# spacejam/tla-rust

Measured on AMD Instinct MI355X. Metric: distinct states/sec, raft.tla (3 servers), higher is better.
Workload: dtype u64

## Files before the change

### tla_rust_amd/build.py

```python
import os
import subprocess
from pathlib import Path

PKG = Path(__file__).resolve().parent
CSRC = PKG / "csrc"
OUT = PKG / "_build"
LIB = OUT / "libtlamc.so"
CLI = OUT / "mc"

SOURCES = ["engine.hip", "frontend.cpp"]

ENGINE_BASE = ["engine.hip", "hip_owned.h", "engine_kernels.h", "engine_sim.h", "sim_walk.h", "engine_behaviours.h", "behaviour.h", "engine_coverage.h", "coverage.h", "engine_violations.h", "violations.h",
               "engine_graph.h",
               "graph.h", "liveness.h", "live_query.h", "state_graph.h", "spec_gen.h", "mc_common.h", "spec_registry.h", "../../include/tlamc.h"]
ENGINE_OWN = {0: ["spec_pluscal.h", "spec_raft.h", "spec_ssi.h", "spec_vm.h", "spec_vm_cfg.h", "spec_paxos.h", "engine_pairs.h"], 7: ["spec_paxos.h"], 1: ["spec_pluscal.h"],
              2: ["spec_raft.h"], 3: ["spec_raft.h"], 4: ["spec_raft.h"], 5: ["spec_ssi.h", "engine_pairs.h"], 6: ["spec_vm.h", "spec_vm_cfg.h"]}
STATE_GRAPH_DEPS = ["state_graph.hip", "state_graph.h", "engine_live.h", "hip_owned.h", "liveness.h", "live_query.h", "graph.h", "coverage.h", "mc_common.h", "spec_registry.h",
                    "spec_gen.h", "spec_pluscal.h", "spec_raft.h", "spec_ssi.h", "spec_vm.h", "spec_vm_cfg.h", "spec_paxos.h", "../../include/tlamc.h"]


def _stale(target, deps):
    if not target.exists():
        return True
    t = target.stat().st_mtime
    return any(d.stat().st_mtime > t for d in deps)


def build(force=False, verbose=False):
    OUT.mkdir(exist_ok=True)
    hipcc = os.environ.get("HIPCC", "/opt/rocm/bin/hipcc")
    deps = list(CSRC.glob("*")) + [PKG.parent / "include" / "tlamc.h"]
    srcs = [str(CSRC / s) for s in SOURCES if (CSRC / s).exists()]
    common = [hipcc, "--offload-arch=gfx950", "-O3", "-std=c++17", "-fPIC", "-Wno-unused-value", "-Wno-unused-result",
              "-I", str(PKG.parent / "include")]
    if os.environ.get("TLAMC_LINE_TABLES"):
        common.append("-gline-tables-only")
    if os.environ.get("TLAMC_EXTRA_DEFS"):
        common += os.environ["TLAMC_EXTRA_DEFS"].split()
    if os.environ.get("TLAMC_PHASE_PROF"):
        common.append("-DMC_PHASE_PROF")
    jobs, objs = [], []
    for tu in range(8):
        obj = OUT / f"engine_tu{tu}.o"
        objs.append(obj)
        if force or _stale(obj, [CSRC / h for h in ENGINE_BASE + ENGINE_OWN[tu]]):
            jobs.append((obj, subprocess.Popen(common + ["-x", "hip", f"-DMC_TU={tu}", "-c", str(CSRC / "engine.hip"), "-o", str(obj)])))
    obj = OUT / "state_graph.o"
    objs.append(obj)
    if force or _stale(obj, [CSRC / d for d in STATE_GRAPH_DEPS]):
        jobs.append((obj, subprocess.Popen(common + ["-x", "hip", "-c", str(CSRC / "state_graph.hip"), "-o", str(obj)])))
    host_deps = {"frontend": ["frontend.cpp", "pcal.h", "spec_vm.h", "mc_common.h", "tlaeval.h"], "pcal": ["pcal.cpp", "pcal.h"],
                 "tlaeval": ["tlaeval.cpp", "tlaeval.h"],
                 "pcal_compile": ["pcal_compile.cpp", "pcal.h", "spec_vm.h", "spec_vm_cfg.h", "mc_common.h"],
                 "pcal_codegen": ["pcal_codegen.cpp", "pcal.h", "spec_vm.h", "mc_common.h"]}
    for name, dd in host_deps.items():
        obj = OUT / f"{name}.o"
        objs.append(obj)
        if force or _stale(obj, [CSRC / d for d in dd] + [PKG.parent / "include" / "tlamc.h"]):
            jobs.append((obj, subprocess.Popen(common + ["-x", "hip", "-c", str(CSRC / f"{name}.cpp"), "-o", str(obj)])))
    obj = OUT / "shard_rccl.o"
    objs.append(obj)
    if force or _stale(obj, [CSRC / "shard_rccl.cpp", CSRC / "shard_loop.h", PKG.parent / "include" / "tlamc.h"]):
        jobs.append((obj, subprocess.Popen(common + ["-x", "hip", "-c", str(CSRC / "shard_rccl.cpp"), "-o", str(obj)])))
    for obj, pr in jobs:
        if pr.wait() != 0:
            raise RuntimeError(f"hipcc failed for {obj.name}")
    if force or jobs or not LIB.exists():
        cmd = [hipcc, "--offload-arch=gfx950", "-shared", "-fPIC", "-o", str(LIB)] + [str(o) for o in objs] + ["-ldl", "-pthread"]
        if verbose:
            print(" ".join(cmd))
        subprocess.run(cmd, check=True)
    main = CSRC / "mc_main.cpp"
    if main.exists() and (force or _stale(CLI, deps + [LIB])):
        cmd = [hipcc, "-O2", "-std=c++17", "-I", str(PKG.parent / "include"), "-o", str(CLI), str(main),
               "-L", str(OUT), "-ltlamc", "-Wl,-rpath,$ORIGIN"]
        if verbose:
            print(" ".join(cmd))
        subprocess.run(cmd, check=True)
    calib_src = PKG.parent / "profiles" / "calib" / "calib_fetch.hip"
    calib = OUT / "calib_fetch"
    if calib_src.exists() and (force or _stale(calib, [calib_src])):
        subprocess.run([hipcc, "--offload-arch=gfx950", "-O3", "-Wno-unused-value", "-Wno-unused-result", "-o", str(calib), str(calib_src)], check=True)
    loc_src = PKG.parent / "profiles" / "calib" / "probe_locality.hip"
    loc = OUT / "probe_locality"
    if loc_src.exists() and (force or _stale(loc, [loc_src])):
        subprocess.run([hipcc, "--offload-arch=gfx950", "-O3", "-Wno-unused-value", "-Wno-unused-result", "-o", str(loc), str(loc_src)], check=True)
    return LIB


if __name__ == "__main__":
    print(build(force=True, verbose=True))
```

### tla_rust_amd/csrc/coverage.h

```cpp
#pragma once
#include "mc_common.h"
#include "spec_registry.h"
#include "spec_gen.h"

namespace mc {

constexpr int COV_MAX_BINS = 512;

MC_HD bool cov_counts(unsigned st) { return (st & ST_ENABLED) != 0; }

template <class S>
struct CovAction;

template <>
struct CovAction<SpecAtomicAdd> {
    static constexpr bool BY_SLOT = true;
    MC_HD static int nbins(const SpecAtomicAdd::Params &) { return 3 + 1; }
    MC_HD static bool listed(const SpecAtomicAdd::Params &, int a) { return a >= 0 && a < 3; }
    template <class Ref>
    MC_HD static int of(const SpecAtomicAdd::Params &p, const SpecAtomicAdd::Local &, Ref, int slot) { return SpecAtomicAdd::action_of(p, nullptr, slot); }
};
template <>
struct CovAction<SpecPcalIntro> {
    static constexpr bool BY_SLOT = false;
    MC_HD static int nbins(const SpecPcalIntro::Params &) { return 5 + 1; }
    MC_HD static bool listed(const SpecPcalIntro::Params &, int a) { return a >= 0 && a < 5; }
    template <class Ref>
    MC_HD static int of(const SpecPcalIntro::Params &p, const SpecPcalIntro::Local &l, Ref, int slot) { return SpecPcalIntro::action_of(p, &l.w, slot); }
};
template <>
struct CovAction<SpecPaxos> {
    static constexpr bool BY_SLOT = true;
    MC_HD static int nbins(const PaxosParams &) { return 6 + 1; }
    MC_HD static bool listed(const PaxosParams &p, int a) { return p.kind == 1 ? (a >= 0 && a < 2) : (a >= 2 && a < 6); }
    template <class Ref>
    MC_HD static int of(const PaxosParams &p, const SpecPaxos::Local &, Ref, int slot) { return SpecPaxos::action_of(p, nullptr, slot); }
};
template <int N>
struct CovAction<SpecRaft<N>> {
    using S = SpecRaft<N>;
    static constexpr bool BY_SLOT = false;
    MC_HD static int nbins(const RaftParams &) { return 10 + 1; }
    MC_HD static bool listed(const RaftParams &, int a) { return a >= 0 && a < 10; }
    template <class Ref>
    MC_HD static int of(const RaftParams &p, const typename S::Local &l, Ref s, int slot) {
        typename S::Delta d;
        int action = -1;
        S::compute(p, l, s, slot, d, action);
        return action;
    }
};
template <>
struct CovAction<SpecSsi> {
    static constexpr bool BY_SLOT = false;
    MC_HD static int nbins(const SsiParams &) { return 7 + 1; }
    MC_HD static bool listed(const SsiParams &, int a) { return a >= 0 && a < 7; }
    template <class Ref>
    MC_HD static int of(const SsiParams &p, const SpecSsi::Local &l, Ref, int slot) {
        SpecSsi::Delta d;
        int action = -1;
        SpecSsi::compute(p, l, slot, d, action);
        return action;
    }
};
MC_HD int cov_vm_nlabels(const VmParams &p) { return p.self_tab - p.label_tab; }
template <int MAXV>
struct CovAction<SpecVmT<MAXV>> {
    using S = SpecVmT<MAXV>;
    static constexpr bool BY_SLOT = false;
    MC_HD static int nbins(const VmParams &p) { return cov_vm_nlabels(p) + 1 + 1; }
    MC_HD static bool listed(const VmParams &p, int a) { return a >= 0 && a <= cov_vm_nlabels(p) && a != p.done; }
    template <class Ref>
    MC_HD static int of(const VmParams &p, const typename S::Local &l, Ref, int slot) {
        if (slot >= p.ninst * p.maxch) return cov_vm_nlabels(p);
        return slot < 0 ? -1 : l.v[p.pc_base + slot / p.maxch];
    }
};
template <int MAXV>
struct CovAction<SpecVmCfgT<MAXV>> : CovAction<SpecVmT<MAXV>> {};
template <class G>
struct CovAction<SpecGenT<G>> {
    using S = SpecGenT<G>;
    static constexpr bool BY_SLOT = false;
    MC_HD static int nbins(const VmParams &) { return G::NLABELS + 1 + 1; }
    MC_HD static bool listed(const VmParams &, int a) { return a >= 0 && a <= G::NLABELS && a != G::DONE; }
    template <class Ref>
    MC_HD static int of(const VmParams &, const typename S::Local &, Ref s, int slot) {
        if (slot >= G::NINST * G::MAXCH) return G::NLABELS;
        return slot < 0 ? -1 : (int)G::pc_from_row(s, slot / G::MAXCH);
    }
};

template <class S, class Add>
inline void cov_state(const typename S::Params &prm, CWordRef s, Add &&add) {
    typename S::Local loc;
    S::load(prm, s, loc);
    const int ns = S::nslots(prm, loc);
    for (int slot = 0; slot < ns; ++slot) {
        uint64_t fp = 0;
        const unsigned st = S::eval(prm, loc, s, slot, fp);
        if (cov_counts(st)) add(CovAction<S>::of(prm, loc, s, slot));
    }
}

}
```

### tla_rust_amd/csrc/engine.hip

```cpp
#include <hip/hip_runtime.h>

#include <algorithm>
#include <chrono>
#include <memory>
#include <type_traits>
#include <string>
#include <vector>

#include "spec_registry.h"
#include "hip_owned.h"

namespace mc {

#ifndef MC_TU
#define MC_TU -1
#endif
}
#include "engine_kernels.h"
#include "engine_pairs.h"
#include "engine_sim.h"
#include "engine_behaviours.h"
#include "engine_coverage.h"
#include "engine_violations.h"
#include "engine_graph.h"
#include "state_graph.h"
namespace mc {

struct EngineBase {
    DevBuf<int32_t> owned_device_blob;
    uint64_t program_hash = 0;
    mc_progress_fn progress_fn = nullptr;
    void *progress_user = nullptr;
    double progress_interval = 1.0;
    std::chrono::steady_clock::time_point progress_last;
    bool stop_requested = false;
    void report_progress(uint32_t levels, uint64_t generated, uint64_t distinct, uint64_t queue) {
        if (!progress_fn) return;
        const auto now = std::chrono::steady_clock::now();
        if (std::chrono::duration<double>(now - progress_last).count() < progress_interval) return;
        progress_last = now;
        progress_fn(progress_user, levels, generated, distinct, queue);
    }
    virtual ~EngineBase() = default;
    virtual int run(mc_result *out) = 0;
    virtual int step(uint32_t levels, mc_result *out) = 0;
    virtual int trace(uint8_t *states_out, int32_t *actions_out, size_t *n_inout) = 0;
    virtual int kernel_stats(mc_kernel_stats *out) = 0;
    virtual int read_states(uint64_t first, uint64_t count, uint8_t *out) = 0;
    virtual int debug_reexpand(unsigned extra_flags, double *ms) = 0;
    virtual int debug_phases(uint64_t *out48, int reset) = 0;
    virtual int debug_flags(uint32_t set, uint32_t clear) = 0;
    virtual int seen_layout(uint64_t *buckets, uint32_t *slots) = 0;
    virtual int checkpoint(const char *path) = 0;
    virtual int restore(const char *path) = 0;
    virtual int shard_begin() = 0;
    virtual int shard_begin_replicated(uint64_t min_frontier, uint64_t max_distinct, uint64_t max_levels, uint64_t *levels_out, uint32_t *nlevels) = 0;
    virtual int shard_level_size(uint64_t *n) = 0;
    virtual int shard_set_stream(void *hip_stream, int enable) = 0;
    virtual int shard_expand_launch(unsigned slot, uint64_t first, uint64_t count, uint64_t send_cap) = 0;
    virtual int shard_expand_finish(unsigned slot, uint64_t *send_fp, uint64_t send_cap, uint64_t *send_counts) = 0;
    virtual int shard_probe(const uint64_t *recv_fp, uint64_t n, uint8_t *answers) = 0;
    virtual int shard_expand_pack(unsigned slot, uint64_t *send_fp, uint64_t cap) = 0;
    virtual int shard_probe_pack(const uint64_t *recv_fp, uint64_t cap, uint8_t *answers) = 0;
    virtual int shard_keep_pack(unsigned slot, const uint8_t *answers_back, uint64_t cap) = 0;
    virtual int shard_wait_keep(unsigned slot) = 0;
    virtual int shard_materialise(unsigned slot, const uint8_t *answers_back, uint8_t *send_states, uint64_t send_cap, uint64_t *send_counts) = 0;
    virtual int shard_ingest(const uint8_t *recv_states, uint64_t n) = 0;
    virtual int shard_keep(unsigned slot, const uint8_t *answers_back, uint64_t *n_new) = 0;
    virtual int shard_end_level(uint64_t *new_local) = 0;
    virtual int shard_counters(uint64_t *generated, uint64_t *distinct_local, int32_t *verdict) = 0;
    virtual int shard_check_frontier() = 0;
    virtual int shard_materialise_parents(unsigned slot, uint64_t *send_parents) = 0;
    virtual int shard_ingest_parents(const uint64_t *recv_parents, uint64_t n, unsigned src_rank) = 0;
    virtual int shard_violation(int32_t *found, uint64_t *idx, uint32_t *slot, int32_t *verdict, int32_t *invariant) = 0;
    virtual int shard_fetch(uint64_t idx, uint8_t *state_out, uint32_t *parent_rank, uint64_t *parent_idx, uint32_t *parent_slot) = 0;
    virtual int shard_info(void **main_stream, uint64_t *chunk_states, int32_t *traced) = 0;
    virtual int shard_note_levels(const uint64_t *levels, uint32_t n, int32_t verdict) = 0;
    virtual int shard_resume(uint64_t *levels_out, uint32_t *nlevels) = 0;
    virtual int shard_checkpoint(const char *path) = 0;
    virtual int shard_restore(const char *path) = 0;
    virtual size_t state_bytes() const = 0;
    virtual int simulate(const mc_sim_opts *opts, mc_sim_result *out) = 0;
    virtual int behaviours(const mc_beh_opts *opts, mc_beh_verdict *out, mc_beh_result *result) = 0;
    virtual int behaviours_refused() = 0;
    virtual const mc_spec_desc *spec_desc() const = 0;
    virtual int coverage(mc_action_coverage *out, size_t *n_inout) = 0;
    virtual int violations(mc_violations_info *info, mc_violation *out, size_t *n_inout) = 0;
    virtual int violation_trace(size_t k, uint8_t *states_out, int32_t *actions_out, size_t *n_inout) = 0;
    StateGraph gr;
    bool sharded = false;
    hipStream_t graph_stream = nullptr;
    const std::vector<uint64_t> *graph_levels = nullptr;
    virtual int graph(mc_graph_info *out) = 0;
    virtual int predicates(uint64_t first, uint64_t count, uint32_t *bits_out) = 0;
    virtual int liveness_run(const LiveQuery &q, const mc_live_property *prop, mc_live_info *out, mc_live_check_info *check_out, mc_live_strong_info *strong_out) = 0;
    int liveness_edge_units(uint64_t first, uint64_t count, int8_t *unit_out) { return gr.live_unit_read(first, count, unit_out); }
    int graph_read(uint64_t first, uint64_t count, uint64_t *offsets_out, uint32_t *dst_out, int32_t *action_out, size_t *nedges_inout) {
        return gr.read(first, count, offsets_out, dst_out, action_out, nedges_inout);
    }
    int scc(mc_scc_info *out) {
        memset(out, 0, sizeof *out);
        if (sharded) { set_error("mc_engine_scc: not available for a sharded engine (shard_count > 1)"); return MC_EBADCFG; }
        if (!gr.built) { mc_graph_info gi; if (int rc = graph(&gi)) return rc; }
        return gr.scc(graph_stream, out);
    }
    int scc_read(uint64_t first, uint64_t count, uint32_t *scc_out) { return gr.scc_read(first, count, scc_out); }
    int liveness_components(uint64_t first, uint64_t count, uint32_t *scc_out) { return gr.live_scc_read(first, count, scc_out); }
    int liveness_trace(uint32_t *prefix_out, size_t *nprefix_inout, uint32_t *cycle_out, size_t *ncycle_inout) {
        return gr.live_trace(*graph_levels, prefix_out, nprefix_inout, cycle_out, ncycle_inout);
    }
};

static uint64_t round_pow2(uint64_t v) {
    uint64_t p = 1;
    while (p < v) p <<= 1;
    return p;
}

struct KTimer {
    std::vector<Event> pool;
    struct Pending { int which; size_t e0, e1; uint64_t units; };
    std::vector<Pending> pending;
    size_t used = 0;
    bool enabled = false;
    hipEvent_t get() {
        if (used == pool.size()) pool.emplace_back(hipEventDefault);
        return pool[used++].get();
    }
    void resolve(mc_kernel_stat *stats ) {
        for (auto &p : pending) {
            float ms = 0;
            hipEventElapsedTime(&ms, pool[p.e0].get(), pool[p.e1].get());
            stats[p.which].launches++;
            stats[p.which].ms_total += ms;
            stats[p.which].units += p.units;
        }
        pending.clear();
        used = 0;
    }
};

template <class S, class = void>
struct HasExport : std::false_type {};
template <class S>
struct HasExport<S, decltype((void)S::EXPORT_WORDS)> : std::true_type {};
template <class S, class = void>
struct PackedRows : std::false_type {};
template <class S>
struct PackedRows<S, decltype((void)S::PACKED_ROWS)> : std::integral_constant<bool, S::PACKED_ROWS> {};

static_assert((unsigned)SIM_VK_INVARIANT == VK_INVARIANT && (unsigned)SIM_VK_ASSERT == VK_ASSERT && (unsigned)SIM_VK_DEADLOCK == VK_DEADLOCK, "one verdict_of_kind");
static int32_t verdict_of_kind(unsigned kind) {
    return kind == VK_INVARIANT ? MC_V_INVARIANT : kind == VK_ASSERT ? MC_V_ASSERT : kind == VK_DEADLOCK ? MC_V_DEADLOCK : MC_V_SPECERR;
}
struct Viol {
    unsigned kind, slot;
    int32_t verdict, invariant;
    explicit Viol(unsigned long long key)
        : kind((unsigned)(key & 7u)), slot((unsigned)(key >> 8 & 0xffffu)), verdict(verdict_of_kind(kind)), invariant(kind == VK_INVARIANT ? (int32_t)(key >> 3 & 31u) : -1) {}
    bool extra_state() const { return kind == VK_INVARIANT && slot < SLOT_PARENT; }
};

struct CkIdent {
    char magic[8];
    uint32_t spec_id, nparams;
    int64_t params[16];
    uint32_t words, has_trace;
};
struct CkHeader {
    CkIdent id;
    uint64_t distinct, generated, cells, lo, hi, nlevels;
};
struct ShCkHeader {
    CkIdent id;
    uint32_t rank, world;
    uint64_t table_cap, lo, hi, next, dup, nlevels;
};
struct ShCkCounters {
    uint64_t arena_next, viol_key, via_list;
    uint64_t generated[NSHARD], cells[NSHARD];
    uint32_t error, pad;
};
static_assert(sizeof(CkIdent) == 152 && offsetof(CkIdent, spec_id) == 8 && offsetof(CkIdent, params) == 16 && offsetof(CkIdent, words) == 144 && offsetof(CkIdent, has_trace) == 148, "checkpoint identity");
static_assert(sizeof(CkHeader) == 200 && offsetof(CkHeader, distinct) == 152 && offsetof(CkHeader, generated) == 160 && offsetof(CkHeader, cells) == 168 &&
              offsetof(CkHeader, lo) == 176 && offsetof(CkHeader, hi) == 184 && offsetof(CkHeader, nlevels) == 192, "TLAMCCK1 header");
static_assert(sizeof(ShCkHeader) == 208 && offsetof(ShCkHeader, rank) == 152 && offsetof(ShCkHeader, world) == 156 && offsetof(ShCkHeader, table_cap) == 160 &&
              offsetof(ShCkHeader, lo) == 168 && offsetof(ShCkHeader, hi) == 176 && offsetof(ShCkHeader, next) == 184 && offsetof(ShCkHeader, dup) == 192 &&
              offsetof(ShCkHeader, nlevels) == 200, "TLAMCSK2 header");
static_assert(NSHARD == 8 && sizeof(ShCkCounters) == 160 && offsetof(ShCkCounters, generated) == 24 && offsetof(ShCkCounters, cells) == 88 && offsetof(ShCkCounters, error) == 152, "TLAMCSK2 counters");
struct CkFormat { const char *magic, *writer, *reader, *not_ours, *other_program; };
static constexpr CkFormat CK_FUSED{"TLAMCCK1", "checkpoint", "restore", "not a checkpoint file",
                                   "the checkpoint was written by another compiled program (algorithm, constants, invariants or constraints differ)"};
static constexpr CkFormat CK_RANK{"TLAMCSK2", "mc_shard_checkpoint", "mc_shard_restore", "not a per-rank checkpoint file (of this library version)",
                                  "the checkpoint was written by another compiled program"};
struct CkPart { void *p; size_t bytes; };
struct FileCloser { FILE *f; ~FileCloser() { if (f) fclose(f); } };

template <class S>
struct Engine : EngineBase {
    using Params = typename S::Params;
    int W = 1;
    unsigned max_slots = 1;
    Params prm;
    mc_spec_desc desc;
    mc_config cfg;
    Stream stream, stream2;
    Stream stream_b;
    Event ev_level, ev_e[2], ev_m[2];
    DevBuf<uint64_t> d_arena, d_table, d_cand, d_inittmp;
    DevBuf<uint32_t> d_newlist, d_parent;
    DevBuf<uint64_t> d_newfp;
    DevBuf<uint16_t> d_nsl, d_pslot;
    DevBuf<uint8_t> d_prank;
    DevBuf<DevCounters> d_ctr;
    PinnedBuf<DevCounters> h_ctr;
    DevBuf<LevelCtl> d_lc;
    PinnedBuf<LevelCtl> h_lc;
    uint64_t table_cap = 0, arena_cap = 0, chunk = 0, row_stride = 0, seg_cap = 0;
    bool seen_sparse = false, use_matrix = false;
    bool no_slices = getenv("TLAMC_NOSLICE") != nullptr;
    double inwave_growth_limit = getenv("TLAMC_INWAVE_GROWTH") ? atof(getenv("TLAMC_INWAVE_GROWTH")) : 10.0;
    KTimer timer;
    mc_kernel_stat kstat[3];
    struct Fused {
        bool have_run = false, have_viol = false;
        unsigned long long last_viol = ~0ull;
        std::vector<uint64_t> level_start;
        uint64_t last_distinct = 0, last_generated = 0, cells = 0, inwave = 0;
        uint64_t stop_frontier = 0, lo = 0, hi = 0;
        bool mat_inwave_level = false;
        uint64_t mat_list_hint = 0;
    } fr;
    struct HandOver {
        bool pending = false, in_place = false;
        uint64_t distinct = 0, generated = 0, cells = 0, lo = 0;
        std::vector<uint64_t> level_start;
    } ck;
    struct ShSlot {
        DevBuf<uint64_t> rt_fp;
        DevBuf<uint32_t> rt_src, pend_src;
        DevBuf<PaddedCounter> rt_cur;
        uint64_t rt_subcap = 0, pend_total = 0, chunk_base = 0, count = 0, ncols = 0;
        BlockPlan plan;
        uint64_t moved = 0;
        OwnerOffsets pend_off;
        bool launched = false, keep_pending = false;
    };
    struct Shard {
        uint64_t lo = 0, hi = 0, next = 0;
        uint64_t dup = 0;
        ShSlot sl[2];
        DevBuf<uint32_t> d_new_src, d_incl;
        DevBuf<unsigned long long> d_ends;
        PinnedBuf<unsigned long long> h_ends;
        PinnedBuf<PaddedCounter> h_cur;
        DevBuf<char> d_scan_tmp;
        hipStream_t ext_stream = nullptr;
        bool ext_side = false;
        Event ev_slot[2], ev_keep[2], ev_ans;
        Event ev_append;
        Event ev_exp[2];
        Event ev_mat[2];
        std::vector<uint64_t> levels;
        bool ck_ok = false, resume = false;
        std::unique_ptr<mc_result> prefix_res{new mc_result()};
    } sh;
    struct Sim {
        DevBuf<uint64_t> buf[2];
        DevBuf<uint32_t> wst;
        DevBuf<SimCounters> ctr;
        std::vector<uint64_t> trace_rows;
        std::vector<int32_t> trace_acts;
        size_t trace_n = 0;
    } sim;
    struct Beh {
        DevBuf<uint64_t> set[2], stage, rows, first, carry, mask;
        DevBuf<mc_beh_verdict> out;
        DevBuf<BehCounters> ctr;
    } beh;
    struct Cov {
        bool on = false;
        int nbins = 0;
        DevBuf<unsigned long long> bins;
        std::vector<uint64_t> host;
        uint64_t init_generated = 0;
    } cov;
    struct Vio {
        bool on = false;
        DevBuf<ViolBins> bins;
        ViolBins host;
        bool have_first = false, fatal = false;
        unsigned long long first_key = ~0ull;
        uint32_t flagged_levels = 0, passes = 0;
    } vio;

    unsigned slices_for(uint64_t ncols, bool blind) const {
        if (!WantsSlices<S>::value || S::FIX_SLOTS != 0 || UsesFamilies<S>::value || pairs_only() || use_matrix || max_slots < 16 || no_slices) return 1;
        const uint64_t waves = (ncols + 63) / 64;
        uint64_t sg = blind ? 32 : (16384 + waves - 1) / waves;
        if (sg > 32) sg = 32;
        if (sg > max_slots / 4) sg = max_slots / 4;
        return sg < 1 ? 1u : (unsigned)sg;
    }
    uint64_t seen_arg() const { return seen_sparse ? ((table_cap / MC_SPARSE_SLOTS) | SEEN_SPARSE) : table_cap / 8; }
    unsigned nranks() const { return cfg.shard_count > 1 ? cfg.shard_count : 1; }

    int alloc() {
        W = S::words(prm);
        max_slots = (unsigned)S::max_slots(prm);
        use_matrix = (cfg.flags & MC_F_MATRIX) != 0;
        HIP_TRY(hipSetDevice(cfg.device));
        HIP_TRY(stream.create());
        sharded = cfg.shard_count > 1;
        graph_stream = stream;
        graph_levels = &fr.level_start;
        {
            const char *pe = getenv("TLAMC_PRIO");
            int lo_p = 0, hi_p = 0;
            hipDeviceGetStreamPriorityRange(&lo_p, &hi_p);
            if (pe && *pe == '1') HIP_TRY(stream2.create(hi_p));
            else if (pe && *pe == '2') HIP_TRY(stream2.create(lo_p));
            else HIP_TRY(stream2.create());
        }
        for (int i = 0; i < 2; i++) { HIP_TRY(ev_e[i].create()); HIP_TRY(ev_m[i].create()); }
        {
            const char *es = getenv("TLAMC_EXPAND_STREAMS");
            if (es && *es == '2') {
                HIP_TRY(stream_b.create());
                HIP_TRY(ev_level.create());
            }
        }
        table_cap = cfg.table_capacity ? cfg.table_capacity : (1ull << 24);
        table_cap = (table_cap + 63) / 64 * 64;
        if (table_cap / 8 > 0xffffffffull) { set_error("table_capacity: at most 2^35 - 8 slots per device"); return MC_EBADCFG; }
        arena_cap = cfg.arena_capacity ? cfg.arena_capacity : (1ull << 22);
        arena_cap = (arena_cap + 63) & ~63ull;
        if (arena_cap >= (1ull << 32) - 1) { set_error("arena_capacity must be < 2^32 states"); return MC_EBADCFG; }
        static const double sparse_ratio = getenv("TLAMC_SPARSE_RATIO") && atof(getenv("TLAMC_SPARSE_RATIO")) >= 1.25 ? atof(getenv("TLAMC_SPARSE_RATIO")) : 3.0;
        seen_sparse = (double)table_cap >= sparse_ratio * (double)arena_cap && table_cap / MC_SPARSE_SLOTS <= 0xffffffffull && !getenv("TLAMC_DENSE_TABLE");
        chunk = cfg.chunk_states ? cfg.chunk_states : (1ull << 18);
        chunk = (chunk + 255) & ~255ull;
        if (chunk > (1ull << 24) - 256) chunk = (1ull << 24) - 256;
        if (max_slots > 255) { set_error("spec has more than 255 action slots per state"); return MC_EBADCFG; }
        row_stride = chunk + 256;
        HIP_TRY(d_arena.alloc(arena_cap * W));
        HIP_TRY(d_table.alloc(table_cap));
        HIP_TRY(d_cand.alloc((size_t)(use_matrix ? max_slots : 1) * row_stride));
        seg_cap = (row_stride / NSHARD + 256) * max_slots;
        seg_cap += seg_cap / 64 + 65;
        HIP_TRY(d_newlist.alloc((size_t)2 * NSHARD * seg_cap));
        if (HasKnownFp<S>::value && !use_matrix) HIP_TRY(d_newfp.alloc((size_t)2 * NSHARD * seg_cap));
        {
            const uint64_t ni = S::num_init(prm);
            HIP_TRY(d_inittmp.alloc((size_t)(ni < chunk ? ni : chunk) * W));
        }
        HIP_TRY(d_nsl.alloc(row_stride));
        if (cfg.flags & MC_F_TRACE) {
            HIP_TRY(d_parent.alloc(arena_cap));
            HIP_TRY(d_pslot.alloc(arena_cap));
            if (cfg.shard_count > 1) {
                HIP_TRY(d_prank.alloc(arena_cap));
                HIP_TRY(hipMemset(d_prank, 0xff, arena_cap));
            }
        }
        HIP_TRY(d_ctr.alloc(1));
        HIP_TRY(h_ctr.alloc(1));
        HIP_TRY(d_lc.alloc(1));
        HIP_TRY(h_lc.alloc(1));
        timer.enabled = (cfg.flags & MC_F_TIMING) != 0;
        if (cfg.flags & MC_F_COVERAGE) {
            cov.nbins = CovAction<S>::nbins(prm);
            if (cov.nbins > COV_MAX_BINS) { set_error("MC_F_COVERAGE: the model has more actions than the coverage histogram has bins (" + std::to_string(COV_MAX_BINS - 1) + ")"); return MC_EBADCFG; }
            HIP_TRY(cov.bins.alloc((size_t)2 * cov.nbins));
            HIP_TRY(hipMemset(cov.bins, 0, (size_t)2 * cov.nbins * sizeof(unsigned long long)));
            cov.host.assign((size_t)2 * cov.nbins, 0);
            cov.on = true;
        }
        if (cfg.flags & MC_F_CONTINUE) {
            if (ViolModel<S>::ninv(prm) > VIOL_MAX_INV) { set_error("MC_F_CONTINUE: the model has more than 32 invariants"); return MC_EBADCFG; }
            HIP_TRY(vio.bins.alloc(1));
            vio.on = true;
        }
        return MC_OK;
    }

    int viol_begin() {
        memset(&vio.host, 0, sizeof vio.host);
        for (int i = 0; i < VIOL_CELLS; i++) vio.host.first[i] = ~0ull;
        vio.have_first = vio.fatal = false;
        vio.first_key = ~0ull;
        vio.flagged_levels = vio.passes = 0;
        HIP_TRY(hipMemcpyAsync(vio.bins, &vio.host, sizeof vio.host, hipMemcpyHostToDevice, stream));
        return MC_OK;
    }
    void viol_stored(uint64_t lo, uint64_t hi) {
        for (uint64_t c0 = lo; c0 < hi; c0 += chunk) {
            const uint64_t c1 = c0 + chunk < hi ? c0 + chunk : hi;
            hipLaunchKernelGGL(k_viol_stored<S>, dim3((unsigned)((c1 - c0 + 255) / 256)), dim3(256), 0, stream, prm, (const uint64_t *)d_arena,
                               (const uint32_t *)d_parent, (const uint16_t *)d_pslot, c0, c1, vio.bins.p);
            vio.passes++;
        }
    }
    void viol_frontier(uint64_t lo, uint64_t hi) {
        each_chunk(lo, hi, [&](uint64_t c0, uint64_t c1, uint64_t ncols) {
            hipLaunchKernelGGL(k_viol_frontier<S>, dim3((unsigned)((ncols + 255) / 256)), dim3(256), 0, stream, prm, (const uint64_t *)d_arena,
                               c0, c1, ncols, (unsigned)cfg.flags, vio.bins.p);
            vio.passes++;
        });
    }
    int viol_level(uint64_t lo, uint64_t hi, uint64_t new_hi, bool expanded) {
        if (!vio.have_first) { vio.have_first = true; vio.first_key = h_ctr->viol_key; }
        vio.flagged_levels++;
        if (expanded) viol_frontier(lo, hi);
        if (!expanded || ChecksOnExpand<S>::value) viol_stored(lo, hi);
        else viol_stored(hi, new_hi);
        HIP_TRY(hipGetLastError());
        HIP_TRY(hipMemcpyAsync(&vio.host, vio.bins, sizeof vio.host, hipMemcpyDeviceToHost, stream));
        HIP_TRY(hipStreamSynchronize(stream));
        if (vio.host.count[VIOL_BINS + VIOL_BIN_FATAL]) { vio.fatal = true; return MC_OK; }
        hipLaunchKernelGGL(k_clear_viol_key, dim3(1), dim3(1), 0, stream, d_ctr.p);
        h_ctr->viol_key = ~0ull;
        return MC_OK;
    }
    uint32_t level_of(uint64_t idx) const {
        const auto it = std::upper_bound(fr.level_start.begin(), fr.level_start.end(), idx);
        return (uint32_t)(it - fr.level_start.begin());
    }
    struct ViolEntry { mc_violation v; int shown; unsigned long long key; };
    size_t viol_entries() const { return (size_t)ViolModel<S>::ninv(prm) + ((cfg.flags & MC_F_DEADLOCK) ? 1 : 0) + (vio.fatal ? 1 : 0); }
    int viol_entry(size_t k, ViolEntry &e) {
        const size_t ninv = (size_t)ViolModel<S>::ninv(prm);
        memset(&e, 0, sizeof e);
        e.v.invariant = -1;
        e.v.first_state = ~0ull;
        const bool dl = (cfg.flags & MC_F_DEADLOCK) != 0;
        int bin;
        if (k < ninv) { bin = (int)k; e.v.kind = MC_V_INVARIANT; e.v.invariant = (int32_t)k; }
        else if (dl && k == ninv) { bin = VIOL_BIN_DEADLOCK; e.v.kind = MC_V_DEADLOCK; }
        else if (vio.fatal && k == ninv + (dl ? 1 : 0)) bin = VIOL_BIN_FATAL;
        else { set_error("mc_engine_violations: entry out of range"); return MC_EBADCFG; }
        e.v.states = vio.host.count[bin];
        e.v.outside = vio.host.count[VIOL_BINS + bin];
        if (e.v.states) { e.shown = 1; e.v.first_state = vio.host.first[bin]; }
        else if (e.v.outside) {
            e.shown = 2;
            e.key = vio.host.first[VIOL_BINS + bin];
            e.v.first_state = viol_idx(e.key);
            if (bin == VIOL_BIN_FATAL) { const Viol f(e.key); e.v.kind = f.verdict; e.v.invariant = f.invariant; }
        }
        if (e.shown) {
            e.v.first_level = level_of(e.v.first_state);
            e.v.trace_len = e.v.first_level + (e.shown == 2 && Viol(e.key).extra_state() ? 1u : 0u);
        }
        return MC_OK;
    }
    int violations(mc_violations_info *info, mc_violation *out, size_t *n_inout) override {
        if (!vio.on) { set_error("mc_engine_violations: the engine was created without MC_F_CONTINUE"); return MC_ESTATE; }
        if (!fr.have_run) { set_error("mc_engine_violations: needs a search of this engine that returned a result"); return MC_ESTATE; }
        const size_t n = viol_entries();
        if (info) { info->flagged_levels = vio.flagged_levels; info->passes = vio.passes; info->fatal = vio.fatal ? 1u : 0u; info->pad = 0; }
        if (n > *n_inout || !out) { *n_inout = n; set_error("mc_engine_violations: buffer too small"); return MC_EBADCFG; }
        HIP_TRY(hipSetDevice(cfg.device));
        for (size_t k = 0; k < n; k++) {
            ViolEntry e;
            if (int rc = viol_entry(k, e)) return rc;
            out[k] = e.v;
        }
        *n_inout = n;
        return MC_OK;
    }
    int violation_trace(size_t k, uint8_t *states_out, int32_t *actions_out, size_t *n_inout) override {
        if (!vio.on) { set_error("mc_engine_violation_trace: the engine was created without MC_F_CONTINUE"); return MC_ESTATE; }
        if (!fr.have_run) { set_error("mc_engine_violation_trace: needs a search of this engine that returned a result"); return MC_ESTATE; }
        if (k >= viol_entries()) { set_error("mc_engine_violation_trace: entry out of range"); return MC_EBADCFG; }
        HIP_TRY(hipSetDevice(cfg.device));
        ViolEntry e;
        if (int rc = viol_entry(k, e)) return rc;
        if (!e.shown) { set_error("mc_engine_violation_trace: the entry has nothing to show"); return MC_EBADCFG; }
        const bool extra = e.shown == 2 && Viol(e.key).extra_state();
        return chain_trace(e.v.first_state, extra, extra ? Viol(e.key).slot : 0u, states_out, actions_out, n_inout);
    }

    template <class F>
    void each_chunk(uint64_t lo, uint64_t hi, F &&f) { mc::each_chunk(lo, hi, chunk, f); }
    void cov_generated(uint64_t lo, uint64_t hi) {
        each_chunk(lo, hi, [&](uint64_t c0, uint64_t c1, uint64_t ncols) {
            hipLaunchKernelGGL(k_coverage_generated<S>, dim3((unsigned)((ncols + 255) / 256)), dim3(256), 0, stream, prm, (const uint64_t *)d_arena,
                               c0, c1, ncols, cov.bins.p, cov.nbins);
        });
    }
    void cov_distinct(uint64_t lo, uint64_t hi) {
        for (uint64_t c0 = lo; c0 < hi; c0 += chunk) {
            const uint64_t c1 = c0 + chunk < hi ? c0 + chunk : hi;
            hipLaunchKernelGGL(k_coverage_distinct<S>, dim3((unsigned)((c1 - c0 + 255) / 256)), dim3(256), 0, stream, prm, (const uint64_t *)d_arena,
                               (const uint32_t *)d_parent, (const uint16_t *)d_pslot, c0, c1, cov.bins.p + cov.nbins, cov.nbins);
        }
    }
    int cov_begin(uint64_t expanded, uint64_t stored) {
        HIP_TRY(hipMemsetAsync(cov.bins, 0, (size_t)2 * cov.nbins * sizeof(unsigned long long), stream));
        cov.init_generated = S::num_init(prm);
        cov_generated(0, expanded);
        cov_distinct(0, stored);
        return MC_OK;
    }
    int cov_end() {
        HIP_TRY(hipMemcpyAsync(cov.host.data(), cov.bins, cov.host.size() * sizeof(uint64_t), hipMemcpyDeviceToHost, stream));
        HIP_TRY(hipStreamSynchronize(stream));
        cov.host[0] += cov.init_generated;
        return MC_OK;
    }
    int coverage(mc_action_coverage *out, size_t *n_inout) override {
        if (!cov.on) { set_error("mc_engine_coverage: the engine was created without MC_F_COVERAGE"); return MC_ESTATE; }
        size_t n = 1;
        for (int a = 0; a + 1 < cov.nbins; a++) n += CovAction<S>::listed(prm, a) ? 1 : 0;
        if (n > *n_inout || !out) { *n_inout = n; set_error("mc_engine_coverage: buffer too small"); return MC_EBADCFG; }
        size_t k = 0;
        for (int a = -1; a + 1 < cov.nbins; a++) {
            if (a >= 0 && !CovAction<S>::listed(prm, a)) continue;
            out[k].action = a;
            out[k].pad = 0;
            out[k].generated = cov.host[(size_t)a + 1];
            out[k].distinct = cov.host[(size_t)cov.nbins + a + 1];
            k++;
        }
        *n_inout = n;
        return MC_OK;
    }

    template <class K, class... A>
    void graph_chunks(K kernel, uint64_t lo, uint64_t hi, A... args) {
        each_chunk(lo, hi, [&](uint64_t c0, uint64_t c1, uint64_t ncols) {
            hipLaunchKernelGGL(kernel, dim3((unsigned)((ncols + 255) / 256)), dim3(256), 0, stream, prm, (const uint64_t *)d_arena, c0, c1, ncols,
                               (const uint64_t *)d_table, seen_arg(), args...);
        });
    }
    int graph(mc_graph_info *out) override {
        memset(out, 0, sizeof *out);
        if (cfg.shard_count > 1) { set_error("mc_engine_graph: not available for a sharded engine (shard_count > 1)"); return MC_EBADCFG; }
        if (!fr.have_run || ck.pending) {
            set_error("mc_engine_graph: needs a search of this engine that returned a result (mc_engine_run / mc_engine_step; not a simulation, "
                      "not a restored checkpoint that has not run yet: its seen-set is not built)");
            return MC_ESTATE;
        }
        gr.release();
        gr.device = cfg.device;
        const uint64_t n = fr.last_distinct, expanded = fr.lo;
        if (n + 1 > 0x7fffffffull) { set_error("mc_engine_graph: at most 2^31 - 2 states (the scan's item count)"); return MC_EBADCFG; }
        HIP_TRY(hipSetDevice(cfg.device));
        const auto t0 = std::chrono::steady_clock::now();
        DevBuf<uint32_t> slot_index, degree;
        DevBuf<GraphCounters> d_gc;
        DevBuf<char> scan_tmp;
        int rc;
        if ((rc = graph_alloc(slot_index, table_cap, "the fingerprint -> state index"))) return rc;
        if ((rc = graph_alloc(degree, n + 1, "the out-degrees"))) return rc;
        if ((rc = graph_alloc(gr.offsets, n + 1, "the row offsets"))) { gr.release(); return rc; }
        if ((rc = graph_alloc(d_gc, 1, "the counters"))) { gr.release(); return rc; }
        const int built = graph_build(n, expanded, slot_index, degree, d_gc, scan_tmp);
        if (built) { gr.release(); return built; }
        gr.info.states = n;
        gr.info.expanded = expanded;
        gr.info.init_states = fr.level_start.size() > 1 ? fr.level_start[1] : n;
        gr.info.seconds = std::chrono::duration<double>(std::chrono::steady_clock::now() - t0).count();
        gr.built = true;
        *out = gr.info;
        return MC_OK;
    }
    int graph_build(uint64_t n, uint64_t expanded, DevBuf<uint32_t> &slot_index, DevBuf<uint32_t> &degree, DevBuf<GraphCounters> &d_gc, DevBuf<char> &scan_tmp) {
        GraphCounters gc;
        memset(&gc, 0, sizeof gc);
        gc.first_bad = ~0ull;
        HIP_TRY(hipMemcpyAsync(d_gc, &gc, sizeof gc, hipMemcpyHostToDevice, stream));
        HIP_TRY(hipMemsetAsync(slot_index, 0xff, table_cap * sizeof(uint32_t), stream));
        HIP_TRY(hipMemsetAsync(degree, 0, (n + 1) * sizeof(uint32_t), stream));
        if (n) hipLaunchKernelGGL(k_graph_index<S>, dim3((unsigned)((n + 255) / 256)), dim3(256), 0, stream, prm, (const uint64_t *)d_arena, n,
                                  (const uint64_t *)d_table, seen_arg(), slot_index.p, table_cap, d_gc.p);
        graph_chunks(k_graph_degree<S>, 0, expanded, degree.p, d_gc.p);
        HIP_TRY(hipGetLastError());
        if (int rc = scan_exclusive_u32_to_u64(degree.p, gr.offsets.p, n + 1, scan_tmp, stream, "mc_engine_graph")) return rc;
        uint64_t edges = 0;
        HIP_TRY(hipMemcpyAsync(&edges, gr.offsets.p + n, sizeof edges, hipMemcpyDeviceToHost, stream));
        HIP_TRY(hipMemcpyAsync(&gc, d_gc, sizeof gc, hipMemcpyDeviceToHost, stream));
        HIP_TRY(hipStreamSynchronize(stream));
        if (int rc = graph_inconsistent(gc)) return rc;
        if (int rc = graph_alloc(gr.dst, edges, "the edges' successors")) return rc;
        if (int rc = graph_alloc(gr.act, edges, "the edges' actions")) return rc;
        graph_chunks(k_graph_fill<S>, 0, expanded, (const uint32_t *)slot_index.p, table_cap, (const uint64_t *)gr.offsets.p, gr.dst.p, gr.act.p, d_gc.p);
        HIP_TRY(hipGetLastError());
        HIP_TRY(hipMemcpyAsync(&gc, d_gc, sizeof gc, hipMemcpyDeviceToHost, stream));
        HIP_TRY(hipStreamSynchronize(stream));
        if (int rc = graph_inconsistent(gc)) return rc;
        gr.info.edges = edges;
        gr.info.self_loops = gc.self_loops;
        gr.info.dropped = gc.dropped;
        gr.info.max_out_degree = gc.max_degree;
        return MC_OK;
    }
    static int graph_inconsistent(const GraphCounters &gc) {
        if (!gc.missing_states && !gc.missing_succ) return MC_OK;
        const unsigned long long idx = gc.first_bad >> 16;
        const unsigned slot = (unsigned)(gc.first_bad & 0xffffu);
        set_error("mc_engine_graph: the seen-set does not hold " + std::to_string(gc.missing_states) + " stored state(s) and " + std::to_string(gc.missing_succ) +
                  " in-model successor(s); the first: state " + std::to_string(idx) + (slot == GRAPH_SLOT_SELF ? " itself" : ", slot " + std::to_string(slot)) +
                  " (two different states with one 64-bit fingerprint are the only legitimate cause: the second is never stored); no graph was built");
        return MC_ESTATE;
    }

    int predicates_build(const char *call) {
        if constexpr (!LivePred<S>::HAS) {
            return MC_ENOSPEC;
        } else {
            auto &lv = gr.lv;
            if (lv.pred_built) return MC_OK;
            LivePredTab tab;
            memset(&tab, 0, sizeof tab);
            tab.n = vm_live_preds(prm.host, tab.entry, LIVE_MAX_PREDS);
            if (tab.n > LIVE_MAX_PREDS) { set_error(std::string(call) + ": at most 32 predicates"); return MC_EBADCFG; }
            const uint64_t n = gr.info.states;
            HIP_TRY(hipSetDevice(cfg.device));
            DevBuf<unsigned long long> d_bad;
            if (int rc = graph_alloc(lv.pred, n, "the predicate bits", call)) return rc;
            if (int rc = graph_alloc(d_bad, 1, "the counters", call)) return rc;
            unsigned long long bad = ~0ull;
            HIP_TRY(hipMemcpyAsync(d_bad, &bad, sizeof bad, hipMemcpyHostToDevice, stream));
            HIP_TRY(hipMemsetAsync(lv.pred, 0, (n ? n : 1) * sizeof(uint32_t), stream));
            if (tab.n) graph_chunks(k_live_pred<S>, 0, n, tab, lv.pred.p, d_bad.p);
            HIP_TRY(hipGetLastError());
            HIP_TRY(hipMemcpyAsync(&bad, d_bad, sizeof bad, hipMemcpyDeviceToHost, stream));
            HIP_TRY(hipStreamSynchronize(stream));
            if (bad != ~0ull) {
                lv.pred.reset();
                set_error(std::string(call) + ": evaluating the predicate `" + vm_live_pred_text(prm.host, (int)(bad & 0xff)) + "` fails in state " +
                          std::to_string(bad >> 8) + " (an evaluation error: a function applied outside its domain, an overflow, ...)");
                return MC_ESTATE;
            }
            lv.pred_built = true;
            lv.npred = tab.n;
            return MC_OK;
        }
    }
    int predicates(uint64_t first, uint64_t count, uint32_t *bits_out) override {
        if (cfg.shard_count > 1) { set_error("mc_engine_predicates: not available for a sharded engine (shard_count > 1)"); return MC_EBADCFG; }
        if constexpr (!LivePred<S>::HAS) {
            set_error("mc_engine_predicates: this lowering has no compiled predicates (compiled PlusCal programs only)");
            return MC_ENOSPEC;
        } else {
            if (!gr.built) { mc_graph_info gi; if (int rc = graph(&gi)) return rc; }
            if (int rc = predicates_build("mc_engine_predicates")) return rc;
            return gr.pred_read(first, count, bits_out);
        }
    }

    static_assert(LiveProc<S>::HAS == LivePred<S>::HAS, "a lowering with process instances compiles predicates, and no other does");
    DevBuf<int8_t> live_unit_tab;
    int liveness_run(const LiveQuery &query, const mc_live_property *prop, mc_live_info *out, mc_live_check_info *check_out, mc_live_strong_info *strong_out) override {
        LiveQuery q = query;
        const std::string call(q.call);
        auto t0 = std::chrono::steady_clock::now();
        if (out) memset(out, 0, sizeof *out);
        if (check_out) memset(check_out, 0, sizeof *check_out);
        if (strong_out) memset(strong_out, 0, sizeof *strong_out);
        if (cfg.shard_count > 1) { set_error(call + ": not available for a sharded engine (shard_count > 1)"); return MC_EBADCFG; }
        if constexpr (!LiveProc<S>::HAS) {
            set_error(call + ": this lowering has no process instances (compiled PlusCal programs only)");
            return MC_ENOSPEC;
        } else {
            if (!fr.have_run || ck.pending || fr.have_viol || fr.hi != fr.lo) {
                set_error(call + ": needs a search of this engine that finished without a violation and with an empty queue (the complete state graph)");
                return MC_ESTATE;
            }
            if (!q.fu) {
                const int np = LiveProc<S>::count(prm);
                if (np > LIVE_MAX_PROCS) { set_error(call + ": at most 64 process instances"); return MC_EBADCFG; }
                q.all = np >= 64 ? ~0ull : (1ull << np) - 1;
            }
            if (prop && prop->refused) { set_error(call + ": the front end refused " + prop->name); return MC_EBADCFG; }
            if (prop && q.term()) { set_error(call + ": " + live_unknown_kind(q.kind)); return MC_EBADCFG; }
            if (int rc = live_query_check(q, prop ? vm_live_preds(prm.host, nullptr, 0) : 0)) return rc;
            int ni = 0, nl = 0;
            if (q.fu) {
                const int nu = vm_live_units(prm.host, &ni, &nl, nullptr, 0);
                if (q.fu->nunits < nu) { set_error(call + ": the program has " + std::to_string(nu) + " units, the table " + std::to_string(q.fu->nunits)); return MC_EBADCFG; }
            }
            if (!gr.built || !gr.lv.scc_built) { mc_scc_info si; if (int rc = scc(&si)) return rc; }
            auto &lv = gr.lv;
            const uint64_t edges = gr.info.edges;
            HIP_TRY(hipSetDevice(cfg.device));
            if (!q.refine && !prop) t0 = std::chrono::steady_clock::now();
            if (!q.fu && !lv.proc_built) {
                if (int rc = graph_alloc(lv.proc, edges, "the edges' processes", q.call)) return rc;
                HIP_TRY(hipMemsetAsync(lv.proc, 0xff, (edges ? edges : 1) * sizeof(int8_t), stream));
                graph_chunks(k_live_proc<S>, 0, fr.lo, (const uint64_t *)gr.offsets.p, lv.proc.p);
                lv.proc_built = true;
            }
            if (q.fu && !lv.unit_built) {
                std::vector<int8_t> tab((size_t)ni * (size_t)nl + 1, (int8_t)LIVE_TERM);
                vm_live_units(prm.host, &ni, &nl, tab.data(), (int)tab.size());
                if (int rc = graph_alloc(live_unit_tab, tab.size(), "the units of the labels", q.call)) return rc;
                if (int rc = graph_alloc(lv.unit, edges, "the edges' units", q.call)) return rc;
                HIP_TRY(hipMemcpyAsync(live_unit_tab, tab.data(), tab.size() * sizeof(int8_t), hipMemcpyHostToDevice, stream));
                HIP_TRY(hipMemsetAsync(lv.unit, 0xff, (edges ? edges : 1) * sizeof(int8_t), stream));
                graph_chunks(k_live_unit<S>, 0, fr.lo, (const uint64_t *)gr.offsets.p, LiveUnitTab{ni, nl, (const int8_t *)live_unit_tab.p}, lv.unit.p);
                HIP_TRY(hipStreamSynchronize(stream));
                lv.unit_built = true;
            }
            if (prop) if (int rc = predicates_build(q.call)) return rc;
            return gr.live_check(q, stream, t0, out, check_out, strong_out);
        }
    }

    template <class F>
    void timed(int which, uint64_t units, F &&launch, hipStream_t on = nullptr) {
        if (!timer.enabled) { launch(); return; }
        if (!on) on = stream;
        hipEvent_t a = timer.get(), b = timer.get();
        size_t ia = timer.used - 2, ib = timer.used - 1;
        hipEventRecord(a, on);
        launch();
        hipEventRecord(b, on);
        timer.pending.push_back({which, ia, ib, units});
    }

    int read_counters() {
        if (stream_b) HIP_TRY(hipStreamSynchronize(stream_b));
        HIP_TRY(hipStreamSynchronize(stream2));
        HIP_TRY(hipMemcpyAsync(h_ctr, d_ctr, sizeof(DevCounters), hipMemcpyDeviceToHost, stream));
        HIP_TRY(hipStreamSynchronize(stream));
        if (timer.enabled) timer.resolve(kstat);
        return MC_OK;
    }
    int check_dev_error() {
        if (h_ctr->error & DEV_EOVERFLOW) { set_error("packed-state capacity exceeded (raft messages / elections / allLogs slots, or a PlusCal sequence longer than its cells, or a recursive PlusCal procedure deeper than $TLAMC_PCAL_STACK frames)"); return MC_EOVERFLOW; }
        if (h_ctr->error & DEV_ETABLE) { set_error("seen-set full: raise table_capacity"); return MC_ETABLEFULL; }
        if (h_ctr->error & DEV_EROUTE) { set_error("sharded round: an exchange bucket is full (raise the fan-out allowance / send capacity)"); return MC_EROUTE; }
        if (h_ctr->error & DEV_EARENA) { set_error("state arena full: raise arena_capacity"); return MC_EARENA; }
        return MC_OK;
    }

    bool inwave_ok() const { return (UsesFamilies<S>::value || UsesPairs<S>::value) && !use_matrix && !(cfg.flags & (MC_F_NOFAMILY | MC_F_NOINWAVE)); }
    bool pairs_only() const { return UsesPairs<S>::value && inwave_ok(); }
    void set_inwave(RouteArgs &rt) const {
        if (!inwave_ok()) return;
        rt.arena_w = d_arena;
        rt.arena_cap = arena_cap;
        rt.parent = d_parent;
        rt.pslot = d_pslot;
    }
    static unsigned mat_grid(uint64_t ncols) {
        const unsigned bx = (unsigned)((ncols + 255) / 256);
        const unsigned gm = bx < 8 * 256 ? (bx + 7) / 8 : 256;
        return gm ? gm : 1u;
    }
    void finish_materialise(uint64_t chunk_base, uint64_t ncols, unsigned parity, hipStream_t expanded_on = nullptr) {
        if (pairs_only()) return;
        unsigned gm = mat_grid(ncols);
        if (fr.mat_inwave_level) {
            const uint64_t want = (fr.mat_list_hint * 4 + 255) / 256;
            const unsigned per_seg = (unsigned)((want + NSHARD - 1) / NSHARD);
            if (per_seg < gm) gm = per_seg ? per_seg : 1u;
        }
        hipEventRecord(ev_e[parity].get(), expanded_on ? expanded_on : stream.s);
        hipStreamWaitEvent(stream2, ev_e[parity].get(), 0);
        timed(2, 0, [&] {
            hipLaunchKernelGGL(k_materialise<S>, dim3(gm, NSHARD), dim3(256), 0, stream2, prm, d_arena, chunk_base, d_newlist,
                               seg_cap, arena_cap, d_parent, d_pslot, d_ctr, parity, (const LevelCtl *)nullptr, (const uint64_t *)d_newfp);
        }, stream2);
        hipLaunchKernelGGL(k_commit, dim3(1), dim3(1), 0, stream2, d_ctr, parity);
        hipEventRecord(ev_m[parity].get(), stream2);
        static const bool serial = getenv("TLAMC_SERIAL") != nullptr;
        if (serial) hipStreamSynchronize(stream2);
    }
    void enqueue_blind_level(uint64_t max_states) {
        const uint64_t ncols = max_states + 64;
        RouteArgs rt{};
        rt.lc = d_lc;
        rt.new_fp = d_newfp;
        set_inwave(rt);
        const unsigned sg = slices_for(ncols, true);
        const bool dl = sg > 1 && (cfg.flags & MC_F_DEADLOCK);
        if (dl) { rt.succ = d_nsl; hipMemsetAsync(d_nsl, 0, ncols * sizeof(uint16_t), stream); }
        const unsigned lflags = cfg.flags | ((cfg.flags & MC_F_PARK) ? MC_FI_PARK : 0u);
        timed(0, 0, [&] {
            launch_expand<S, false>(!(cfg.flags & MC_F_NOFAMILY), lflags, ncols, stream, sg, prm, (const uint64_t *)d_arena,
                                    (uint64_t)0, (uint64_t)0, ncols, d_table.p, seen_arg(), d_newlist.p, seg_cap, d_ctr.p, cfg.flags, rt, 0u);
            if (dl) hipLaunchKernelGGL(k_deadlock_slices, dim3((unsigned)((ncols + 255) / 256)), dim3(256), 0, stream, (const uint16_t *)d_nsl,
                                       (uint64_t)0, (uint64_t)0, ncols, (const LevelCtl *)d_lc, d_ctr);
        });
        if (!pairs_only()) timed(2, 0, [&] {
            hipLaunchKernelGGL(k_materialise<S>, dim3(32, NSHARD), dim3(256), 0, stream, prm, d_arena, (uint64_t)0, d_newlist, seg_cap,
                               arena_cap, d_parent, d_pslot, d_ctr, 0u, (const LevelCtl *)d_lc, (const uint64_t *)d_newfp);
        });
        hipLaunchKernelGGL(k_end_level, dim3(1), dim3(1), 0, stream, d_ctr, d_lc);
    }

    template <bool INIT>
    void finish_chunk(uint64_t chunk_base_or_first, uint64_t ncols, unsigned rows) {
        const unsigned bx = (unsigned)((ncols + 255) / 256);
        timed(1, ncols * rows, [&] {
            hipLaunchKernelGGL(k_insert, dim3(bx, rows), dim3(256), 0, stream, d_cand, row_stride, ncols, d_nsl, d_table,
                               seen_arg(), d_newlist, d_ctr);
        });
        const unsigned gm = bx < 2048 ? bx : 2048;
        timed(2, 0, [&] {
            if (INIT)
                hipLaunchKernelGGL(k_init_materialise<S>, dim3(gm), dim3(256), 0, stream, prm, d_arena, chunk_base_or_first,
                                   d_inittmp, d_newlist, arena_cap, d_parent, d_pslot, d_ctr);
            else
                hipLaunchKernelGGL(k_materialise<S>, dim3(gm, 1), dim3(256), 0, stream, prm, d_arena, chunk_base_or_first,
                                   d_newlist, seg_cap, arena_cap, d_parent, d_pslot, d_ctr, 0u, (const LevelCtl *)nullptr, (const uint64_t *)nullptr);
        });
        hipLaunchKernelGGL(k_commit, dim3(1), dim3(1), 0, stream, d_ctr, 0u);
    }

    int seed_init(unsigned rank, unsigned count, bool resuming, bool in_place, std::chrono::steady_clock::time_point *t0) {
        if (!in_place) HIP_TRY(hipMemsetAsync(d_table, 0, table_cap * sizeof(uint64_t), stream));
        HIP_TRY(hipMemsetAsync(d_ctr, 0, sizeof(DevCounters), stream));
        DevCounters init_c;
        memset(&init_c, 0, sizeof init_c);
        init_c.viol_key = ~0ull;
        if (resuming) {
            init_c.arena_next = ck.distinct;
            init_c.generated[0].v = ck.generated;
            init_c.cells[0].v = ck.cells;
        }
        HIP_TRY(hipMemcpyAsync(d_ctr, &init_c, sizeof init_c, hipMemcpyHostToDevice, stream));
        if (t0) {
            HIP_TRY(hipStreamSynchronize(stream));
            *t0 = std::chrono::steady_clock::now();
        }
        if (resuming && ck.distinct && !in_place)
            hipLaunchKernelGGL(k_reseed_table<S>, dim3((unsigned)((ck.distinct + 255) / 256)), dim3(256), 0, stream, prm,
                               (const uint64_t *)d_arena, ck.distinct, d_table, seen_arg(), d_ctr);
        const uint64_t ninit = resuming ? 0 : S::num_init(prm);
        for (uint64_t first = 0; first < ninit; first += chunk) {
            const uint64_t n = ninit - first < chunk ? ninit - first : chunk;
            const uint64_t ncols = (n + 63) & ~63ull;
            hipLaunchKernelGGL(k_init_cand<S>, dim3((unsigned)((ncols + 255) / 256)), dim3(256), 0, stream, prm, first, n,
                               d_inittmp, d_cand, ncols, d_nsl, d_ctr, rank, count);
            finish_chunk<true>(first, ncols, 1);
        }
        return MC_OK;
    }
    int close_level(uint64_t &lo, uint64_t &hi, uint64_t new_hi, uint32_t &level, mc_result *out) {
        lo = hi;
        hi = new_hi;
        if (hi > lo) {
            fr.level_start.push_back(lo);
            if (level < MC_MAX_LEVELS) out->level_distinct[level] = hi - lo;
            level++;
        }
        if (level >= MC_MAX_LEVELS) { set_error("too many BFS levels"); return MC_EBADCFG; }
        return MC_OK;
    }

    int run(mc_result *out) override {
        memset(out, 0, sizeof *out);
        out->violated_invariant = -1;
        memset(kstat, 0, sizeof kstat);
        fr.have_viol = false;
        sim.trace_n = 0;
        stop_requested = false;
        gr.release();
        fr.have_run = false;
        fr.level_start.clear();
        HIP_TRY(hipSetDevice(cfg.device));
        const bool resuming = ck.pending, in_place = ck.pending && ck.in_place;
        ck.pending = ck.in_place = false;
        std::chrono::steady_clock::time_point t0;
        int rc = seed_init(0u, 1u, resuming, in_place, &t0);
        if (rc) return rc;
        progress_last = t0;
        auto progress = [&](uint32_t lv, uint64_t lo_, uint64_t hi_) {
            if (!progress_fn) return;
            uint64_t g = 0;
            for (int t = 0; t < NSHARD; t++) g += h_ctr->generated[t].v;
            report_progress(lv, g, hi_, hi_ - lo_);
        };
        if (inwave_ok()) hipLaunchKernelGGL(k_set_alloc_mode, dim3(1), dim3(1), 0, stream, d_ctr, 1u);
        bool alloc_atomic = inwave_ok();
        uint64_t prev_frontier = ~0ull >> 12;
        if ((rc = read_counters())) return rc;
        if ((rc = check_dev_error())) return rc;
        uint64_t lo = 0, hi = h_ctr->arena_next;
        uint32_t level = 1;
        out->level_distinct[0] = hi;
        fr.level_start.push_back(0);
        if (cov.on && !in_place && (rc = cov_begin(resuming ? ck.lo : 0, hi))) return rc;
        if (vio.on) {
            if ((rc = viol_begin())) return rc;
            if (!resuming && h_ctr->viol_key != ~0ull && (rc = viol_level(0, hi, hi, false))) return rc;
        }
        if (resuming) {
            fr.level_start = ck.level_start;
            level = (uint32_t)fr.level_start.size();
            lo = ck.lo;
            for (uint32_t k = 0; k < level && k < MC_MAX_LEVELS; k++)
                out->level_distinct[k] = (k + 1 < level ? fr.level_start[k + 1] : hi) - fr.level_start[k];
        }
        int budget = 0;
        uint64_t via_seen = 0;
        const bool park_levels = (cfg.flags & MC_F_PARK) != 0;
        fr.mat_list_hint = ~0ull >> 8;
        fr.mat_inwave_level = false;
        static const int blind_log2 = getenv("TLAMC_BLIND_LOG2") ? atoi(getenv("TLAMC_BLIND_LOG2")) : 20;
        uint64_t blind_max = 1ull << (blind_log2 >= 10 && blind_log2 <= 23 && slices_for((1ull << 16) + 64, true) == 1 ? blind_log2 : 16);
        if (chunk < blind_max) blind_max = chunk;
        while (hi > lo) {
            if (h_ctr->viol_key != ~0ull) break;
            if (fr.stop_frontier && hi - lo >= fr.stop_frontier) break;
            if (cfg.max_levels && level >= cfg.max_levels) { budget = 1; break; }
            if (cfg.max_distinct && hi >= cfg.max_distinct) { budget = 1; break; }
            if (stop_requested) { budget = 1; break; }
            if (!use_matrix && !(cfg.flags & MC_F_NOBATCH) && hi - lo <= blind_max) {
                memset(h_lc, 0, sizeof(LevelCtl));
                h_lc->lo = lo;
                h_lc->hi = hi;
                h_lc->max_states = fr.stop_frontier && fr.stop_frontier - 1 < blind_max ? fr.stop_frontier - 1 : blind_max;
                h_lc->max_distinct = cfg.max_distinct;
                h_lc->levels_left = cfg.max_levels ? (unsigned)(cfg.max_levels - level) : 0u;
                HIP_TRY(hipMemcpyAsync(d_lc, h_lc, sizeof(LevelCtl), hipMemcpyHostToDevice, stream));
                HIP_TRY(hipStreamSynchronize(stream2));
                if (inwave_ok() && !alloc_atomic) {
                    hipLaunchKernelGGL(k_set_alloc_mode, dim3(1), dim3(1), 0, stream, d_ctr, 1u);
                    alloc_atomic = true;
                }
                for (int k = 0; k < BLIND_BATCH; k++) enqueue_blind_level(blind_max);
                HIP_TRY(hipMemcpyAsync(h_lc, d_lc, sizeof(LevelCtl), hipMemcpyDeviceToHost, stream));
                if ((rc = read_counters())) return rc;
                if ((rc = check_dev_error())) return rc;
                for (unsigned k = 0; k < h_lc->nlev; k++) {
                    kstat[0].units += hi - lo;
                    if (cov.on) { cov_generated(lo, hi); cov_distinct(hi, h_lc->level_hi[k]); }
                    if (vio.on && k + 1 == h_lc->nlev && h_ctr->viol_key != ~0ull && (rc = viol_level(lo, hi, h_lc->level_hi[k], true))) return rc;
                    if ((rc = close_level(lo, hi, h_lc->level_hi[k], level, out))) return rc;
                }
                progress(level, lo, hi);
                prev_frontier = hi > lo ? hi - lo : 1;
                continue;
            }
            const bool lvl_inwave = inwave_ok() && (pairs_only() || (double)(hi - lo) <= inwave_growth_limit * (double)prev_frontier);
            if (inwave_ok() && lvl_inwave != alloc_atomic) {
                hipLaunchKernelGGL(k_set_alloc_mode, dim3(1), dim3(1), 0, stream, d_ctr, lvl_inwave ? 1u : 0u);
                alloc_atomic = lvl_inwave;
            }
            prev_frontier = hi - lo;
            fr.mat_inwave_level = lvl_inwave;
            unsigned chunk_no = 0;
            const bool two_streams = stream_b && !use_matrix && hi - lo > chunk && !(slices_for(chunk, false) > 1 && (cfg.flags & MC_F_DEADLOCK));
            if (two_streams) {
                hipEventRecord(ev_level.get(), stream);
                hipStreamWaitEvent(stream_b, ev_level.get(), 0);
            }
            for (uint64_t c0 = lo; c0 < hi; ++chunk_no) {
                const unsigned parity = chunk_no & 1u;
                const uint64_t base = c0 & ~63ull;
                uint64_t c1 = base + chunk;
                if (c1 > hi) c1 = hi;
                const uint64_t ncols = ((c1 - base) + 63) & ~63ull;
                if (use_matrix) {
                    timed(0, c1 - c0, [&] {
                        hipLaunchKernelGGL(k_expand<S>, dim3((unsigned)((ncols + 255) / 256)), dim3(256), 0, stream, prm, d_arena,
                                           c0, c1, d_cand, row_stride, ncols, d_nsl, d_ctr, cfg.flags);
                    });
                    finish_chunk<false>(base, ncols, max_slots);
                } else {
                    hipStream_t es = two_streams && parity ? stream_b.s : stream.s;
                    if (chunk_no >= 2) hipStreamWaitEvent(es, ev_m[parity].get(), 0);
                    RouteArgs rt_new{};
                    rt_new.new_fp = d_newfp;
                    if (lvl_inwave) set_inwave(rt_new);
                    const unsigned sg = slices_for(ncols, false);
                    const bool dl = sg > 1 && (cfg.flags & MC_F_DEADLOCK);
                    if (dl) { rt_new.succ = d_nsl; hipMemsetAsync(d_nsl, 0, ncols * sizeof(uint16_t), es); }
                    const unsigned lflags = cfg.flags | (lvl_inwave && park_levels ? MC_FI_PARK : 0u);
                    timed(0, c1 - c0, [&] {
                        launch_expand<S, false>(!(cfg.flags & MC_F_NOFAMILY), lflags, ncols, es, sg, prm,
                                                (const uint64_t *)d_arena, c0, c1, ncols, d_table.p, seen_arg(), d_newlist.p, seg_cap, d_ctr.p,
                                                cfg.flags, rt_new, parity);
                        if (dl) hipLaunchKernelGGL(k_deadlock_slices, dim3((unsigned)((ncols + 255) / 256)), dim3(256), 0, es,
                                                   (const uint16_t *)d_nsl, c0, c1, ncols, (const LevelCtl *)nullptr, d_ctr);
                    }, es);
                    finish_materialise(base, ncols, parity, es);
                }
                c0 = c1;
            }
            if ((rc = read_counters())) return rc;
            if ((rc = check_dev_error())) return rc;
            {
                const uint64_t via = h_ctr->via_list - via_seen;
                via_seen = h_ctr->via_list;
                const double growth = hi > lo ? (double)(h_ctr->arena_next - hi) / (double)(hi - lo) : 1.0;
                fr.mat_list_hint = (uint64_t)((double)(via / (chunk_no ? chunk_no : 1u)) * (growth > 1.0 ? growth : 1.0)) + 1;
            }
            if (cov.on) { cov_generated(lo, hi); cov_distinct(hi, h_ctr->arena_next); }
            if (vio.on && h_ctr->viol_key != ~0ull && (rc = viol_level(lo, hi, h_ctr->arena_next, true))) return rc;
            if ((rc = close_level(lo, hi, h_ctr->arena_next, level, out))) return rc;
            progress(level, lo, hi);
        }
        if (cov.on && (rc = cov_end())) return rc;
        if (hi > lo && h_ctr->viol_key == ~0ull && !fr.stop_frontier && (rc = check_frontier(lo, hi))) return rc;
        if (vio.on && hi > lo && !vio.fatal && h_ctr->viol_key != ~0ull && (rc = viol_level(lo, hi, hi, false))) return rc;
        const unsigned long long run_key = vio.on && vio.have_first ? vio.first_key : h_ctr->viol_key;
        const auto t1 = std::chrono::steady_clock::now();
        out->seconds = std::chrono::duration<double>(t1 - t0).count();
        out->distinct = h_ctr->arena_next;
        fr.last_distinct = h_ctr->arena_next;
        kstat[2].units = h_ctr->arena_next;
        out->generated = 0;
        fr.cells = 0;
        for (int t = 0; t < NSHARD; t++) { out->generated += h_ctr->generated[t].v; fr.cells += h_ctr->cells[t].v; }
        fr.last_generated = out->generated;
        fr.inwave = inwave_ok() && h_ctr->arena_next >= h_ctr->via_list + (resuming ? ck.distinct : 0)
                           ? h_ctr->arena_next - h_ctr->via_list - (resuming ? ck.distinct : 0) : 0;
        fr.have_run = true;
        out->queue_left = hi - lo;
        out->depth = level;
        out->levels = level;
        fr.lo = lo;
        fr.hi = hi;
        if (run_key != ~0ull) {
            fr.have_viol = true;
            fr.last_viol = run_key;
            const Viol v(fr.last_viol);
            out->verdict = v.verdict;
            out->violated_invariant = v.invariant;
            std::vector<uint64_t> chain;
            if (build_chain(chain) == MC_OK) out->trace_len = (uint32_t)chain.size() + (v.extra_state() ? 1u : 0u);
        } else {
            out->verdict = budget ? MC_V_BUDGET : MC_V_OK;
        }
        return MC_OK;
    }

    int step(uint32_t levels, mc_result *out) override {
        if (!levels) return MC_EBADCFG;
        const uint64_t saved = cfg.max_levels;
        const bool cont = fr.have_run && !fr.have_viol && fr.hi > fr.lo && !ck.pending;
        if (cont) {
            ck.distinct = fr.last_distinct; ck.generated = fr.last_generated; ck.cells = fr.cells; ck.lo = fr.lo;
            ck.level_start = fr.level_start;
            ck.pending = ck.in_place = true;
            cfg.max_levels = (uint64_t)fr.level_start.size() + levels;
        } else if (ck.pending) {
            cfg.max_levels = (uint64_t)ck.level_start.size() + levels;
        } else {
            cfg.max_levels = levels;
        }
        const int rc = run(out);
        cfg.max_levels = saved;
        if (rc) ck.pending = ck.in_place = false;
        return rc;
    }
    bool ck_params_comparable() const { return desc.spec_id != MC_SPEC_PCAL; }
    void ck_fill_ident(CkIdent &id, const CkFormat &fmt) const {
        memcpy(id.magic, fmt.magic, 8);
        id.spec_id = desc.spec_id;
        id.nparams = ck_params_comparable() ? desc.nparams : 1;
        for (uint32_t i = 0; i < id.nparams && i < 16; i++) id.params[i] = desc.params[i];
        if (!ck_params_comparable()) id.params[0] = (int64_t)program_hash;
        id.words = (uint32_t)W;
        id.has_trace = d_parent ? 1u : 0u;
    }
    static int ck_fail(int code, const char *who, const std::string &msg) { set_error(std::string(who) + ": " + msg); return code; }
    int ck_check_ident(const CkIdent &id, const CkFormat &fmt) const {
        if (memcmp(id.magic, fmt.magic, 8) != 0) return ck_fail(MC_EPARSE, fmt.reader, fmt.not_ours);
        if (id.spec_id != desc.spec_id || id.words != (uint32_t)W) return ck_fail(MC_EBADCFG, fmt.reader, "the checkpoint belongs to another spec");
        if (ck_params_comparable() && (id.nparams != desc.nparams || memcmp(id.params, desc.params, sizeof(int64_t) * (id.nparams < 16 ? id.nparams : 16)) != 0))
            return ck_fail(MC_EBADCFG, fmt.reader, "the checkpoint was written with other constants / invariants");
        if (!ck_params_comparable() && (id.nparams != 1 || (uint64_t)id.params[0] != program_hash)) return ck_fail(MC_EBADCFG, fmt.reader, fmt.other_program);
        return MC_OK;
    }
    std::vector<CkPart> ck_sections(uint64_t n, bool per_rank) const {
        std::vector<CkPart> v{{d_arena.p, (size_t)((n + 63) >> 6) * (size_t)W * 64 * sizeof(uint64_t)}};
        if (d_parent) {
            v.push_back({d_parent.p, (size_t)n * sizeof(uint32_t)});
            v.push_back({d_pslot.p, (size_t)n * sizeof(uint16_t)});
        }
        if (per_rank && d_prank) v.push_back({d_prank.p, (size_t)n});
        if (per_rank) v.push_back({d_table.p, (size_t)table_cap * sizeof(uint64_t)});
        return v;
    }
    int ck_write(const CkFormat &fmt, const char *path, std::initializer_list<CkPart> host, const std::vector<CkPart> &dev) {
        FILE *f = fopen(path, "wb");
        if (!f) return ck_fail(MC_EBADCFG, fmt.writer, std::string("cannot write ") + path);
        FileCloser closer{f};
        int rc = MC_OK;
        for (const CkPart &h : host)
            if (!rc && fwrite(h.p, 1, h.bytes, f) != h.bytes) rc = ck_fail(MC_EBADCFG, fmt.writer, "short write");
        for (const CkPart &d : dev) {
            if (rc) break;
            std::vector<char> buf(d.bytes < (64u << 20) ? d.bytes : (64u << 20));
            for (size_t off = 0; off < d.bytes && !rc; off += buf.size()) {
                const size_t n = d.bytes - off < buf.size() ? d.bytes - off : buf.size();
                HIP_TRY(hipMemcpy(buf.data(), (const char *)d.p + off, n, hipMemcpyDeviceToHost));
                if (fwrite(buf.data(), 1, n, f) != n) rc = ck_fail(MC_EBADCFG, "checkpoint", "short write");
            }
        }
        closer.f = nullptr;
        if (fclose(f) != 0 && !rc) rc = ck_fail(MC_EBADCFG, fmt.writer, "close failed");
        return rc;
    }
    template <class H>
    int ck_read_header(const CkFormat &fmt, FILE *f, H &h) const {
        if (fread(&h, sizeof h, 1, f) != 1) return ck_fail(MC_EPARSE, fmt.reader, fmt.not_ours);
        return ck_check_ident(h.id, fmt);
    }
    static int ck_read_host(const CkFormat &fmt, FILE *f, std::initializer_list<CkPart> host) {
        for (const CkPart &h : host)
            if (fread(h.p, 1, h.bytes, f) != h.bytes) return ck_fail(MC_EPARSE, fmt.reader, "the checkpoint file is truncated");
        return MC_OK;
    }
    static int ck_read_sections(FILE *f, const std::vector<CkPart> &dev) {
        for (const CkPart &d : dev) {
            std::vector<char> buf(d.bytes < (64u << 20) ? d.bytes : (64u << 20));
            for (size_t off = 0; off < d.bytes; off += buf.size()) {
                const size_t n = d.bytes - off < buf.size() ? d.bytes - off : buf.size();
                if (fread(buf.data(), 1, n, f) != n) return ck_fail(MC_EPARSE, "restore", "the checkpoint file is truncated");
                HIP_TRY(hipMemcpy((char *)d.p + off, buf.data(), n, hipMemcpyHostToDevice));
            }
        }
        return MC_OK;
    }
    int checkpoint(const char *path) override {
        if (cfg.shard_count > 1) { set_error("checkpoint: not available for a sharded engine"); return MC_EBADCFG; }
        if (!fr.have_run || fr.have_viol) { set_error("checkpoint: needs a completed mc_engine_run that stopped on a budget (or finished) without a violation"); return MC_EBADCFG; }
        HIP_TRY(hipSetDevice(cfg.device));
        HIP_TRY(hipDeviceSynchronize());
        CkHeader h;
        memset(&h, 0, sizeof h);
        ck_fill_ident(h.id, CK_FUSED);
        h.distinct = fr.last_distinct; h.generated = fr.last_generated; h.cells = fr.cells;
        h.lo = fr.lo; h.hi = fr.hi; h.nlevels = fr.level_start.size();
        return ck_write(CK_FUSED, path, {{&h, sizeof h}, {fr.level_start.data(), fr.level_start.size() * sizeof(uint64_t)}}, ck_sections(fr.last_distinct, false));
    }
    int restore(const char *path) override {
        if (cfg.shard_count > 1) { set_error("restore: not available for a sharded engine"); return MC_EBADCFG; }
        gr.release();
        FileCloser f{fopen(path, "rb")};
        if (!f.f) return ck_fail(MC_EPARSE, "restore", std::string("cannot read ") + path);
        CkHeader h;
        int rc = ck_read_header(CK_FUSED, f.f, h);
        if (rc) return rc;
        if (h.distinct * 10 > table_cap * 9) return ck_fail(MC_ETABLEFULL, "restore", "table_capacity cannot hold the checkpoint's states (load > 0.9)");
        if (h.distinct > arena_cap) return ck_fail(MC_EARENA, "restore", "arena_capacity is smaller than the checkpoint");
        if (h.hi != h.distinct || h.lo > h.hi || h.nlevels == 0 || h.nlevels >= MC_MAX_LEVELS) return ck_fail(MC_EPARSE, "restore", "inconsistent header");
        if (d_parent && !h.id.has_trace) return ck_fail(MC_EBADCFG, "restore", "the checkpoint holds no parent pointers (written without MC_F_TRACE); run without MC_F_TRACE");
        ck.level_start.assign((size_t)h.nlevels, 0);
        if ((rc = ck_read_host(CK_FUSED, f.f, {{ck.level_start.data(), ck.level_start.size() * sizeof(uint64_t)}}))) return rc;
        bool ok = ck.level_start[0] == 0 && ck.level_start.back() < h.hi && (h.lo == h.hi || ck.level_start.back() == h.lo);
        for (size_t k = 1; k < ck.level_start.size() && ok; k++) ok = ck.level_start[k] > ck.level_start[k - 1];
        if (!ok) return ck_fail(MC_EPARSE, "restore", "inconsistent level table");
        HIP_TRY(hipSetDevice(cfg.device));
        if ((rc = ck_read_sections(f.f, ck_sections(h.distinct, false)))) return rc;
        ck.distinct = h.distinct; ck.generated = h.generated; ck.cells = h.cells; ck.lo = h.lo;
        ck.pending = true;
        return MC_OK;
    }
    int shard_checkpoint(const char *path) override {
        if (!sh.ck_ok || sh.levels.empty()) { set_error("mc_shard_checkpoint: needs a sharded run that ended (finished, or stopped on a budget) without an error"); return MC_EBADCFG; }
        HIP_TRY(hipSetDevice(cfg.device));
        HIP_TRY(hipDeviceSynchronize());
        ShCkHeader h;
        memset(&h, 0, sizeof h);
        ck_fill_ident(h.id, CK_RANK);
        h.rank = cfg.shard_rank; h.world = nranks();
        h.table_cap = table_cap | (seen_sparse ? SEEN_SPARSE : 0); h.lo = sh.lo; h.hi = sh.hi; h.next = sh.next; h.dup = sh.dup; h.nlevels = sh.levels.size();
        DevCounters dc;
        HIP_TRY(hipMemcpy(&dc, d_ctr, sizeof dc, hipMemcpyDeviceToHost));
        ShCkCounters c;
        memset(&c, 0, sizeof c);
        c.arena_next = dc.arena_next; c.viol_key = dc.viol_key; c.via_list = dc.via_list; c.error = dc.error;
        for (int t = 0; t < NSHARD; t++) { c.generated[t] = dc.generated[t].v; c.cells[t] = dc.cells[t].v; }
        return ck_write(CK_RANK, path, {{&h, sizeof h}, {sh.levels.data(), sh.levels.size() * sizeof(uint64_t)}, {&c, sizeof c}}, ck_sections(sh.next, true));
    }
    int shard_restore_read(FILE *f, ShCkHeader &h, ShCkCounters &fc) {
        int rc = ck_read_header(CK_RANK, f, h);
        if (rc) return rc;
        const char *who = CK_RANK.reader;
        if (h.rank != cfg.shard_rank || h.world != nranks()) return ck_fail(MC_EBADCFG, who, "the file is another rank's, or of a run with another number of ranks");
        if (h.table_cap != (table_cap | (seen_sparse ? SEEN_SPARSE : 0)))
            return ck_fail(MC_EBADCFG, who, "table_capacity differs from the checkpointed run's, or the bucket form it implies (4 slots when the table is >= 3 x the arena): the seen-set slice is stored as it lay in HBM");
        if (h.next > arena_cap) return ck_fail(MC_EARENA, who, "arena_capacity is smaller than the checkpoint");
        if (h.lo > h.hi || h.hi != h.next || h.dup > h.next || h.nlevels == 0 || h.nlevels >= MC_MAX_LEVELS) return ck_fail(MC_EPARSE, who, "inconsistent header");
        if ((d_parent.p != nullptr) != (h.id.has_trace != 0)) return ck_fail(MC_EBADCFG, who, "MC_F_TRACE differs from the checkpointed run's");
        sh.levels.assign((size_t)h.nlevels, 0);
        if ((rc = ck_read_host(CK_RANK, f, {{sh.levels.data(), sh.levels.size() * sizeof(uint64_t)}, {&fc, sizeof fc}}))) return rc;
        if (fc.arena_next != h.next || fc.viol_key != ~0ull || fc.error) return ck_fail(MC_EPARSE, who, "inconsistent counters");
        HIP_TRY(hipSetDevice(cfg.device));
        HIP_TRY(hipDeviceSynchronize());
        if ((rc = ck_read_sections(f, ck_sections(h.next, true)))) return rc;
        if (fgetc(f) != EOF) return ck_fail(MC_EPARSE, who, "trailing bytes (not the file this engine's configuration wrote)");
        return MC_OK;
    }
    int shard_restore(const char *path) override {
        if (int rc = refuse_packed()) return rc;
        FileCloser f{fopen(path, "rb")};
        if (!f.f) return ck_fail(MC_EPARSE, "mc_shard_restore", std::string("cannot read ") + path);
        ShCkHeader h;
        ShCkCounters fc;
        if (int rc = shard_restore_read(f.f, h, fc)) { sh.levels.clear(); return rc; }
        DevCounters c;
        memset(&c, 0, sizeof c);
        c.arena_next = fc.arena_next; c.viol_key = fc.viol_key; c.via_list = fc.via_list;
        for (int t = 0; t < NSHARD; t++) { c.generated[t].v = fc.generated[t]; c.cells[t].v = fc.cells[t]; }
        HIP_TRY(hipMemcpy(d_ctr, &c, sizeof c, hipMemcpyHostToDevice));
        memset(kstat, 0, sizeof kstat);
        sh.lo = h.lo; sh.hi = h.hi; sh.next = h.next; sh.dup = h.dup;
        fr.last_distinct = sh.next;
        fr.have_viol = false;
        sh.sl[0].launched = sh.sl[1].launched = false;
        sh.resume = true;
        sh.ck_ok = false;
        return MC_OK;
    }

    int fetch_state(uint64_t idx, uint64_t *words) {
        const uint64_t *src = d_arena + ((idx >> 6) * (uint64_t)W) * 64 + (idx & 63);
        HIP_TRY(hipMemcpy2D(words, sizeof(uint64_t), src, 64 * sizeof(uint64_t), sizeof(uint64_t), W, hipMemcpyDeviceToHost));
        return MC_OK;
    }
    int build_chain(std::vector<uint64_t> &chain) {
        chain.clear();
        if (!fr.have_viol) return MC_ESTATE;
        if (Viol(fr.last_viol).slot == SLOT_INIT) return MC_OK;
        return chain_to(viol_idx(fr.last_viol), chain);
    }
    int chain_to(uint64_t idx, std::vector<uint64_t> &chain) {
        chain.clear();
        if (!d_parent) { set_error("engine created without MC_F_TRACE"); return MC_ESTATE; }
        for (int guard = 0; guard < MC_MAX_LEVELS; ++guard) {
            chain.push_back(idx);
            uint32_t p;
            HIP_TRY(hipMemcpy(&p, d_parent + idx, sizeof p, hipMemcpyDeviceToHost));
            if (p == 0xffffffffu) break;
            idx = p;
        }
        std::vector<uint64_t> rev(chain.rbegin(), chain.rend());
        chain.swap(rev);
        return MC_OK;
    }
    int trace(uint8_t *states_out, int32_t *actions_out, size_t *n_inout) override {
        if (sim.trace_n) return sim_trace_out(states_out, actions_out, n_inout);
        if (!fr.have_viol) { *n_inout = 0; return MC_OK; }
        HIP_TRY(hipSetDevice(cfg.device));
        const Viol v(fr.last_viol);
        if (v.slot == SLOT_INIT) {
            std::vector<uint64_t> words(W);
            S::init(prm, viol_idx(fr.last_viol), WordRef{words.data(), 1});
            std::vector<int32_t> acts{-1};
            return trace_out(words, acts, states_out, actions_out, n_inout);
        }
        return chain_trace(viol_idx(fr.last_viol), v.extra_state(), v.slot, states_out, actions_out, n_inout);
    }
    int chain_trace(uint64_t end, bool extra, unsigned slot, uint8_t *states_out, int32_t *actions_out, size_t *n_inout) {
        std::vector<uint64_t> words, chain;
        std::vector<int32_t> acts;
        int rc = chain_to(end, chain);
        if (rc) return rc;
        words.resize(chain.size() * W);
        for (size_t k = 0; k < chain.size(); ++k) {
            if ((rc = fetch_state(chain[k], &words[k * W]))) return rc;
            if (k == 0) acts.push_back(-1);
            else {
                uint16_t ps;
                HIP_TRY(hipMemcpy(&ps, d_pslot + chain[k], sizeof ps, hipMemcpyDeviceToHost));
                acts.push_back(S::action_of(prm, &words[(k - 1) * W], (int)ps));
            }
        }
        if (extra) {
            std::vector<uint64_t> last(words.end() - W, words.end());
            words.resize(words.size() + W);
            S::apply(prm, CWordRef{last.data(), 1}, (int)slot, WordRef{&words[words.size() - W], 1});
            acts.push_back(S::action_of(prm, last.data(), (int)slot));
        }
        return trace_out(words, acts, states_out, actions_out, n_inout);
    }
    int trace_out(const std::vector<uint64_t> &words, const std::vector<int32_t> &acts, uint8_t *states_out, int32_t *actions_out, size_t *n_inout) {
        const size_t n = acts.size();
        if (n > *n_inout) { *n_inout = n; set_error("trace buffer too small"); return MC_EBADCFG; }
        if constexpr (HasExport<S>::value) {
            for (size_t k = 0; k < n; ++k) S::export_row(prm, &words[k * W], (uint64_t *)states_out + k * (size_t)S::EXPORT_WORDS);
        } else
        memcpy(states_out, words.data(), n * W * sizeof(uint64_t));
        memcpy(actions_out, acts.data(), n * sizeof(int32_t));
        *n_inout = n;
        return MC_OK;
    }
    int read_states(uint64_t first, uint64_t count, uint8_t *out) override {
        if (!count) return MC_OK;
        if (first + count > fr.last_distinct) { set_error("read_states: range beyond the states found by the last run"); return MC_EBADCFG; }
        HIP_TRY(hipSetDevice(cfg.device));
        DevBuf<uint64_t> tmp;
        const uint64_t piece = 1ull << 20;
        HIP_TRY(tmp.alloc((count < piece ? count : piece) * W));
        for (uint64_t off = 0; off < count; off += piece) {
            const uint64_t n = count - off < piece ? count - off : piece;
            hipLaunchKernelGGL(k_gather_states, dim3((unsigned)((n * W + 255) / 256)), dim3(256), 0, stream, d_arena, W, first + off, n, tmp);
            hipError_t e1, e2;
            if constexpr (HasExport<S>::value) {
                std::vector<uint64_t> rows((size_t)n * W);
                e1 = hipMemcpyAsync(rows.data(), tmp, n * W * sizeof(uint64_t), hipMemcpyDeviceToHost, stream);
                e2 = hipStreamSynchronize(stream);
                if (e1 == hipSuccess && e2 == hipSuccess)
                    for (uint64_t k = 0; k < n; ++k) S::export_row(prm, &rows[(size_t)k * W], (uint64_t *)out + (size_t)(off + k) * (size_t)S::EXPORT_WORDS);
            } else {
                e1 = hipMemcpyAsync(out + off * W * sizeof(uint64_t), tmp, n * W * sizeof(uint64_t), hipMemcpyDeviceToHost, stream);
                e2 = hipStreamSynchronize(stream);
            }
            if (e1 != hipSuccess || e2 != hipSuccess) { set_error("read_states: copy failed"); return MC_EHIP; }
        }
        return MC_OK;
    }
    int debug_flags(uint32_t set, uint32_t clear) override { cfg.flags = (cfg.flags & ~clear) | set; return MC_OK; }
    int seen_layout(uint64_t *buckets, uint32_t *slots) override {
        *buckets = seen_arg() & ~SEEN_SPARSE;
        *slots = seen_sparse ? MC_SPARSE_SLOTS : 8;
        return MC_OK;
    }
    int debug_phases(uint64_t *out48, int reset) override {
#ifdef MC_PHASE_PROF
        HIP_TRY(hipSetDevice(cfg.device));
        HIP_TRY(hipDeviceSynchronize());
        HIP_TRY(hipMemcpyFromSymbol(out48, HIP_SYMBOL(g_phase), 48 * sizeof(uint64_t)));
        if (reset) { static const unsigned long long zero[48] = {}; HIP_TRY(hipMemcpyToSymbol(HIP_SYMBOL(g_phase), zero, sizeof zero)); }
        return MC_OK;
#else
        (void)out48; (void)reset;
        set_error("the library was built without MC_PHASE_PROF");
        return MC_ESTATE;
#endif
    }
    int debug_reexpand(unsigned extra_flags, double *ms) override {
        HIP_TRY(hipSetDevice(cfg.device));
        Event a(hipEventDefault), b(hipEventDefault);
        HIP_TRY(hipEventRecord(a.get(), stream));
        for (uint64_t c0 = 0; c0 < fr.last_distinct; c0 += chunk) {
            const uint64_t c1 = c0 + chunk < fr.last_distinct ? c0 + chunk : fr.last_distinct;
            const uint64_t ncols = ((c1 - c0) + 63) & ~63ull;
            launch_expand<S, false>(!((cfg.flags | extra_flags) & MC_F_NOFAMILY), cfg.flags | extra_flags, ncols, stream, 0u, prm,
                                    (const uint64_t *)d_arena, c0, c1, ncols, d_table.p, seen_arg(), d_newlist.p, seg_cap, d_ctr.p,
                                    cfg.flags | extra_flags, RouteArgs{}, 0u);
            hipLaunchKernelGGL(k_commit, dim3(1), dim3(1), 0, stream, d_ctr, 0u);
        }
        HIP_TRY(hipEventRecord(b.get(), stream));
        HIP_TRY(hipStreamSynchronize(stream));
        float t = 0;
        HIP_TRY(hipEventElapsedTime(&t, a.get(), b.get()));
        *ms = t;
        return MC_OK;
    }
    int shard_alloc(ShSlot &q, uint64_t send_cap) {
        const unsigned P = nranks();
        if (send_cap > q.pend_src.n) {
            q.rt_fp.reset(); q.rt_src.reset(); q.pend_src.reset();
            q.rt_subcap = (send_cap / (P * NSHARD)) * 2 + 4096;
            HIP_TRY(q.rt_fp.alloc((size_t)P * NSHARD * q.rt_subcap));
            HIP_TRY(q.rt_src.alloc((size_t)P * NSHARD * q.rt_subcap));
            HIP_TRY(q.pend_src.alloc(send_cap));
        }
        HIP_TRY(q.rt_cur.reserve((size_t)(P * NSHARD)));
        if (send_cap > sh.d_incl.n) {
            sh.d_new_src.reset(); sh.d_incl.reset();
            HIP_TRY(sh.d_new_src.alloc(send_cap));
            HIP_TRY(sh.d_incl.alloc(send_cap));
        }
        HIP_TRY(sh.d_ends.reserve(8));
        HIP_TRY(sh.h_ends.reserve(8));
        HIP_TRY(sh.h_cur.reserve((size_t)8 * NSHARD));
        return MC_OK;
    }
    static int refuse_packed() {
        if constexpr (PackedRows<S>::value) { set_error("this engine of generated code stores rows packed to its program's cell ranges and serves ONE GPU: create a sharded engine with shard_count > 1 (or $TLAMC_JIT_PACK=0)"); return MC_EBADCFG; }
        return MC_OK;
    }
    void shard_reset_slots() {
        hipSetDevice(cfg.device);
        hipDeviceSynchronize();
        for (auto &q : sh.sl) { q.launched = false; q.keep_pending = false; q.pend_total = 0; q.moved = 0; q.count = 0; }
    }
    int shard_begin() override {
        int rc = refuse_packed();
        if (rc) return rc;
        if (nranks() > 8) { set_error("at most 8 shards"); return MC_EBADCFG; }
        sh.dup = 0;
        sh.resume = sh.ck_ok = false;
        shard_reset_slots();
        HIP_TRY(hipSetDevice(cfg.device));
        memset(kstat, 0, sizeof kstat);
        if ((rc = seed_init(cfg.shard_rank, cfg.shard_count, false, false, nullptr))) return rc;
        if ((rc = read_counters())) return rc;
        if ((rc = check_dev_error())) return rc;
        sh.lo = 0;
        sh.hi = sh.next = h_ctr->arena_next;
        fr.last_distinct = sh.next;
        return MC_OK;
    }
    int shard_begin_replicated(uint64_t min_frontier, uint64_t max_distinct, uint64_t max_levels, uint64_t *levels_out, uint32_t *nlevels) override {
        if (int rc = refuse_packed()) return rc;
        if (nranks() > 8) { set_error("at most 8 shards"); return MC_EBADCFG; }
        mc_result &res = *sh.prefix_res;
        sh.resume = sh.ck_ok = false;
        shard_reset_slots();
        const uint64_t saved_md = cfg.max_distinct, saved_ml = cfg.max_levels;
        cfg.max_distinct = max_distinct;
        cfg.max_levels = max_levels;
        fr.stop_frontier = min_frontier ? min_frontier : 1;
        const int rc = run(&res);
        fr.stop_frontier = 0;
        cfg.max_distinct = saved_md;
        cfg.max_levels = saved_ml;
        if (rc) return rc;
        const uint32_t cap = *nlevels;
        *nlevels = res.levels;
        for (uint32_t k = 0; k < res.levels && k < cap; k++) levels_out[k] = res.level_distinct[k];
        if (res.levels > cap) { set_error("shard_begin_replicated: level buffer too small"); return MC_EBADCFG; }
        const unsigned P = nranks(), r = cfg.shard_rank;
        const uint64_t lo = fr.lo, hi = fr.hi;
        const bool go_on = h_ctr->viol_key == ~0ull && hi > lo;
        if (go_on)
            hipLaunchKernelGGL(k_take_owned<S>, dim3((unsigned)((hi - lo + 255) / 256)), dim3(256), 0, stream, prm, d_arena, lo, hi, r, P, hi,
                               arena_cap, d_parent, d_pslot, d_ctr);
        hipLaunchKernelGGL(k_after_prefix, dim3(1), dim3(1), 0, stream, d_ctr, (unsigned long long)hi, r != 0 ? 1 : 0);
        int rc2 = read_counters();
        if (rc2) return rc2;
        if ((rc2 = check_dev_error())) return rc2;
        sh.lo = hi;
        sh.hi = sh.next = h_ctr->arena_next;
        sh.dup = r == 0 ? sh.hi - hi : sh.hi;
        fr.last_distinct = sh.next;
        return MC_OK;
    }
    int shard_level_size(uint64_t *n) override { *n = sh.hi - sh.lo; return MC_OK; }
    int shard_note_levels(const uint64_t *levels, uint32_t n, int32_t verdict) override {
        sh.levels.assign(levels, levels + n);
        sh.ck_ok = verdict == MC_V_OK || verdict == MC_V_BUDGET;
        return MC_OK;
    }
    int shard_resume(uint64_t *levels_out, uint32_t *nlevels) override {
        const uint32_t cap = *nlevels;
        *nlevels = 0;
        if (!sh.resume) return MC_OK;
        if (sh.levels.size() > cap) { set_error("shard_resume: level buffer too small"); return MC_EBADCFG; }
        for (size_t k = 0; k < sh.levels.size(); k++) levels_out[k] = sh.levels[k];
        *nlevels = (uint32_t)sh.levels.size();
        sh.resume = false;
        return MC_OK;
    }
    int shard_info(void **main_stream, uint64_t *chunk_states, int32_t *traced) override {
        HIP_TRY(hipSetDevice(cfg.device));
        if (main_stream) *main_stream = (void *)stream;
        if (chunk_states) *chunk_states = chunk;
        if (traced) *traced = d_parent.p != nullptr;
        return MC_OK;
    }
    size_t state_bytes() const override { return (size_t)W * 8; }
    hipStream_t side() const { return sh.ext_side ? sh.ext_stream : stream2; }
    void append_begin(hipStream_t s) { if (sh.ev_append.made()) hipStreamWaitEvent(s, sh.ev_append.get(), 0); }
    void append_end(hipStream_t s) { hipEventRecord(sh.ev_append.get(), s); }
    int side_done() {
        if (!sh.ext_side) HIP_TRY(hipStreamSynchronize(stream2));
        return MC_OK;
    }
    int shard_set_stream(void *hip_stream, int enable) override {
        HIP_TRY(hipSetDevice(cfg.device));
        HIP_TRY(hipStreamSynchronize(side()));
        sh.ext_stream = (hipStream_t)hip_stream;
        sh.ext_side = enable != 0;
        return MC_OK;
    }
    int materialise_local(unsigned slot) {
        const ShSlot &q = sh.sl[slot];
        append_begin(stream2);
        timed(2, 0, [&] {
            hipLaunchKernelGGL(k_materialise<S>, dim3(mat_grid(q.ncols), NSHARD), dim3(256), 0, stream2, prm, d_arena, q.chunk_base, d_newlist, seg_cap,
                               arena_cap, d_parent, d_pslot, d_ctr, slot, (const LevelCtl *)nullptr, (const uint64_t *)d_newfp);
        }, stream2);
        hipLaunchKernelGGL(k_commit, dim3(1), dim3(1), 0, stream2, d_ctr, slot);
        append_end(stream2);
        HIP_TRY(hipEventRecord(sh.ev_mat[slot].get(), stream2));
        return MC_OK;
    }
    int shard_expand_launch(unsigned slot, uint64_t first, uint64_t count, uint64_t send_cap) override {
        HIP_TRY(hipSetDevice(cfg.device));
        if (slot > 1) { set_error("shard_expand: slot must be 0 or 1"); return MC_EBADCFG; }
        ShSlot &q = sh.sl[slot];
        const unsigned P = nranks();
        int rc = shard_alloc(q, send_cap);
        if (rc) return rc;
        q.pend_total = 0;
        q.count = count;
        q.launched = true;
        for (unsigned t = 0; t <= 8; t++) q.pend_off.off[t] = 0;
        if (first + count > sh.hi - sh.lo) { set_error("shard_expand: chunk outside the local frontier"); return MC_EBADCFG; }
        if (count > chunk) { set_error("shard_expand: chunk larger than chunk_states"); return MC_EBADCFG; }
        if (!count) return MC_OK;
        if (sh.ev_slot[slot].made()) HIP_TRY(hipStreamWaitEvent(stream, sh.ev_slot[slot].get(), 0));
        if (sh.ev_mat[slot].made()) HIP_TRY(hipStreamWaitEvent(stream, sh.ev_mat[slot].get(), 0));
        HIP_TRY(hipMemsetAsync(q.rt_cur, 0, (size_t)(P * NSHARD) * sizeof(PaddedCounter), stream));
        const uint64_t c0 = sh.lo + first, c1 = c0 + count, base = c0 & ~63ull;
        const uint64_t ncols = ((c1 - base) + 63) & ~63ull;
        q.chunk_base = base;
        RouteArgs rt{P, q.rt_cur, q.rt_fp, q.rt_src, q.rt_subcap};
        rt.my_rank = cfg.shard_rank;
        rt.new_fp = d_newfp;
        q.ncols = ncols;
        timed(0, count, [&] {
            launch_expand<S, true>(!(cfg.flags & MC_F_NOFAMILY), cfg.flags, ncols, stream, 0u, prm,
                                   (const uint64_t *)d_arena, c0, c1, ncols, d_table.p, seen_arg(), d_newlist.p, seg_cap, d_ctr.p, cfg.flags, rt, slot);
        });
        return MC_OK;
    }
    int shard_expand_finish(unsigned slot, uint64_t *send_fp, uint64_t send_cap, uint64_t *send_counts) override {
        HIP_TRY(hipSetDevice(cfg.device));
        if (slot > 1 || !sh.sl[slot].launched) { set_error("shard_expand_finish: no expand in flight for this slot"); return MC_EBADCFG; }
        ShSlot &q = sh.sl[slot];
        q.launched = false;
        const unsigned P = nranks();
        for (unsigned t = 0; t < P; t++) send_counts[t] = 0;
        if (!q.count) return MC_OK;
        PaddedCounter *cur = sh.h_cur;
        HIP_TRY(hipMemcpyAsync(cur, q.rt_cur, (size_t)(P * NSHARD) * sizeof(PaddedCounter), hipMemcpyDeviceToHost, stream));
        HIP_TRY(hipMemcpyAsync(h_ctr, d_ctr, sizeof(DevCounters), hipMemcpyDeviceToHost, stream));
        HIP_TRY(hipStreamSynchronize(stream));
        int rc;
        if ((rc = check_dev_error())) return rc;
        uint64_t total = 0;
        for (unsigned t = 0; t < P; t++) {
            q.pend_off.off[t] = total;
            for (unsigned x = 0; x < NSHARD; x++) {
                if (cur[t * NSHARD + x].v > q.rt_subcap) { set_error("shard_expand: route bucket overflow (raise send_cap)"); return MC_EROUTE; }
                send_counts[t] += cur[t * NSHARD + x].v;
            }
            total += send_counts[t];
        }
        for (unsigned t = P; t <= 8; t++) q.pend_off.off[t] = total;
        if (total >= (1ull << 31)) { set_error("shard_expand: more than 2^31 candidates in one round (lower chunk_states)"); return MC_EARENA; }
        if (total > q.pend_src.n) { set_error("shard_expand: more candidates in one round than the slot's pending list holds (raise the fan-out allowance)"); return MC_EROUTE; }
        if (total > send_cap) { set_error("shard_expand: send buffer too small (raise the fan-out allowance)"); return MC_EROUTE; }
        q.pend_total = total;
        if (q.keep_pending) {
            HIP_TRY(hipStreamWaitEvent(side(), sh.ev_keep[slot].get(), 0));
            q.keep_pending = false;
        }
        if ((rc = materialise_local(slot))) return rc;
        if (total) {
            RouteArgs rt{P, q.rt_cur, q.rt_fp, q.rt_src, q.rt_subcap};
            hipLaunchKernelGGL(k_compact_buckets, dim3(64, P * NSHARD), dim3(256), 0, side(), rt, send_fp, q.pend_src);
        }
        HIP_TRY(hipEventRecord(sh.ev_slot[slot].get(), side()));
        return side_done();
    }
    int shard_probe(const uint64_t *recv_fp, uint64_t n, uint8_t *answers) override {
        HIP_TRY(hipSetDevice(cfg.device));
        if (!n) return MC_OK;
        timed(1, n, [&] {
            hipLaunchKernelGGL(k_probe, dim3((unsigned)((n + 255) / 256)), dim3(256), 0, side(), recv_fp, n, d_table, seen_arg(), answers, d_ctr);
        }, side());
        return side_done();
    }
    int shard_expand_pack(unsigned slot, uint64_t *send_fp, uint64_t cap) override {
        HIP_TRY(hipSetDevice(cfg.device));
        if (slot > 1 || !sh.sl[slot].launched) { set_error("shard_expand_pack: no expand in flight for this slot"); return MC_EBADCFG; }
        ShSlot &q = sh.sl[slot];
        q.launched = false;
        const unsigned P = nranks();
        if (cap < 2 || (uint64_t)P * cap > q.pend_src.n || (uint64_t)P * cap >= (1ull << 31)) { set_error("shard_expand_pack: capacity does not fit the slot's buffers"); return MC_EBADCFG; }
        q.pend_total = (uint64_t)P * cap;
        for (unsigned t = 0; t <= 8; t++) q.pend_off.off[t] = (t < P ? t : P) * cap;
        HIP_TRY(hipEventRecord(sh.ev_exp[slot].get(), stream));
        if (q.keep_pending) {
            HIP_TRY(hipStreamWaitEvent(stream, sh.ev_keep[slot].get(), 0));
            q.keep_pending = false;
        }
        if (q.count) {
            HIP_TRY(hipStreamWaitEvent(stream2, sh.ev_exp[slot].get(), 0));
            const int rc = materialise_local(slot);
            if (rc) return rc;
            RouteArgs rt{P, q.rt_cur, q.rt_fp, q.rt_src, q.rt_subcap};
            hipLaunchKernelGGL(k_compact_packed, dim3(64, P * NSHARD), dim3(256), 0, stream, rt, cap, send_fp, q.pend_src, d_ctr);
        } else {
            for (unsigned t = 0; t < P; t++) HIP_TRY(hipMemsetAsync(send_fp + (uint64_t)t * cap, 0, sizeof(uint64_t), stream));
        }
        HIP_TRY(hipEventRecord(sh.ev_slot[slot].get(), stream));
        if (!sh.ext_side) HIP_TRY(hipStreamSynchronize(stream));
        return side_done();
    }
    int shard_probe_pack(const uint64_t *recv_fp, uint64_t cap, uint8_t *answers) override {
        HIP_TRY(hipSetDevice(cfg.device));
        const uint64_t total = (uint64_t)nranks() * cap;
        if (!total) return MC_OK;
        timed(1, total, [&] {
            hipLaunchKernelGGL(k_probe_packed, dim3((unsigned)(nranks() * ((cap + 255) / 256))), dim3(256), 0, side(), recv_fp, cap, nranks(), d_table,
                               seen_arg(), answers, d_ctr);
        }, side());
        return side_done();
    }
    int shard_keep_pack(unsigned slot, const uint8_t *answers_back, uint64_t cap) override {
        if (slot > 1 || sh.sl[slot].pend_total != (uint64_t)nranks() * cap) { set_error("shard_keep_pack: not the capacity the slot was packed with"); return MC_EBADCFG; }
        return shard_keep(slot, answers_back, nullptr);
    }
    int shard_wait_keep(unsigned slot) override {
        if (slot > 1) return MC_EBADCFG;
        HIP_TRY(hipSetDevice(cfg.device));
        if (sh.sl[slot].keep_pending) HIP_TRY(hipStreamWaitEvent(side(), sh.ev_keep[slot].get(), 0));
        return MC_OK;
    }
    int shard_materialise(unsigned slot, const uint8_t *answers_back, uint8_t *send_states, uint64_t send_cap, uint64_t *send_counts) override {
        HIP_TRY(hipSetDevice(cfg.device));
        if (slot > 1) return MC_EBADCFG;
        ShSlot &q = sh.sl[slot];
        const unsigned P = nranks();
        for (unsigned t = 0; t < P; t++) send_counts[t] = 0;
        q.moved = 0;
        if (!q.pend_total) return MC_OK;
        const unsigned bx = (unsigned)((q.pend_total + 255) / 256);
        int rc = scan_answers_inclusive(answers_back, sh.d_incl.p, q.pend_total, sh.d_scan_tmp, side());
        if (rc) return rc;
        hipLaunchKernelGGL(k_gather_range_ends, dim3(1), dim3(64), 0, side(), sh.d_incl, q.pend_off, P, sh.d_ends);
        unsigned long long *ends = sh.h_ends;
        HIP_TRY(hipMemcpyAsync(ends, sh.d_ends, P * sizeof(unsigned long long), hipMemcpyDeviceToHost, side()));
        HIP_TRY(hipStreamSynchronize(side()));
        OwnerOffsets start;
        std::vector<PaddedCounter> cnt(P);
        for (unsigned t = 0; t <= 8; t++) start.off[t] = 0;
        for (unsigned t = 0; t < P; t++) {
            start.off[t] = t ? ends[t - 1] : 0;
            cnt[t].v = ends[t] - start.off[t];
        }
        hipLaunchKernelGGL(k_compact_new, dim3(bx), dim3(256), 0, side(), answers_back, sh.d_incl, q.pend_src, q.pend_total, q.pend_off, start, P,
                           sh.d_new_src);
        BlockPlan plan;
        uint64_t blocks = 0;
        for (unsigned t = 0; t < 8; t++) {
            plan.blk_off[t] = blocks;
            plan.cnt[t] = t < P ? cnt[t].v : 0;
            if (t < P) { send_counts[t] = cnt[t].v; blocks += (cnt[t].v + 63) / 64; }
        }
        plan.blk_off[8] = blocks;
        for (unsigned t = P; t < 8; t++) plan.blk_off[t] = blocks;
        q.plan = plan;
        q.moved = 0;
        for (unsigned t = 0; t < P; t++) q.moved += plan.cnt[t];
        if (blocks * 64 > send_cap) { set_error("shard_materialise: state send buffer too small"); return MC_EARENA; }
        if (blocks) {
            timed(2, blocks * 64, [&] {
                hipLaunchKernelGGL(k_send_materialise<S>, dim3((unsigned)((blocks * 64 + 255) / 256)), dim3(256), 0, side(), prm, d_arena,
                                   q.chunk_base, sh.d_new_src, q.pend_off, plan, P, (uint64_t *)send_states);
            }, side());
        }
        return side_done();
    }
    int shard_keep(unsigned slot, const uint8_t *answers_back, uint64_t *n_new) override {
        HIP_TRY(hipSetDevice(cfg.device));
        if (n_new) *n_new = 0;
        if (slot > 1) return MC_EBADCFG;
        ShSlot &q = sh.sl[slot];
        if (!q.pend_total) return MC_OK;
        const unsigned bx = (unsigned)((q.pend_total + 255) / 256);
        hipStream_t ks = stream2;
        if (sh.ext_side) {
            HIP_TRY(hipEventRecord(sh.ev_ans.get(), sh.ext_stream));
            HIP_TRY(hipStreamWaitEvent(ks, sh.ev_ans.get(), 0));
        }
        int rc = scan_answers_inclusive(answers_back, sh.d_incl.p, q.pend_total, sh.d_scan_tmp, ks);
        if (rc) return rc;
        append_begin(ks);
        const uint32_t *d_total = sh.d_incl + (q.pend_total - 1);
        OwnerOffsets one, zero;
        for (unsigned t = 0; t <= 8; t++) { one.off[t] = t ? q.pend_total : 0; zero.off[t] = 0; }
        hipLaunchKernelGGL(k_compact_new, dim3(bx), dim3(256), 0, ks, answers_back, sh.d_incl, q.pend_src, q.pend_total, one, zero, 1u, sh.d_new_src);
        timed(2, 0, [&] {
            hipLaunchKernelGGL(k_materialise_list<S>, dim3(bx), dim3(256), 0, ks, prm, d_arena, q.chunk_base, sh.d_new_src, d_total, arena_cap,
                               d_parent, d_pslot, d_ctr);
        }, ks);
        hipLaunchKernelGGL(k_bump_arena_next, dim3(1), dim3(1), 0, ks, d_ctr, d_total, 0ull, (unsigned long long)arena_cap);
        append_end(ks);
        HIP_TRY(hipEventRecord(sh.ev_keep[slot].get(), ks));
        q.keep_pending = true;
        if (!sh.ext_side) {
            uint32_t total32 = 0;
            HIP_TRY(hipMemcpyAsync(&total32, d_total, sizeof total32, hipMemcpyDeviceToHost, ks));
            HIP_TRY(hipStreamSynchronize(ks));
            if (n_new) *n_new = total32;
        }
        return MC_OK;
    }
    int shard_ingest(const uint8_t *recv_states, uint64_t n) override {
        HIP_TRY(hipSetDevice(cfg.device));
        if (!n) return MC_OK;
        append_begin(side());
        hipLaunchKernelGGL(k_ingest, dim3((unsigned)((n + 255) / 256)), dim3(256), 0, side(), d_arena, W, (const uint64_t *)recv_states, n,
                           arena_cap, d_parent, d_ctr);
        hipLaunchKernelGGL(k_bump_arena_next, dim3(1), dim3(1), 0, side(), d_ctr, (const uint32_t *)nullptr, (unsigned long long)n,
                           (unsigned long long)arena_cap);
        append_end(side());
        return side_done();
    }
    int shard_materialise_parents(unsigned slot, uint64_t *send_parents) override {
        HIP_TRY(hipSetDevice(cfg.device));
        if (slot > 1) return MC_EBADCFG;
        ShSlot &q = sh.sl[slot];
        if (!q.moved) return MC_OK;
        hipLaunchKernelGGL(k_send_parents, dim3((unsigned)((q.moved + 255) / 256)), dim3(256), 0, side(), (const uint32_t *)sh.d_new_src, q.chunk_base,
                           q.pend_off, q.plan, nranks(), send_parents);
        return side_done();
    }
    int shard_ingest_parents(const uint64_t *recv_parents, uint64_t n, unsigned src_rank) override {
        HIP_TRY(hipSetDevice(cfg.device));
        if (!n || !d_prank) return MC_OK;
        hipLaunchKernelGGL(k_ingest_parents, dim3((unsigned)((n + 255) / 256)), dim3(256), 0, side(), recv_parents, n, src_rank, d_parent, d_pslot,
                           d_prank, (const DevCounters *)d_ctr);
        return side_done();
    }
    int shard_violation(int32_t *found, uint64_t *idx, uint32_t *slot, int32_t *verdict, int32_t *invariant) override {
        HIP_TRY(hipSetDevice(cfg.device));
        HIP_TRY(hipStreamSynchronize(side()));
        int rc = read_counters();
        if (rc) return rc;
        *found = h_ctr->viol_key != ~0ull;
        *idx = 0; *slot = 0; *verdict = MC_V_OK; *invariant = -1;
        if (*found) {
            const Viol v(h_ctr->viol_key);
            *idx = viol_idx(h_ctr->viol_key);
            *slot = v.slot;
            *verdict = v.verdict;
            *invariant = v.invariant;
        }
        return MC_OK;
    }
    int shard_fetch(uint64_t idx, uint8_t *state_out, uint32_t *parent_rank, uint64_t *parent_idx, uint32_t *parent_slot) override {
        HIP_TRY(hipSetDevice(cfg.device));
        if (idx & (1ull << 63)) {
            const uint64_t ord = idx & ~(1ull << 63);
            if (ord >= S::num_init(prm)) return MC_EBADCFG;
            S::init(prm, ord, WordRef{(uint64_t *)state_out, 1});
            *parent_rank = cfg.shard_rank;
            *parent_idx = 0xffffffffull;
            *parent_slot = SLOT_INIT;
            return MC_OK;
        }
        if (!d_parent) { set_error("engine created without MC_F_TRACE"); return MC_ESTATE; }
        if (idx >= arena_cap) return MC_EBADCFG;
        HIP_TRY(hipDeviceSynchronize());
        int rc = fetch_state(idx, (uint64_t *)state_out);
        if (rc) return rc;
        uint32_t p = 0;
        uint16_t ps = 0;
        uint8_t pr = 0xff;
        HIP_TRY(hipMemcpy(&p, d_parent + idx, sizeof p, hipMemcpyDeviceToHost));
        HIP_TRY(hipMemcpy(&ps, d_pslot + idx, sizeof ps, hipMemcpyDeviceToHost));
        if (d_prank) HIP_TRY(hipMemcpy(&pr, d_prank + idx, sizeof pr, hipMemcpyDeviceToHost));
        *parent_rank = pr == 0xff ? cfg.shard_rank : pr;
        *parent_idx = p;
        *parent_slot = ps;
        return MC_OK;
    }
    int shard_end_level(uint64_t *new_local) override {
        HIP_TRY(hipSetDevice(cfg.device));
        if (sh.sl[0].launched || sh.sl[1].launched) { set_error("shard_end_level: an expand is still in flight"); return MC_EBADCFG; }
        HIP_TRY(hipStreamSynchronize(side()));
        HIP_TRY(hipStreamSynchronize(stream2));
        int rc = read_counters();
        if (rc) return rc;
        if ((rc = check_dev_error())) return rc;
        sh.next = h_ctr->arena_next;
        fr.last_distinct = sh.next;
        sh.lo = sh.hi;
        sh.hi = sh.next;
        *new_local = sh.hi - sh.lo;
        return MC_OK;
    }
    int check_frontier(uint64_t lo, uint64_t hi) {
        if constexpr (ChecksOnExpand<S>::value) {
            if (hi > lo) {
                hipLaunchKernelGGL(k_check_frontier<S>, dim3((unsigned)((hi - lo + 255) / 256)), dim3(256), 0, stream, prm,
                                   (const uint64_t *)d_arena, lo, hi, d_ctr);
                return read_counters();
            }
        }
        return MC_OK;
    }
    int shard_check_frontier() override {
        HIP_TRY(hipSetDevice(cfg.device));
        HIP_TRY(hipStreamSynchronize(side()));
        HIP_TRY(hipStreamSynchronize(stream2));
        return check_frontier(sh.lo, sh.hi);
    }
    int shard_counters(uint64_t *generated, uint64_t *distinct_local, int32_t *verdict) override {
        HIP_TRY(hipSetDevice(cfg.device));
        HIP_TRY(hipStreamSynchronize(side()));
        int rc = read_counters();
        if (rc) return rc;
        if ((rc = check_dev_error())) return rc;
        *generated = 0;
        for (int t = 0; t < NSHARD; t++) *generated += h_ctr->generated[t].v;
        *distinct_local = h_ctr->arena_next - sh.dup;
        *verdict = h_ctr->viol_key != ~0ull ? Viol(h_ctr->viol_key).verdict : MC_V_OK;
        return MC_OK;
    }
    static constexpr uint64_t SIM_ROUND = 1ull << 18;
    static constexpr uint32_t SIM_ITERS = 16;
    static constexpr uint64_t SIM_MAX_WALKS = 1ull << 40;
    int sim_round(SimArgs a, uint64_t n, SimCounters &c, uint64_t walks_before, bool allow_stop, uint64_t rounds_done, bool *complete) {
        a.n = n;
        a.ncols = (n + 63) & ~63ull;
        *complete = false;
        HIP_TRY(hipMemsetAsync(sim.wst, 0, n * sizeof(uint32_t), stream));
        const unsigned blocks = (unsigned)((a.ncols + 255) / 256);
        const uint64_t launches = ((uint64_t)a.depth + 1 + SIM_ITERS - 1) / SIM_ITERS;
        for (uint64_t l = 0; l < launches; ++l) {
            hipLaunchKernelGGL(k_simulate<S>, dim3(blocks), dim3(256), 0, stream, prm, a);
            HIP_TRY(hipGetLastError());
            HIP_TRY(hipMemcpyAsync(&c, sim.ctr, sizeof c, hipMemcpyDeviceToHost, stream));
            HIP_TRY(hipStreamSynchronize(stream));
            if (c.error) break;
            if (allow_stop) report_progress((uint32_t)rounds_done, c.generated, c.steps, c.walks);
            if (c.walks - walks_before >= n) { *complete = true; break; }
            if (allow_stop && stop_requested) break;
        }
        return MC_OK;
    }
    int simulate(const mc_sim_opts *o, mc_sim_result *out) override {
        memset(out, 0, sizeof *out);
        out->violated_invariant = -1;
        if (!o || o->depth < 1 || o->depth > MC_SIM_MAX_DEPTH || (o->record && (!o->record_slots || !o->record_len || !o->record_end))) {
            set_error("simulate: depth must be 1 .. MC_SIM_MAX_DEPTH, and a record request needs its three arrays");
            return MC_EBADCFG;
        }
        if (o->num > SIM_MAX_WALKS) { set_error("simulate: at most 2^40 walks"); return MC_EBADCFG; }
        if (cfg.shard_count > 1) { set_error("simulate: not available for a sharded engine"); return MC_EBADCFG; }
        fr.have_run = fr.have_viol = false;
        ck.pending = ck.in_place = false;
        stop_requested = false;
        gr.release();
        sim.trace_n = 0;
        sim.trace_rows.clear();
        sim.trace_acts.clear();
        HIP_TRY(hipSetDevice(cfg.device));
        const uint64_t lanes = ((o->num && o->num < SIM_ROUND ? o->num : SIM_ROUND) + 63) & ~63ull;
        HIP_TRY(sim.buf[0].reserve(lanes * W));
        HIP_TRY(sim.buf[1].reserve(lanes * W));
        HIP_TRY(sim.wst.reserve(lanes));
        HIP_TRY(sim.ctr.reserve(1));
        int rc;
        const uint64_t K = o->record;
        DevBuf<int32_t> d_rslots, d_tslots;
        DevBuf<uint32_t> d_rlen, d_tlen;
        DevBuf<uint64_t> d_rows;
        if (K) {
            HIP_TRY(d_rslots.alloc(K * o->depth));
            HIP_TRY(d_rlen.alloc(2 * K));
            HIP_TRY(hipMemsetAsync(d_rslots, 0xff, K * o->depth * sizeof(int32_t), stream));
            HIP_TRY(hipMemsetAsync(d_rlen, 0, 2 * K * sizeof(uint32_t), stream));
        }
        SimCounters c;
        memset(&c, 0, sizeof c);
        c.viol = ~0ull;
        HIP_TRY(hipMemcpyAsync(sim.ctr, &c, sizeof c, hipMemcpyHostToDevice, stream));
        SimArgs a{};
        a.seed = o->seed;
        a.buf0 = sim.buf[0];
        a.buf1 = sim.buf[1];
        a.wst = sim.wst;
        a.depth = o->depth;
        a.iters = SIM_ITERS;
        a.deadlock = (cfg.flags & MC_F_DEADLOCK) ? 1u : 0u;
        a.ctr = sim.ctr;
        a.rec_first = 0;
        a.rec_count = K;
        a.rec_slots = d_rslots;
        a.rec_len = d_rlen;
        a.rec_end = d_rlen ? d_rlen + K : nullptr;
        const auto t0 = std::chrono::steady_clock::now();
        progress_last = t0;
        bool stopped = false;
        uint64_t rounds = 0;
        for (uint64_t first = 0; !o->num || first < o->num; first += SIM_ROUND, ++rounds) {
            if (first >= SIM_MAX_WALKS) { stopped = true; break; }
            const uint64_t n = o->num && o->num - first < SIM_ROUND ? o->num - first : SIM_ROUND;
            a.w0 = first;
            const uint64_t before = c.walks;
            bool complete = false;
            if ((rc = sim_round(a, n, c, before, true, rounds, &complete))) return rc;
            if (c.error & DEV_EOVERFLOW) { set_error("packed-state capacity exceeded (raft messages / elections / allLogs slots, or a PlusCal sequence longer than its cells, or a recursive PlusCal procedure deeper than $TLAMC_PCAL_STACK frames)"); return MC_EOVERFLOW; }
            if (!complete) { stopped = true; c.viol = ~0ull; break; }
            if (c.viol != ~0ull) break;
            if (stop_requested) { stopped = true; break; }
        }
        out->seconds = std::chrono::duration<double>(std::chrono::steady_clock::now() - t0).count();
        out->walks = c.walks;
        out->steps = c.steps;
        out->generated = c.generated;
        out->max_depth = c.max_depth;
        out->verdict = stopped ? MC_V_BUDGET : MC_V_OK;
        if (K) {
            HIP_TRY(hipMemcpy(o->record_slots, d_rslots, K * o->depth * sizeof(int32_t), hipMemcpyDeviceToHost));
            HIP_TRY(hipMemcpy(o->record_len, d_rlen, K * sizeof(uint32_t), hipMemcpyDeviceToHost));
            HIP_TRY(hipMemcpy(o->record_end, d_rlen + K, K * sizeof(uint32_t), hipMemcpyDeviceToHost));
        }
        if (c.viol == ~0ull) return MC_OK;
        const unsigned long long key = c.viol;
        const unsigned kind = sim_key_kind(key), vslot = sim_key_slot(key);
        out->verdict = verdict_of_kind(kind);
        if (kind == SIM_VK_INVARIANT) out->violated_invariant = (int)sim_key_inv(key);
        out->violating_walk = sim_key_walk(key);
        HIP_TRY(d_tslots.alloc((size_t)o->depth));
        HIP_TRY(d_tlen.alloc(2));
        HIP_TRY(d_rows.alloc(((size_t)o->depth + 1) * W));
        HIP_TRY(hipMemsetAsync(d_tslots, 0xff, (size_t)o->depth * sizeof(int32_t), stream));
        SimCounters c2;
        memset(&c2, 0, sizeof c2);
        c2.viol = ~0ull;
        HIP_TRY(hipMemcpyAsync(sim.ctr, &c2, sizeof c2, hipMemcpyHostToDevice, stream));
        a.w0 = out->violating_walk;
        a.rec_first = out->violating_walk;
        a.rec_count = 1;
        a.rec_slots = d_tslots;
        a.rec_len = d_tlen;
        a.rec_end = d_tlen + 1;
        a.rec_rows = d_rows;
        bool complete = false;
        if ((rc = sim_round(a, 1, c2, 0, false, 0, &complete))) return rc;
        uint32_t len = 0;
        HIP_TRY(hipMemcpy(&len, d_tlen, sizeof len, hipMemcpyDeviceToHost));
        if (c2.viol != key || len < 1 || len > o->depth) { set_error("simulate: the violating walk did not repeat in record mode"); return MC_ESTATE; }
        const bool extra = kind == SIM_VK_INVARIANT && vslot < SIM_SLOT_PARENT;
        const size_t n = len + (extra ? 1u : 0u);
        std::vector<int32_t> slots(len > 1 ? len - 1 : 1);
        sim.trace_rows.resize(n * W);
        HIP_TRY(hipMemcpy(sim.trace_rows.data(), d_rows, n * W * sizeof(uint64_t), hipMemcpyDeviceToHost));
        if (len > 1) HIP_TRY(hipMemcpy(slots.data(), d_tslots, (len - 1) * sizeof(int32_t), hipMemcpyDeviceToHost));
        sim.trace_acts.assign(1, -1);
        for (size_t k = 1; k < len; ++k) sim.trace_acts.push_back(S::action_of(prm, &sim.trace_rows[(k - 1) * W], slots[k - 1]));
        if (extra) sim.trace_acts.push_back(S::action_of(prm, &sim.trace_rows[(size_t)(len - 1) * W], (int)vslot));
        sim.trace_n = n;
        out->trace_len = (uint32_t)n;
        return MC_OK;
    }
    int sim_trace_out(uint8_t *states_out, int32_t *actions_out, size_t *n_inout) {
        const size_t n = sim.trace_n;
        if (n > *n_inout) { *n_inout = n; set_error("trace buffer too small"); return MC_EBADCFG; }
        if constexpr (HasExport<S>::value) {
            for (size_t k = 0; k < n; ++k) S::export_row(prm, &sim.trace_rows[k * W], (uint64_t *)states_out + k * (size_t)S::EXPORT_WORDS);
        } else
        memcpy(states_out, sim.trace_rows.data(), n * W * sizeof(uint64_t));
        memcpy(actions_out, sim.trace_acts.data(), n * sizeof(int32_t));
        *n_inout = n;
        return MC_OK;
    }
    static constexpr uint32_t BEH_ITERS = 16;
    const mc_spec_desc *spec_desc() const override { return &desc; }
    int behaviours_refused() override {
        if (cfg.shard_count > 1) { set_error("behaviours: not available for a sharded engine (shard_count > 1)"); return MC_EBADCFG; }
        if (PackedRows<S>::value || HasExport<S>::value) {
            set_error("behaviours: not available for an MC_F_JIT engine: generated code packs its rows, and there is no import_row that turns an observation "
                      "in the interpreter's layout into one (create the engine without MC_F_JIT)");
            return MC_EBADCFG;
        }
        if (S::num_init(prm) > MC_BEH_MAX_INIT) { set_error("behaviours: the model has more than 65536 initial states"); return MC_EBADCFG; }
        return MC_OK;
    }
    int behaviours(const mc_beh_opts *o, mc_beh_verdict *out, mc_beh_result *res) override {
        memset(res, 0, sizeof *res);
        res->first_rejected = ~0ull;
        if (int rc = behaviours_refused()) return rc;
        if constexpr (PackedRows<S>::value || HasExport<S>::value) return MC_EBADCFG;
        else {
        if (o->count && (!o->first || !o->rows || !out)) { set_error("behaviours: first, rows and the verdict array are needed"); return MC_EBADCFG; }
        for (uint64_t b = 0; b < o->count; ++b)
            if (o->first[b + 1] <= o->first[b] || o->first[b + 1] - o->first[b] >= (1ull << 31)) {
                set_error("behaviours: behaviour " + std::to_string(b) + " is empty (T = 0), or longer than 2^31 - 1 observations");
                return MC_EBADCFG;
            }
        if (!o->count) return MC_OK;
        HIP_TRY(hipSetDevice(cfg.device));
        struct Drain { hipStream_t s; ~Drain() { (void)hipStreamSynchronize(s); } } drain{stream};
        const uint32_t iters = o->iters ? o->iters : BEH_ITERS;
        const uint64_t R = chunk / 64 < o->count ? chunk / 64 : o->count;
        std::vector<uint64_t> hmask(W, ~0ull);
        if (o->mask) memcpy(hmask.data(), o->mask, (size_t)W * sizeof(uint64_t));
        const bool full = beh_mask_full(hmask.data(), W);
        for (int k = 0; k < 2; ++k) HIP_TRY(beh.set[k].reserve(R * 64 * W));
        HIP_TRY(beh.stage.reserve(R * 64 * W));
        HIP_TRY(beh.first.reserve(R + 1));
        HIP_TRY(beh.carry.reserve(R));
        HIP_TRY(beh.out.reserve(R));
        HIP_TRY(beh.ctr.reserve(1));
        BehCounters c;
        memset(&c, 0, sizeof c);
        c.first_rejected = ~0ull;
        HIP_TRY(hipMemcpyAsync(beh.ctr, &c, sizeof c, hipMemcpyHostToDevice, stream));
        if (!full) {
            HIP_TRY(beh.mask.reserve(W));
            HIP_TRY(hipMemcpyAsync(beh.mask, hmask.data(), (size_t)W * sizeof(uint64_t), hipMemcpyHostToDevice, stream));
        }
        BehArgs a{};
        a.mask = full ? nullptr : (const uint64_t *)beh.mask;
        a.flags = o->flags;
        a.iters = iters;
        a.ctr = beh.ctr;
        const size_t lds = ((size_t)2 * W + MC_BEH_MAX_CANDIDATES) * sizeof(uint64_t);
        std::vector<uint64_t> rel(R + 1);
        const auto t0 = std::chrono::steady_clock::now();
        for (uint64_t b0 = 0; b0 < o->count; b0 += R) {
            const uint64_t n = o->count - b0 < R ? o->count - b0 : R;
            const uint64_t r0 = o->first[b0], nrows = o->first[b0 + n] - r0;
            uint64_t longest = 0;
            for (uint64_t k = 0; k <= n; ++k) rel[k] = o->first[b0 + k] - r0;
            for (uint64_t k = 0; k < n; ++k) longest = std::max(longest, rel[k + 1] - rel[k]);
            HIP_TRY(beh.rows.reserve(nrows * W));
            HIP_TRY(hipMemcpyAsync(beh.rows, o->rows + r0 * W * sizeof(uint64_t), nrows * W * sizeof(uint64_t), hipMemcpyHostToDevice, stream));
            HIP_TRY(hipMemcpyAsync(beh.first, rel.data(), (n + 1) * sizeof(uint64_t), hipMemcpyHostToDevice, stream));
            HIP_TRY(hipMemsetAsync(beh.carry, 0, n * sizeof(uint64_t), stream));
            HIP_TRY(hipMemsetAsync(beh.out, 0, n * sizeof(mc_beh_verdict), stream));
            a.b0 = b0;
            a.n = n;
            a.first = beh.first;
            a.rows = beh.rows;
            a.set0 = beh.set[0];
            a.set1 = beh.set[1];
            a.stage = beh.stage;
            a.carry = beh.carry;
            a.out = beh.out;
            for (uint64_t l = 0; l < (longest + iters - 1) / iters; ++l) {
                hipLaunchKernelGGL(k_behaviours<S>, dim3((unsigned)n), dim3(64), lds, stream, prm, a);
                HIP_TRY(hipGetLastError());
            }
            HIP_TRY(hipMemcpyAsync(out + b0, beh.out, n * sizeof(mc_beh_verdict), hipMemcpyDeviceToHost, stream));
            HIP_TRY(hipStreamSynchronize(stream));
        }
        HIP_TRY(hipMemcpy(&c, beh.ctr, sizeof c, hipMemcpyDeviceToHost));
        res->seconds = std::chrono::duration<double>(std::chrono::steady_clock::now() - t0).count();
        res->accepted = c.accepted;
        res->rejected = c.rejected;
        res->ambiguous = c.ambiguous;
        res->observations = c.observations;
        res->generated = c.generated;
        res->first_rejected = c.first_rejected;
        if (c.accepted + c.rejected + c.ambiguous != o->count) { set_error("behaviours: a behaviour was left undecided"); return MC_ESTATE; }
        return MC_OK;
        }
    }
    int kernel_stats(mc_kernel_stats *o) override {
        o->expand = kstat[0];
        o->insert = kstat[1];
        o->materialise = kstat[2];
        o->state_bytes = (uint64_t)W * 8;
        o->cand_cells = fr.cells;
        o->inwave_states = fr.inwave;
        return MC_OK;
    }
};

}

namespace mc {
static int spec_group(const mc_spec_desc *d) {
    if (!d) return 0;
    switch (d->spec_id) {
    case MC_SPEC_ATOMIC_ADD: case MC_SPEC_PCAL_INTRO: return 1;
    case MC_SPEC_RAFT: return d->nparams < 1 ? 0 : d->params[0] == 2 ? 2 : d->params[0] == 3 ? 3 : d->params[0] == 5 ? 4 : 0;
    case MC_SPEC_SSI: return 5;
    case MC_SPEC_PCAL: return 6;
    case MC_SPEC_PAXOS: return 7;
    default: return 0;
    }
}
template <class S>
static int make_engine(const typename S::Params &prm, const mc_spec_desc *spec, const mc_config *cfg, EngineBase **out) {
    auto *e = new Engine<S>();
    e->prm = prm;
    e->desc = *spec;
    e->cfg = *cfg;
    const int r = e->alloc();
    if (r) { delete e; return r; }
    *out = e;
    return MC_OK;
}
}
extern "C" {
int mc_make_engine_1(const mc_spec_desc *, const mc_config *, mc::EngineBase **);
int mc_make_engine_2(const mc_spec_desc *, const mc_config *, mc::EngineBase **);
int mc_make_engine_3(const mc_spec_desc *, const mc_config *, mc::EngineBase **);
int mc_make_engine_4(const mc_spec_desc *, const mc_config *, mc::EngineBase **);
int mc_make_engine_5(const mc_spec_desc *, const mc_config *, mc::EngineBase **);
int mc_make_engine_6(const mc_spec_desc *, const mc_config *, mc::EngineBase **);
int mc_make_engine_7(const mc_spec_desc *, const mc_config *, mc::EngineBase **);
void *mc_jit_factory_opts(const void *program, int pack);
#if MC_TU == 1 || MC_TU == -1
int mc_make_engine_1(const mc_spec_desc *d, const mc_config *c, mc::EngineBase **out) {
    if (d->spec_id == MC_SPEC_ATOMIC_ADD) {
        mc::SpecAtomicAdd::Params p;
        if (mc::SpecAtomicAdd::make_params(d->params, d->nparams, p)) return MC_EBADCFG;
        return mc::make_engine<mc::SpecAtomicAdd>(p, d, c, out);
    }
    mc::SpecPcalIntro::Params p;
    if (mc::SpecPcalIntro::make_params(d->params, d->nparams, p)) return MC_EBADCFG;
    return mc::make_engine<mc::SpecPcalIntro>(p, d, c, out);
}
#endif
#define MC_RAFT_FACTORY(K, SPEC)                                                                   \
    int mc_make_engine_##K(const mc_spec_desc *d, const mc_config *c, mc::EngineBase **out) {      \
        mc::RaftParams p;                                                                          \
        if (mc::SPEC::make_params(d->params, d->nparams, p)) return MC_EBADCFG;                    \
        return mc::make_engine<mc::SPEC>(p, d, c, out);                                            \
    }
#if MC_TU == 2 || MC_TU == -1
MC_RAFT_FACTORY(2, SpecRaft2)
#endif
#if MC_TU == 3 || MC_TU == -1
MC_RAFT_FACTORY(3, SpecRaft3)
#endif
#if MC_TU == 4 || MC_TU == -1
MC_RAFT_FACTORY(4, SpecRaft5)
#endif
#if MC_TU == 5 || MC_TU == -1
int mc_make_engine_5(const mc_spec_desc *d, const mc_config *c, mc::EngineBase **out) {
    mc::SsiParams p;
    if (mc::SpecSsi::make_params(d->params, d->nparams, p)) return MC_EBADCFG;
    return mc::make_engine<mc::SpecSsi>(p, d, c, out);
}
#endif
#if MC_TU == 7 || MC_TU == -1
int mc_make_engine_7(const mc_spec_desc *d, const mc_config *c, mc::EngineBase **out) {
    mc::PaxosParams p;
    if (mc::SpecPaxos::make_params(d->params, d->nparams, p)) return MC_EBADCFG;
    return mc::make_engine<mc::SpecPaxos>(p, d, c, out);
}
#endif
#if MC_TU == 6 || MC_TU == -1
int mc_make_engine_6(const mc_spec_desc *d, const mc_config *c, mc::EngineBase **out) {
    mc::VmParams p;
    if (mc::vm_make_params(d->params, d->nparams, p)) return MC_EBADCFG;
    if (hipSetDevice(c->device) != hipSuccess) { mc::set_error("hipSetDevice failed"); return MC_EHIP; }
    mc::DevBuf<int32_t> d_code;
    const size_t image_words = (size_t)p.code_len + (size_t)mc::vm_ext_words(p);
    if (d_code.alloc(image_words) != hipSuccess ||
        hipMemcpy(d_code, p.code, image_words * sizeof(int32_t), hipMemcpyHostToDevice) != hipSuccess) {
        mc::set_error("cannot upload the PlusCal program image");
        return MC_EHIP;
    }
    uint64_t ph = 0xcbf29ce484222325ull;
    auto mixin = [&](uint64_t v) { ph = (ph ^ v) * 0x100000001b3ull; ph ^= ph >> 29; };
    for (int i = 0; i < p.code_len; i++) mixin((uint32_t)p.code[i]);
    for (int v : {p.nv, p.words, p.ninst, p.maxch, p.pc_base, p.done, p.init_entry, p.ninv, p.ncon, p.label_tab, p.self_tab, p.code_len}) mixin((uint32_t)v);
    for (int i = 0; i < 8; i++) mixin((uint32_t)p.inv_entry[i]);
    mixin(p.num_init);
    if (p.code[p.code_len + mc::VMX_NACON] || p.code[p.code_len + mc::VMX_NVIEW])
        for (int i = 0; i < mc::vm_ext_words(p); i++) mixin((uint32_t)p.code[p.code_len + i]);
    p.code = d_code;
    const int rc = p.nv <= 16 ? mc::make_engine<mc::SpecVmCfg16>(p, d, c, out)
                 : p.nv <= 32 ? mc::make_engine<mc::SpecVmCfg32>(p, d, c, out)
                 : p.nv <= 64 ? mc::make_engine<mc::SpecVmCfg64>(p, d, c, out) : mc::make_engine<mc::SpecVmCfg>(p, d, c, out);
    if (!rc) { (*out)->owned_device_blob = std::move(d_code); (*out)->program_hash = ph ? ph : 1; }
    return rc;
}
#endif
#if MC_TU == 9
}
#include MC_GEN_HEADER
extern "C" {
int mc_make_engine_gen(const mc_spec_desc *d, const mc_config *c, mc::EngineBase **out) {
    mc::VmParams p;
    if (mc::SpecGen::make_params(d->params, d->nparams, p)) { mc::set_error("jit: the generated engine was built from another program"); return MC_EBADCFG; }
    uint64_t ph = 0xcbf29ce484222325ull;
    auto mixin = [&](uint64_t v) { ph = (ph ^ v) * 0x100000001b3ull; ph ^= ph >> 29; };
    for (int i = 0; i < p.code_len; i++) mixin((uint32_t)p.code[i]);
    for (int v : {p.nv, p.words, p.ninst, p.maxch, p.pc_base, p.done, p.init_entry, p.ninv, p.ncon, p.label_tab, p.self_tab, p.code_len}) mixin((uint32_t)v);
    for (int i = 0; i < 8; i++) mixin((uint32_t)p.inv_entry[i]);
    mixin(p.num_init);
    if (p.code[p.code_len + mc::VMX_NACON] || p.code[p.code_len + mc::VMX_NVIEW])
        for (int i = 0; i < mc::vm_ext_words(p); i++) mixin((uint32_t)p.code[p.code_len + i]);
    p.code = nullptr;
    const int rc = mc::make_engine<mc::SpecGen>(p, d, c, out);
    if (mc::SpecGen::PACKED_ROWS) { mixin(0x7061636bu); mixin((uint32_t)mc::SpecGen::MAX_WORDS); }
    if (!rc) (*out)->program_hash = ph ? ph : 1;
    return rc;
}
#endif
}

#if MC_TU == 0 || MC_TU == -1
static thread_local std::string g_last_error;
using namespace mc;

struct mc_engine {
    EngineBase *impl;
};

extern "C" {

int mc_device_count(void) {
    int n = 0;
    if (hipGetDeviceCount(&n) != hipSuccess) return 0;
    return n;
}

int mc_engine_create(const mc_spec_desc *spec, const mc_config *cfg, mc_engine **out) {
    if (!spec || !cfg || !out) return MC_EBADCFG;
    *out = nullptr;
    if (mc_device_count() <= 0) { set_error("no HIP device: libtlamc has no CPU fallback"); return MC_EHIP; }
    g_last_error.clear();
    mc_config with_trace;
    if (cfg->flags & MC_F_COVERAGE) {
        if (cfg->shard_count > 1) { set_error("MC_F_COVERAGE: not available for a sharded engine (shard_count > 1)"); return MC_EBADCFG; }
        with_trace = *cfg;
        with_trace.flags |= MC_F_TRACE;
        cfg = &with_trace;
    }
    if (cfg->flags & MC_F_CONTINUE) {
        if (cfg->shard_count > 1) { set_error("MC_F_CONTINUE: not available for a sharded engine (shard_count > 1)"); return MC_EBADCFG; }
        with_trace = *cfg;
        with_trace.flags |= MC_F_TRACE;
        cfg = &with_trace;
    }
    EngineBase *impl = nullptr;
    const int group = spec_group(spec);
    int rc = MC_EBADCFG;
    switch (group) {
    case 1: rc = mc_make_engine_1(spec, cfg, &impl); break;
    case 2: rc = mc_make_engine_2(spec, cfg, &impl); break;
    case 3: rc = mc_make_engine_3(spec, cfg, &impl); break;
    case 4: rc = mc_make_engine_4(spec, cfg, &impl); break;
    case 5: rc = mc_make_engine_5(spec, cfg, &impl); break;
    case 6: {
        const char *ej = getenv("TLAMC_JIT");
        rc = MC_EBADCFG;
        bool jit = false;
        if (((cfg->flags & MC_F_JIT) || (ej && *ej && *ej != '0')) && spec->nparams >= 1 && spec->params[0]) {
            typedef int (*factory_t)(const mc_spec_desc *, const mc_config *, EngineBase **);
            factory_t fn = (factory_t)mc_jit_factory_opts((const void *)(intptr_t)spec->params[0], cfg->shard_count > 1 ? 0 : 1);
            if (fn) { rc = fn(spec, cfg, &impl); jit = true; }
            else fprintf(stderr, "tlamc: MC_F_JIT: %s; interpreting the program on the device instead\n", g_last_error.c_str());
        }
        if (!jit) rc = mc_make_engine_6(spec, cfg, &impl);
        break;
    }
    case 7: rc = mc_make_engine_7(spec, cfg, &impl); break;
    default: break;
    }
    if (rc == MC_OK) *out = new mc_engine{impl};
    else if (rc == MC_EBADCFG && g_last_error.empty()) set_error("unknown spec id or constants out of range");
    return rc;
}
int mc_engine_run(mc_engine *e, mc_result *out) { return e && out ? e->impl->run(out) : MC_EBADCFG; }
int mc_engine_step(mc_engine *e, uint32_t levels, mc_result *out) { return e && out ? e->impl->step(levels, out) : MC_EBADCFG; }
int mc_engine_set_progress(mc_engine *e, mc_progress_fn fn, void *user, double min_interval_seconds) {
    if (!e) return MC_EBADCFG;
    e->impl->progress_fn = fn;
    e->impl->progress_user = user;
    e->impl->progress_interval = min_interval_seconds > 0 ? min_interval_seconds : 0.0;
    return MC_OK;
}
int mc_engine_request_stop(mc_engine *e) {
    if (!e) return MC_EBADCFG;
    e->impl->stop_requested = true;
    return MC_OK;
}
int mc_engine_trace(mc_engine *e, uint8_t *states_out, int32_t *actions_out, size_t *n_inout) {
    return e && n_inout ? e->impl->trace(states_out, actions_out, n_inout) : MC_EBADCFG;
}
int mc_engine_behaviours(mc_engine *e, const mc_beh_opts *opts, mc_beh_verdict *out, mc_beh_result *result) {
    return e && opts && result ? e->impl->behaviours(opts, out, result) : MC_EBADCFG;
}
int mc_engine_behaviour_witness(mc_engine *e, const mc_beh_opts *opts, uint64_t b, uint8_t *states_out, int32_t *slots_out, size_t *n_inout) {
    if (!e || !opts || !n_inout || !opts->first || !opts->rows || b >= opts->count || opts->first[b + 1] <= opts->first[b]) {
        mc_set_error_internal("behaviour_witness: no such behaviour");
        return MC_EBADCFG;
    }
    if (int rc = e->impl->behaviours_refused()) return rc;
    return dispatch_spec(e->impl->spec_desc(), [&](auto s, const auto &prm) {
        using S = decltype(s);
        const size_t W = (size_t)S::words(prm);
        const uint64_t T = opts->first[b + 1] - opts->first[b];
        std::vector<uint64_t> rows(T * W), mask(W);
        memcpy(rows.data(), opts->rows + opts->first[b] * W * sizeof(uint64_t), T * W * sizeof(uint64_t));
        if (opts->mask) memcpy(mask.data(), opts->mask, W * sizeof(uint64_t));
        mc_beh_verdict v;
        BehSets sets;
        beh_check<S>(prm, rows.data(), T, opts->mask ? mask.data() : nullptr, opts->flags, &v, &sets);
        const size_t n = sets.sets.size();
        if (n > *n_inout) { *n_inout = n; mc_set_error_internal("behaviour_witness: buffers too small"); return MC_EBADCFG; }
        *n_inout = n;
        if (!n) return MC_OK;
        if (!states_out || !slots_out) { mc_set_error_internal("behaviour_witness: states_out and slots_out are needed"); return MC_EBADCFG; }
        std::vector<uint64_t> path(n * W);
        beh_witness(sets, (int)W, path.data(), slots_out);
        memcpy(states_out, path.data(), n * W * sizeof(uint64_t));
        return MC_OK;
    });
}
int mc_engine_simulate(mc_engine *e, const mc_sim_opts *opts, mc_sim_result *out) {
    return e && opts && out ? e->impl->simulate(opts, out) : MC_EBADCFG;
}
int mc_engine_coverage(mc_engine *e, mc_action_coverage *out, size_t *n_inout) { return e && n_inout ? e->impl->coverage(out, n_inout) : MC_EBADCFG; }
int mc_engine_violations(mc_engine *e, mc_violations_info *info, mc_violation *out, size_t *n_inout) {
    return e && n_inout ? e->impl->violations(info, out, n_inout) : MC_EBADCFG;
}
int mc_engine_violation_trace(mc_engine *e, size_t k, uint8_t *states_out, int32_t *actions_out, size_t *n_inout) {
    return e && n_inout ? e->impl->violation_trace(k, states_out, actions_out, n_inout) : MC_EBADCFG;
}
int mc_engine_graph(mc_engine *e, mc_graph_info *out) { return e && out ? e->impl->graph(out) : MC_EBADCFG; }
int mc_engine_graph_read(mc_engine *e, uint64_t first, uint64_t count, uint64_t *offsets_out, uint32_t *dst_out, int32_t *action_out, size_t *nedges_inout) {
    return e && nedges_inout ? e->impl->graph_read(first, count, offsets_out, dst_out, action_out, nedges_inout) : MC_EBADCFG;
}
int mc_engine_scc(mc_engine *e, mc_scc_info *out) { return e && out ? e->impl->scc(out) : MC_EBADCFG; }
int mc_engine_scc_read(mc_engine *e, uint64_t first, uint64_t count, uint32_t *scc_out) {
    return e && (scc_out || !count) ? e->impl->scc_read(first, count, scc_out) : MC_EBADCFG;
}
int mc_engine_predicates(mc_engine *e, uint64_t first, uint64_t count, uint32_t *bits_out) {
    return e && (bits_out || !count) ? e->impl->predicates(first, count, bits_out) : MC_EBADCFG;
}
static LiveQuery live_query_procs(const char *call, uint64_t weak, uint64_t strong, const mc_live_property *prop, bool refine) {
    return LiveQuery{call, 0, weak, strong, nullptr, prop ? prop->kind : -1, prop ? prop->p : -1, prop ? prop->q : -1, refine};
}
int mc_engine_liveness(mc_engine *e, uint64_t weak_fair_mask, mc_live_info *out) {
    return e && out ? e->impl->liveness_run(live_query_procs("mc_engine_liveness", weak_fair_mask, 0, nullptr, false), nullptr, out, nullptr, nullptr) : MC_EBADCFG;
}
int mc_engine_liveness_check(mc_engine *e, uint64_t weak_fair_mask, const mc_live_property *prop, mc_live_check_info *out) {
    return e && prop && out ? e->impl->liveness_run(live_query_procs("mc_engine_liveness_check", weak_fair_mask, 0, prop, false), prop, nullptr, out, nullptr) : MC_EBADCFG;
}
int mc_engine_liveness_strong(mc_engine *e, uint64_t weak_mask, uint64_t strong_mask, mc_live_info *out, mc_live_strong_info *strong_out) {
    return e && out && strong_out ? e->impl->liveness_run(live_query_procs("mc_engine_liveness_strong", weak_mask, strong_mask, nullptr, true), nullptr, out, nullptr, strong_out)
                                  : MC_EBADCFG;
}
int mc_engine_liveness_check_strong(mc_engine *e, uint64_t weak_mask, uint64_t strong_mask, const mc_live_property *prop, mc_live_check_info *out,
                                    mc_live_strong_info *strong_out) {
    return e && prop && out && strong_out
               ? e->impl->liveness_run(live_query_procs("mc_engine_liveness_check_strong", weak_mask, strong_mask, prop, true), prop, nullptr, out, strong_out)
               : MC_EBADCFG;
}
int mc_engine_liveness_units(mc_engine *e, const mc_fair_units *fu, mc_live_info *out, mc_live_strong_info *strong_out) {
    return e && fu && out && strong_out ? e->impl->liveness_run(live_query_units("mc_engine_liveness_units", fu, -1, -1, -1), nullptr, out, nullptr, strong_out) : MC_EBADCFG;
}
int mc_engine_liveness_check_units(mc_engine *e, const mc_fair_units *fu, const mc_live_property *prop, mc_live_check_info *out,
                                   mc_live_strong_info *strong_out) {
    return e && fu && prop && out && strong_out
               ? e->impl->liveness_run(live_query_units("mc_engine_liveness_check_units", fu, prop->kind, prop->p, prop->q), prop, nullptr, out, strong_out)
               : MC_EBADCFG;
}
int mc_engine_liveness_edge_units(mc_engine *e, uint64_t first_edge, uint64_t count, int8_t *unit_out) {
    return e && (unit_out || !count) ? e->impl->liveness_edge_units(first_edge, count, unit_out) : MC_EBADCFG;
}
int mc_engine_liveness_components(mc_engine *e, uint64_t first, uint64_t count, uint32_t *scc_out) {
    return e && (scc_out || !count) ? e->impl->liveness_components(first, count, scc_out) : MC_EBADCFG;
}
int mc_engine_liveness_trace(mc_engine *e, uint32_t *prefix_out, size_t *nprefix_inout, uint32_t *cycle_out, size_t *ncycle_inout) {
    return e && nprefix_inout && ncycle_inout ? e->impl->liveness_trace(prefix_out, nprefix_inout, cycle_out, ncycle_inout) : MC_EBADCFG;
}
int mc_engine_kernel_stats(mc_engine *e, mc_kernel_stats *out) { return e && out ? e->impl->kernel_stats(out) : MC_EBADCFG; }
int mc_engine_read_states(mc_engine *e, uint64_t first, uint64_t count, uint8_t *out) {
    return e && (out || !count) ? e->impl->read_states(first, count, out) : MC_EBADCFG;
}
int mc_engine_checkpoint(mc_engine *e, const char *path) { return e && path ? e->impl->checkpoint(path) : MC_EBADCFG; }
int mc_engine_restore(mc_engine *e, const char *path) { return e && path ? e->impl->restore(path) : MC_EBADCFG; }
void mc_engine_destroy(mc_engine *e) {
    if (!e) return;
    delete e->impl;
    delete e;
}

size_t mc_state_bytes(const mc_spec_desc *spec) {
    size_t n = 0;
    dispatch_spec(spec, [&](auto s, const auto &prm) { n = sizeof(uint64_t) * decltype(s)::words(prm); return 0; });
    return n;
}
uint32_t mc_fp_owner(uint64_t fp, uint32_t shard_count) { return fp_owner(fp, shard_count); }
int mc_state_format(const mc_spec_desc *spec, const uint8_t *state, char *buf, size_t cap) {
    if (!state || !buf || !cap) return MC_EBADCFG;
    int n = MC_EBADCFG;
    int rc = dispatch_spec(spec, [&](auto s, const auto &prm) {
        using S = decltype(s);
        uint64_t w[S::MAX_WORDS];
        memcpy(w, state, sizeof(uint64_t) * S::words(prm));
        n = S::format(prm, w, buf, cap);
        if ((size_t)n < cap) buf[n] = 0; else buf[cap - 1] = 0;
        return 0;
    });
    return rc ? rc : n;
}
int mc_state_action(const mc_spec_desc *spec, const uint8_t *state, int32_t slot) {
    if (!state) return MC_EBADCFG;
    int a = -1;
    int rc = dispatch_spec(spec, [&](auto s, const auto &prm) {
        using S = decltype(s);
        uint64_t w[S::MAX_WORDS];
        memcpy(w, state, sizeof(uint64_t) * S::words(prm));
        a = S::action_of(prm, w, (int)slot);
        return 0;
    });
    return rc ? rc : a;
}
int mc_state_apply(const mc_spec_desc *spec, const uint8_t *state, int32_t slot, uint8_t *successor_out) {
    if (!state || !successor_out) return MC_EBADCFG;
    return dispatch_spec(spec, [&](auto s, const auto &prm) {
        using S = decltype(s);
        uint64_t w[S::MAX_WORDS], o[S::MAX_WORDS];
        memcpy(w, state, sizeof(uint64_t) * S::words(prm));
        S::apply(prm, CWordRef{w, 1}, (int)slot, WordRef{o, 1});
        memcpy(successor_out, o, sizeof(uint64_t) * S::words(prm));
        return 0;
    });
}
const char *mc_action_name(const mc_spec_desc *spec, int32_t action) {
    const char *nm = "?";
    dispatch_spec(spec, [&](auto s, const auto &prm) {
        if constexpr (std::is_same_v<std::decay_t<decltype(prm)>, VmParams>) nm = vm_action_name(prm.host, action);
        else nm = decltype(s)::action_name(action);
        return 0;
    });
    return nm;
}
const char *mc_strerror(int code) {
    switch (code) {
    case MC_OK: return "ok";
    case MC_EBADCFG: return "bad spec or configuration";
    case MC_EHIP: return "HIP error / no device";
    case MC_EOVERFLOW: return "packed-state slot array overflow";
    case MC_ETABLEFULL: return "seen-set full";
    case MC_EARENA: return "state arena full";
    case MC_ERCCL: return "exchange failure";
    case MC_ESTATE: return "call sequence error";
    case MC_EPARSE: return "parse error";
    case MC_ENOSPEC: return "module is not a lowered spec";
    case MC_EROUTE: return "exchange bucket full";
    default: return "unknown error";
    }
}
const char *mc_last_error(void) { return g_last_error.c_str(); }
void mc_set_error_internal(const char *msg) { g_last_error = msg ? msg : ""; }


int mc_engine_debug_reexpand(mc_engine *e, unsigned extra_flags, double *ms) { return e && ms ? e->impl->debug_reexpand(extra_flags, ms) : MC_EBADCFG; }
int mc_engine_debug_phases(mc_engine *e, uint64_t *out48, int reset) { return e && out48 ? e->impl->debug_phases(out48, reset) : MC_EBADCFG; }
int mc_engine_debug_flags(mc_engine *e, uint32_t set, uint32_t clear) { return e ? e->impl->debug_flags(set, clear) : MC_EBADCFG; }
int mc_engine_seen_layout(mc_engine *e, uint64_t *buckets, uint32_t *slots) { return e && buckets && slots ? e->impl->seen_layout(buckets, slots) : MC_EBADCFG; }
int mc_shard_begin(mc_engine *e) { return e ? e->impl->shard_begin() : MC_EBADCFG; }
int mc_shard_begin_replicated(mc_engine *e, uint64_t min_frontier, uint64_t max_distinct, uint64_t max_levels, uint64_t *levels_out,
                              uint32_t *nlevels) {
    return e && levels_out && nlevels ? e->impl->shard_begin_replicated(min_frontier, max_distinct, max_levels, levels_out, nlevels) : MC_EBADCFG;
}
int mc_shard_level_size(mc_engine *e, uint64_t *n) { return e && n ? e->impl->shard_level_size(n) : MC_EBADCFG; }
int mc_shard_info(mc_engine *e, void **main_stream_out, uint64_t *chunk_states_out, int32_t *traced_out) {
    return e ? e->impl->shard_info(main_stream_out, chunk_states_out, traced_out) : MC_EBADCFG;
}
size_t mc_engine_state_bytes_internal(mc_engine *e) { return e ? e->impl->state_bytes() : 0; }
int mc_shard_expand(mc_engine *e, uint64_t first, uint64_t count, uint64_t *send_fp, uint64_t send_cap, uint64_t *send_counts) {
    if (!e || !send_counts) return MC_EBADCFG;
    const int rc = e->impl->shard_expand_launch(0, first, count, send_cap);
    return rc ? rc : e->impl->shard_expand_finish(0, send_fp, send_cap, send_counts);
}
int mc_shard_set_stream(mc_engine *e, void *hip_stream, int enable) { return e ? e->impl->shard_set_stream(hip_stream, enable) : MC_EBADCFG; }
int mc_shard_expand_launch(mc_engine *e, uint32_t slot, uint64_t first, uint64_t count, uint64_t send_cap) {
    return e ? e->impl->shard_expand_launch(slot, first, count, send_cap) : MC_EBADCFG;
}
int mc_shard_expand_finish(mc_engine *e, uint32_t slot, uint64_t *send_fp, uint64_t send_cap, uint64_t *send_counts) {
    return e && send_counts ? e->impl->shard_expand_finish(slot, send_fp, send_cap, send_counts) : MC_EBADCFG;
}
int mc_shard_probe(mc_engine *e, const uint64_t *recv_fp, uint64_t n, uint8_t *answers) {
    return e ? e->impl->shard_probe(recv_fp, n, answers) : MC_EBADCFG;
}
int mc_shard_materialise(mc_engine *e, const uint8_t *answers_back, uint8_t *send_states, uint64_t send_cap, uint64_t *send_counts) {
    return e && send_counts ? e->impl->shard_materialise(0, answers_back, send_states, send_cap, send_counts) : MC_EBADCFG;
}
int mc_shard_materialise_slot(mc_engine *e, uint32_t slot, const uint8_t *answers_back, uint8_t *send_states, uint64_t send_cap,
                              uint64_t *send_counts) {
    return e && send_counts ? e->impl->shard_materialise(slot, answers_back, send_states, send_cap, send_counts) : MC_EBADCFG;
}
int mc_shard_ingest(mc_engine *e, const uint8_t *recv_states, uint64_t n) { return e ? e->impl->shard_ingest(recv_states, n) : MC_EBADCFG; }
int mc_shard_expand_pack(mc_engine *e, uint32_t slot, uint64_t *send_fp, uint64_t cap) { return e && send_fp ? e->impl->shard_expand_pack(slot, send_fp, cap) : MC_EBADCFG; }
int mc_shard_probe_pack(mc_engine *e, const uint64_t *recv_fp, uint64_t cap, uint8_t *answers) {
    return e && recv_fp && answers ? e->impl->shard_probe_pack(recv_fp, cap, answers) : MC_EBADCFG;
}
int mc_shard_keep_pack(mc_engine *e, uint32_t slot, const uint8_t *answers_back, uint64_t cap) {
    return e && answers_back ? e->impl->shard_keep_pack(slot, answers_back, cap) : MC_EBADCFG;
}
int mc_shard_wait_keep(mc_engine *e, uint32_t slot) { return e ? e->impl->shard_wait_keep(slot) : MC_EBADCFG; }
int mc_shard_keep(mc_engine *e, const uint8_t *answers_back, uint64_t *n_new) { return e && n_new ? e->impl->shard_keep(0, answers_back, n_new) : MC_EBADCFG; }
int mc_shard_keep_slot(mc_engine *e, uint32_t slot, const uint8_t *answers_back, uint64_t *n_new) {
    return e ? e->impl->shard_keep(slot, answers_back, n_new) : MC_EBADCFG;
}
int mc_shard_end_level(mc_engine *e, uint64_t *new_local) { return e && new_local ? e->impl->shard_end_level(new_local) : MC_EBADCFG; }
int mc_shard_counters(mc_engine *e, uint64_t *generated, uint64_t *distinct_local, int32_t *verdict) {
    return e && generated && distinct_local && verdict ? e->impl->shard_counters(generated, distinct_local, verdict) : MC_EBADCFG;
}
int mc_shard_check_frontier(mc_engine *e) { return e ? e->impl->shard_check_frontier() : MC_EBADCFG; }
int mc_shard_materialise_parents(mc_engine *e, uint32_t slot, uint64_t *send_parents) { return e ? e->impl->shard_materialise_parents(slot, send_parents) : MC_EBADCFG; }
int mc_shard_ingest_parents(mc_engine *e, const uint64_t *recv_parents, uint64_t n, uint32_t src_rank) {
    return e ? e->impl->shard_ingest_parents(recv_parents, n, src_rank) : MC_EBADCFG;
}
int mc_shard_violation(mc_engine *e, int32_t *found, uint64_t *idx, uint32_t *slot, int32_t *verdict, int32_t *invariant) {
    return e && found && idx && slot && verdict && invariant ? e->impl->shard_violation(found, idx, slot, verdict, invariant) : MC_EBADCFG;
}
int mc_shard_note_levels(mc_engine *e, const uint64_t *levels, uint32_t n, int32_t verdict) { return e && (levels || !n) ? e->impl->shard_note_levels(levels, n, verdict) : MC_EBADCFG; }
int mc_shard_resume(mc_engine *e, uint64_t *levels_out, uint32_t *nlevels) { return e && levels_out && nlevels ? e->impl->shard_resume(levels_out, nlevels) : MC_EBADCFG; }
int mc_shard_checkpoint(mc_engine *e, const char *path) { return e && path ? e->impl->shard_checkpoint(path) : MC_EBADCFG; }
int mc_shard_restore(mc_engine *e, const char *path) { return e && path ? e->impl->shard_restore(path) : MC_EBADCFG; }
int mc_shard_fetch(mc_engine *e, uint64_t idx, uint8_t *state_out, uint32_t *parent_rank, uint64_t *parent_idx, uint32_t *parent_slot) {
    return e && state_out && parent_rank && parent_idx && parent_slot ? e->impl->shard_fetch(idx, state_out, parent_rank, parent_idx, parent_slot) : MC_EBADCFG;
}

}
#endif
```

### tla_rust_amd/csrc/spec_registry.h

```cpp
#pragma once
#include "../../include/tlamc.h"
#include "spec_paxos.h"
#include "spec_pluscal.h"
#include "spec_raft.h"
#include "spec_ssi.h"
#include "spec_vm.h"
#include "spec_vm_cfg.h"

namespace mc {

using SpecRaft2 = SpecRaft<2>;
using SpecRaft3 = SpecRaft<3>;
using SpecRaft5 = SpecRaft<5>;

template <class F>
int dispatch_spec(const mc_spec_desc *d, F &&f) {
    if (!d || d->nparams > 16) return MC_EBADCFG;
    switch (d->spec_id) {
    case MC_SPEC_ATOMIC_ADD: {
        SpecAtomicAdd::Params p;
        if (SpecAtomicAdd::make_params(d->params, d->nparams, p)) return MC_EBADCFG;
        return f(SpecAtomicAdd{}, p);
    }
    case MC_SPEC_PCAL_INTRO: {
        SpecPcalIntro::Params p;
        if (SpecPcalIntro::make_params(d->params, d->nparams, p)) return MC_EBADCFG;
        return f(SpecPcalIntro{}, p);
    }
    case MC_SPEC_RAFT: {
        RaftParams p;
        if (d->nparams < 5) return MC_EBADCFG;
        switch (d->params[0]) {
        case 2: if (SpecRaft2::make_params(d->params, d->nparams, p)) return MC_EBADCFG; return f(SpecRaft2{}, p);
        case 3: if (SpecRaft3::make_params(d->params, d->nparams, p)) return MC_EBADCFG; return f(SpecRaft3{}, p);
        case 5: if (SpecRaft5::make_params(d->params, d->nparams, p)) return MC_EBADCFG; return f(SpecRaft5{}, p);
        default: return MC_EBADCFG;
        }
    }
    case MC_SPEC_SSI: {
        SsiParams p;
        if (SpecSsi::make_params(d->params, d->nparams, p)) return MC_EBADCFG;
        return f(SpecSsi{}, p);
    }
    case MC_SPEC_PAXOS: {
        PaxosParams p;
        if (SpecPaxos::make_params(d->params, d->nparams, p)) return MC_EBADCFG;
        return f(SpecPaxos{}, p);
    }
    case MC_SPEC_PCAL: {
        VmParams p;
        if (vm_make_params(d->params, d->nparams, p)) return MC_EBADCFG;
        if (p.nv <= 16) return f(SpecVmCfg16{}, p);
        if (p.nv <= 32) return f(SpecVmCfg32{}, p);
        if (p.nv <= 64) return f(SpecVmCfg64{}, p);
        return f(SpecVmCfg{}, p);
    }
    default: return MC_EBADCFG;
    }
}

}
```

### tla_rust_amd/csrc/violations.h

```cpp
#pragma once
#include "mc_common.h"
#include "spec_registry.h"
#include "spec_gen.h"

namespace mc {

constexpr int VIOL_MAX_INV = 32;
constexpr int VIOL_BIN_DEADLOCK = 32, VIOL_BIN_FATAL = 33, VIOL_BINS = 34;

template <class S, class = void>
struct ViolChecksStored { static constexpr bool value = false; };
template <class S>
struct ViolChecksStored<S, decltype((void)S::CHECK_ON_EXPAND)> { static constexpr bool value = true; };

template <class S>
struct ViolModel;
template <> struct ViolModel<SpecAtomicAdd> { MC_HD static int ninv(const SpecAtomicAdd::Params &) { return 0; } };
template <> struct ViolModel<SpecPcalIntro> { MC_HD static int ninv(const SpecPcalIntro::Params &) { return 1; } };
template <int N> struct ViolModel<SpecRaft<N>> { MC_HD static int ninv(const RaftParams &) { return 2; } };
template <> struct ViolModel<SpecSsi> { MC_HD static int ninv(const SsiParams &) { return 8; } };
template <> struct ViolModel<SpecPaxos> { MC_HD static int ninv(const PaxosParams &p) { return p.kind == 1 ? 1 : 4; } };
template <int MAXV> struct ViolModel<SpecVmT<MAXV>> { MC_HD static int ninv(const VmParams &p) { return p.ninv; } };
template <int MAXV> struct ViolModel<SpecVmCfgT<MAXV>> : ViolModel<SpecVmT<MAXV>> {};
template <class G> struct ViolModel<SpecGenT<G>> { MC_HD static int ninv(const VmParams &) { return G::NINV; } };

enum : unsigned { VIOL_P_NONE = 0, VIOL_P_OUTSIDE = 1 , VIOL_P_FATAL = 2  };
struct ViolPair { unsigned what, bin, kind, inv; bool flagged;  };
template <class S>
MC_HD ViolPair viol_pair(unsigned st) {
    ViolPair r{VIOL_P_NONE, 0u, 0u, 0u, false};
    if (!(st & ST_ENABLED) || (st & ST_OVERFLOW)) return r;
    r.flagged = (st & (ST_ASSERT | ST_SPECERR | ST_INVARIANT)) != 0;
    if (st & ST_ASSERT) { r.what = VIOL_P_FATAL; r.bin = VIOL_BIN_FATAL; r.kind = 2u; return r; }
    if (st & ST_SPECERR) { r.what = VIOL_P_FATAL; r.bin = VIOL_BIN_FATAL; r.kind = 4u; return r; }
    if (!(st & ST_INVARIANT)) return r;
    r.bin = r.inv = (st >> 8) & 31u;
    r.kind = 1u;
    if (st & ST_OUT_OF_MODEL) { r.what = VIOL_P_OUTSIDE; return r; }
    if (ViolChecksStored<S>::value && !(st & ST_SELFLOOP)) { r.what = VIOL_P_FATAL; r.bin = VIOL_BIN_FATAL; }
    return r;
}
template <class S>
MC_HD ViolPair viol_pair(unsigned st, int ninv) {
    ViolPair r = viol_pair<S>(st);
    if (!ViolChecksStored<S>::value && r.kind == 1u && (int)r.inv >= ninv) { r.what = VIOL_P_FATAL; r.bin = VIOL_BIN_FATAL; }
    return r;
}
MC_HD bool viol_ends_search(const ViolPair &r) { return r.what == VIOL_P_FATAL; }
MC_HD int viol_pair_column(const ViolPair &r) { return r.what == VIOL_P_OUTSIDE ? 1 : -1; }
MC_HD bool viol_deadlocked(unsigned enabled_pairs, bool check_deadlock) { return check_deadlock && enabled_pairs == 0; }

template <class S, class Ref, class Own, class Ev>
MC_HD int viol_stored_bin(const typename S::Params &prm, Ref self, bool has_parent, Own &&own, Ev &&ev) {
    unsigned st;
    if constexpr (ViolChecksStored<S>::value) { (void)prm; (void)self; (void)has_parent; (void)ev; st = own(); }
    else {
        (void)own;
        if (!has_parent) st = S::init_status(prm, self);
        else st = ev();
    }
    if (!(st & ST_INVARIANT) || (st & (ST_ASSERT | ST_SPECERR | ST_OUT_OF_MODEL))) return -1;
    return (int)((st >> 8) & 31u);
}
template <class S, class Ref, class Own, class Ev>
MC_HD int viol_stored_bin(const typename S::Params &prm, Ref self, bool has_parent, int ninv, Own &&own, Ev &&ev) {
    const int bin = viol_stored_bin<S>(prm, self, has_parent, own, ev);
    return !ViolChecksStored<S>::value && bin >= ninv ? -1 : bin;
}

}
```

Measured before the change: 4.130 billion.

## Add packed raft state layout with fewer words per row for single-GPU runs

Introduces SpecRaftPacked, a raft spec variant that stores each state row in fewer 64-bit words by bit-packing server, message and log fields, selected by default for 2- and 3-server single-GPU engines. Export, import and trace paths translate between the packed and public layouts, and sharded calls rebuild an unpacked engine when nothing has been searched yet. The aim is to cut memory traffic and hash/store cost per state, at the price of extra pack/unpack arithmetic in the kernels and more code paths to keep consistent.

```diff
diff --git a/tla_rust_amd/build.py b/tla_rust_amd/build.py
--- a/tla_rust_amd/build.py
+++ b/tla_rust_amd/build.py
@@ -13,10 +13,11 @@
 ENGINE_BASE = ["engine.hip", "hip_owned.h", "engine_kernels.h", "engine_sim.h", "sim_walk.h", "engine_behaviours.h", "behaviour.h", "engine_coverage.h", "coverage.h", "engine_violations.h", "violations.h",
                "engine_graph.h",
                "graph.h", "liveness.h", "live_query.h", "state_graph.h", "spec_gen.h", "mc_common.h", "spec_registry.h", "../../include/tlamc.h"]
-ENGINE_OWN = {0: ["spec_pluscal.h", "spec_raft.h", "spec_ssi.h", "spec_vm.h", "spec_vm_cfg.h", "spec_paxos.h", "engine_pairs.h"], 7: ["spec_paxos.h"], 1: ["spec_pluscal.h"],
-              2: ["spec_raft.h"], 3: ["spec_raft.h"], 4: ["spec_raft.h"], 5: ["spec_ssi.h", "engine_pairs.h"], 6: ["spec_vm.h", "spec_vm_cfg.h"]}
+ENGINE_OWN = {0: ["spec_pluscal.h", "spec_raft.h", "spec_raft_packed.h", "spec_ssi.h", "spec_vm.h", "spec_vm_cfg.h", "spec_paxos.h", "engine_pairs.h"], 7: ["spec_paxos.h"], 1: ["spec_pluscal.h"],
+              2: ["spec_raft.h"], 3: ["spec_raft.h"], 4: ["spec_raft.h"], 5: ["spec_ssi.h", "engine_pairs.h"], 6: ["spec_vm.h", "spec_vm_cfg.h"],
+              12: ["spec_raft.h", "spec_raft_packed.h"], 13: ["spec_raft.h", "spec_raft_packed.h"]}
 STATE_GRAPH_DEPS = ["state_graph.hip", "state_graph.h", "engine_live.h", "hip_owned.h", "liveness.h", "live_query.h", "graph.h", "coverage.h", "mc_common.h", "spec_registry.h",
-                    "spec_gen.h", "spec_pluscal.h", "spec_raft.h", "spec_ssi.h", "spec_vm.h", "spec_vm_cfg.h", "spec_paxos.h", "../../include/tlamc.h"]
+                    "spec_gen.h", "spec_pluscal.h", "spec_raft.h", "spec_raft_packed.h", "spec_ssi.h", "spec_vm.h", "spec_vm_cfg.h", "spec_paxos.h", "../../include/tlamc.h"]
 
 
 def _stale(target, deps):
@@ -40,7 +41,7 @@
     if os.environ.get("TLAMC_PHASE_PROF"):
         common.append("-DMC_PHASE_PROF")
     jobs, objs = [], []
-    for tu in range(8):
+    for tu in sorted(ENGINE_OWN):
         obj = OUT / f"engine_tu{tu}.o"
         objs.append(obj)
         if force or _stale(obj, [CSRC / h for h in ENGINE_BASE + ENGINE_OWN[tu]]):
diff --git a/tla_rust_amd/csrc/coverage.h b/tla_rust_amd/csrc/coverage.h
--- a/tla_rust_amd/csrc/coverage.h
+++ b/tla_rust_amd/csrc/coverage.h
@@ -42,6 +42,17 @@
     static constexpr bool BY_SLOT = false;
     MC_HD static int nbins(const RaftParams &) { return 10 + 1; }
     MC_HD static bool listed(const RaftParams &, int a) { return a >= 0 && a < 10; }
+    template <class Ref>
+    MC_HD static int of(const RaftParams &p, const typename S::Local &l, Ref s, int slot) {
+        typename S::Delta d;
+        int action = -1;
+        S::compute(p, l, s, slot, d, action);
+        return action;
+    }
+};
+template <int N>
+struct CovAction<SpecRaftPacked<N>> : CovAction<SpecRaft<N>> {
+    using S = SpecRaftPacked<N>;
     template <class Ref>
     MC_HD static int of(const RaftParams &p, const typename S::Local &l, Ref s, int slot) {
         typename S::Delta d;
diff --git a/tla_rust_amd/csrc/engine.hip b/tla_rust_amd/csrc/engine.hip
--- a/tla_rust_amd/csrc/engine.hip
+++ b/tla_rust_amd/csrc/engine.hip
@@ -80,6 +80,8 @@
     virtual int shard_checkpoint(const char *path) = 0;
     virtual int shard_restore(const char *path) = 0;
     virtual size_t state_bytes() const = 0;
+    virtual int narrow_rows() const = 0;
+    mc_config created_with;
     virtual int simulate(const mc_sim_opts *opts, mc_sim_result *out) = 0;
     virtual int behaviours(const mc_beh_opts *opts, mc_beh_verdict *out, mc_beh_result *result) = 0;
     virtual int behaviours_refused() = 0;
@@ -144,6 +146,16 @@
 struct HasExport : std::false_type {};
 template <class S>
 struct HasExport<S, decltype((void)S::EXPORT_WORDS)> : std::true_type {};
+template <class S, class = void>
+struct RaftPacked : std::false_type {};
+template <class S>
+struct RaftPacked<S, decltype((void)S::RAFT_PACKED)> : std::true_type {};
+template <class S>
+static size_t export_words_of(const typename S::Params &prm, int W) {
+    if constexpr (RaftPacked<S>::value) return (size_t)S::export_words(prm);
+    else if constexpr (HasExport<S>::value) return (size_t)S::EXPORT_WORDS;
+    else return (size_t)W;
+}
 template <class S, class = void>
 struct PackedRows : std::false_type {};
 template <class S>
@@ -1278,8 +1290,8 @@
     int trace_out(const std::vector<uint64_t> &words, const std::vector<int32_t> &acts, uint8_t *states_out, int32_t *actions_out, size_t *n_inout) {
         const size_t n = acts.size();
         if (n > *n_inout) { *n_inout = n; set_error("trace buffer too small"); return MC_EBADCFG; }
-        if constexpr (HasExport<S>::value) {
-            for (size_t k = 0; k < n; ++k) S::export_row(prm, &words[k * W], (uint64_t *)states_out + k * (size_t)S::EXPORT_WORDS);
+        if constexpr (HasExport<S>::value || RaftPacked<S>::value) {
+            for (size_t k = 0; k < n; ++k) S::export_row(prm, &words[k * W], (uint64_t *)states_out + k * export_words_of<S>(prm, W));
         } else
         memcpy(states_out, words.data(), n * W * sizeof(uint64_t));
         memcpy(actions_out, acts.data(), n * sizeof(int32_t));
@@ -1297,12 +1309,12 @@
             const uint64_t n = count - off < piece ? count - off : piece;
             hipLaunchKernelGGL(k_gather_states, dim3((unsigned)((n * W + 255) / 256)), dim3(256), 0, stream, d_arena, W, first + off, n, tmp);
             hipError_t e1, e2;
-            if constexpr (HasExport<S>::value) {
+            if constexpr (HasExport<S>::value || RaftPacked<S>::value) {
                 std::vector<uint64_t> rows((size_t)n * W);
                 e1 = hipMemcpyAsync(rows.data(), tmp, n * W * sizeof(uint64_t), hipMemcpyDeviceToHost, stream);
                 e2 = hipStreamSynchronize(stream);
                 if (e1 == hipSuccess && e2 == hipSuccess)
-                    for (uint64_t k = 0; k < n; ++k) S::export_row(prm, &rows[(size_t)k * W], (uint64_t *)out + (size_t)(off + k) * (size_t)S::EXPORT_WORDS);
+                    for (uint64_t k = 0; k < n; ++k) S::export_row(prm, &rows[(size_t)k * W], (uint64_t *)out + (size_t)(off + k) * export_words_of<S>(prm, W));
             } else {
                 e1 = hipMemcpyAsync(out + off * W * sizeof(uint64_t), tmp, n * W * sizeof(uint64_t), hipMemcpyDeviceToHost, stream);
                 e2 = hipStreamSynchronize(stream);
@@ -1371,7 +1383,12 @@
     }
     static int refuse_packed() {
         if constexpr (PackedRows<S>::value) { set_error("this engine of generated code stores rows packed to its program's cell ranges and serves ONE GPU: create a sharded engine with shard_count > 1 (or $TLAMC_JIT_PACK=0)"); return MC_EBADCFG; }
-        return MC_OK;
+        if constexpr (RaftPacked<S>::value) { set_error("this raft engine has searched with its rows stored in fewer words (one GPU) and cannot go on in sharded steps: create the engine with shard_count > 1, make the mc_shard_* call before the first search, or set $TLAMC_RAFT_PACK=0"); return MC_EBADCFG; }
+        return MC_OK;
+    }
+    int narrow_rows() const override {
+        if constexpr (!RaftPacked<S>::value) return 0;
+        return !fr.have_run && !ck.pending && !sim.trace_n && fr.last_distinct == 0 ? 1 : 2;
     }
     void shard_reset_slots() {
         hipSetDevice(cfg.device);
@@ -1940,8 +1957,8 @@
     int sim_trace_out(uint8_t *states_out, int32_t *actions_out, size_t *n_inout) {
         const size_t n = sim.trace_n;
         if (n > *n_inout) { *n_inout = n; set_error("trace buffer too small"); return MC_EBADCFG; }
-        if constexpr (HasExport<S>::value) {
-            for (size_t k = 0; k < n; ++k) S::export_row(prm, &sim.trace_rows[k * W], (uint64_t *)states_out + k * (size_t)S::EXPORT_WORDS);
+        if constexpr (HasExport<S>::value || RaftPacked<S>::value) {
+            for (size_t k = 0; k < n; ++k) S::export_row(prm, &sim.trace_rows[k * W], (uint64_t *)states_out + k * export_words_of<S>(prm, W));
         } else
         memcpy(states_out, sim.trace_rows.data(), n * W * sizeof(uint64_t));
         memcpy(actions_out, sim.trace_acts.data(), n * sizeof(int32_t));
@@ -1977,9 +1994,15 @@
         struct Drain { hipStream_t s; ~Drain() { (void)hipStreamSynchronize(s); } } drain{stream};
         const uint32_t iters = o->iters ? o->iters : BEH_ITERS;
         const uint64_t R = chunk / 64 < o->count ? chunk / 64 : o->count;
-        std::vector<uint64_t> hmask(W, ~0ull);
-        if (o->mask) memcpy(hmask.data(), o->mask, (size_t)W * sizeof(uint64_t));
-        const bool full = beh_mask_full(hmask.data(), W);
+        const size_t PW = export_words_of<S>(prm, W);
+        std::vector<uint64_t> hmask(PW, ~0ull), imported;
+        if (o->mask) memcpy(hmask.data(), o->mask, PW * sizeof(uint64_t));
+        const bool full = beh_mask_full(hmask.data(), (int)PW);
+        if constexpr (RaftPacked<S>::value) {
+            std::vector<uint64_t> pm(hmask);
+            hmask.assign(W, 0);
+            S::import_row(prm, pm.data(), hmask.data());
+        }
         for (int k = 0; k < 2; ++k) HIP_TRY(beh.set[k].reserve(R * 64 * W));
         HIP_TRY(beh.stage.reserve(R * 64 * W));
         HIP_TRY(beh.first.reserve(R + 1));
@@ -2009,6 +2032,11 @@
             for (uint64_t k = 0; k <= n; ++k) rel[k] = o->first[b0 + k] - r0;
             for (uint64_t k = 0; k < n; ++k) longest = std::max(longest, rel[k + 1] - rel[k]);
             HIP_TRY(beh.rows.reserve(nrows * W));
+            if constexpr (RaftPacked<S>::value) {
+                imported.resize(nrows * W);
+                for (uint64_t k = 0; k < nrows; ++k) S::import_row(prm, (const uint64_t *)o->rows + (r0 + k) * PW, &imported[k * W]);
+                HIP_TRY(hipMemcpyAsync(beh.rows, imported.data(), nrows * W * sizeof(uint64_t), hipMemcpyHostToDevice, stream));
+            } else
             HIP_TRY(hipMemcpyAsync(beh.rows, o->rows + r0 * W * sizeof(uint64_t), nrows * W * sizeof(uint64_t), hipMemcpyHostToDevice, stream));
             HIP_TRY(hipMemcpyAsync(beh.first, rel.data(), (n + 1) * sizeof(uint64_t), hipMemcpyHostToDevice, stream));
             HIP_TRY(hipMemsetAsync(beh.carry, 0, n * sizeof(uint64_t), stream));
@@ -2072,6 +2100,7 @@
     e->prm = prm;
     e->desc = *spec;
     e->cfg = *cfg;
+    e->created_with = *cfg;
     const int r = e->alloc();
     if (r) { delete e; return r; }
     *out = e;
@@ -2086,6 +2115,8 @@
 int mc_make_engine_5(const mc_spec_desc *, const mc_config *, mc::EngineBase **);
 int mc_make_engine_6(const mc_spec_desc *, const mc_config *, mc::EngineBase **);
 int mc_make_engine_7(const mc_spec_desc *, const mc_config *, mc::EngineBase **);
+int mc_make_engine_2p(const mc_spec_desc *, const mc_config *, mc::EngineBase **);
+int mc_make_engine_3p(const mc_spec_desc *, const mc_config *, mc::EngineBase **);
 void *mc_jit_factory_opts(const void *program, int pack);
 #if MC_TU == 1 || MC_TU == -1
 int mc_make_engine_1(const mc_spec_desc *d, const mc_config *c, mc::EngineBase **out) {
@@ -2113,6 +2144,19 @@
 #endif
 #if MC_TU == 4 || MC_TU == -1
 MC_RAFT_FACTORY(4, SpecRaft5)
+#endif
+#define MC_RAFT_PACKED_FACTORY(K, NSRV)                                                            \
+    int mc_make_engine_##K##p(const mc_spec_desc *d, const mc_config *c, mc::EngineBase **out) {   \
+        mc::RaftParams p;                                                                          \
+        if (mc::SpecRaftPacked<NSRV>::make_params(d->params, d->nparams, p)) return MC_EBADCFG;    \
+        if (!mc::SpecRaftPacked<NSRV>::packable(p) || c->shard_count > 1) return MC_EBADCFG;       \
+        return mc::make_engine<mc::SpecRaftPacked<NSRV>>(p, d, c, out);                            \
+    }
+#if MC_TU == 12 || MC_TU == -1
+MC_RAFT_PACKED_FACTORY(2, 2)
+#endif
+#if MC_TU == 13 || MC_TU == -1
+MC_RAFT_PACKED_FACTORY(3, 3)
 #endif
 #if MC_TU == 5 || MC_TU == -1
 int mc_make_engine_5(const mc_spec_desc *d, const mc_config *c, mc::EngineBase **out) {
@@ -2188,6 +2232,32 @@
     EngineBase *impl;
 };
 
+static bool raft_rows_packed(const mc_spec_desc *spec, const mc_config *cfg) {
+    const char *ep = getenv("TLAMC_RAFT_PACK");
+    if ((ep && *ep == '0') || cfg->shard_count > 1 || spec->spec_id != MC_SPEC_RAFT || spec->nparams < 5) return false;
+    RaftParams p;
+    if (spec->params[0] == 2) return !SpecRaft2::make_params(spec->params, spec->nparams, p) && SpecRaftPacked<2>::packable(p);
+    if (spec->params[0] == 3) return !SpecRaft3::make_params(spec->params, spec->nparams, p) && SpecRaftPacked<3>::packable(p);
+    return false;
+}
+static int make_impl(const mc_spec_desc *spec, const mc_config *cfg, bool pack, EngineBase **impl);
+static EngineBase *shard_side(mc_engine *e) {
+    if (e->impl->narrow_rows() != 1) return e->impl;
+    const mc_spec_desc desc = *e->impl->spec_desc();
+    const mc_config cfg = e->impl->created_with;
+    mc_progress_fn fn = e->impl->progress_fn;
+    void *user = e->impl->progress_user;
+    const double interval = e->impl->progress_interval;
+    EngineBase *impl = nullptr;
+    if (make_impl(&desc, &cfg, false, &impl) != MC_OK) return e->impl;
+    delete e->impl;
+    impl->progress_fn = fn;
+    impl->progress_user = user;
+    impl->progress_interval = interval;
+    e->impl = impl;
+    return impl;
+}
+
 extern "C" {
 
 int mc_device_count(void) {
@@ -2215,12 +2285,20 @@
         cfg = &with_trace;
     }
     EngineBase *impl = nullptr;
+    const int rc = make_impl(spec, cfg, raft_rows_packed(spec, cfg), &impl);
+    if (rc == MC_OK) *out = new mc_engine{impl};
+    else if (rc == MC_EBADCFG && g_last_error.empty()) set_error("unknown spec id or constants out of range");
+    return rc;
+}
+}
+static int make_impl(const mc_spec_desc *spec, const mc_config *cfg, bool pack, EngineBase **out) {
+    EngineBase *impl = nullptr;
     const int group = spec_group(spec);
     int rc = MC_EBADCFG;
     switch (group) {
     case 1: rc = mc_make_engine_1(spec, cfg, &impl); break;
-    case 2: rc = mc_make_engine_2(spec, cfg, &impl); break;
-    case 3: rc = mc_make_engine_3(spec, cfg, &impl); break;
+    case 2: rc = pack ? mc_make_engine_2p(spec, cfg, &impl) : mc_make_engine_2(spec, cfg, &impl); break;
+    case 3: rc = pack ? mc_make_engine_3p(spec, cfg, &impl) : mc_make_engine_3(spec, cfg, &impl); break;
     case 4: rc = mc_make_engine_4(spec, cfg, &impl); break;
     case 5: rc = mc_make_engine_5(spec, cfg, &impl); break;
     case 6: {
@@ -2239,10 +2317,10 @@
     case 7: rc = mc_make_engine_7(spec, cfg, &impl); break;
     default: break;
     }
-    if (rc == MC_OK) *out = new mc_engine{impl};
-    else if (rc == MC_EBADCFG && g_last_error.empty()) set_error("unknown spec id or constants out of range");
+    if (rc == MC_OK) *out = impl;
     return rc;
 }
+extern "C" {
 int mc_engine_run(mc_engine *e, mc_result *out) { return e && out ? e->impl->run(out) : MC_EBADCFG; }
 int mc_engine_step(mc_engine *e, uint32_t levels, mc_result *out) { return e && out ? e->impl->step(levels, out) : MC_EBADCFG; }
 int mc_engine_set_progress(mc_engine *e, mc_progress_fn fn, void *user, double min_interval_seconds) {
@@ -2435,69 +2513,69 @@
 int mc_engine_debug_phases(mc_engine *e, uint64_t *out48, int reset) { return e && out48 ? e->impl->debug_phases(out48, reset) : MC_EBADCFG; }
 int mc_engine_debug_flags(mc_engine *e, uint32_t set, uint32_t clear) { return e ? e->impl->debug_flags(set, clear) : MC_EBADCFG; }
 int mc_engine_seen_layout(mc_engine *e, uint64_t *buckets, uint32_t *slots) { return e && buckets && slots ? e->impl->seen_layout(buckets, slots) : MC_EBADCFG; }
-int mc_shard_begin(mc_engine *e) { return e ? e->impl->shard_begin() : MC_EBADCFG; }
+int mc_shard_begin(mc_engine *e) { return e ? shard_side(e)->shard_begin() : MC_EBADCFG; }
 int mc_shard_begin_replicated(mc_engine *e, uint64_t min_frontier, uint64_t max_distinct, uint64_t max_levels, uint64_t *levels_out,
                               uint32_t *nlevels) {
-    return e && levels_out && nlevels ? e->impl->shard_begin_replicated(min_frontier, max_distinct, max_levels, levels_out, nlevels) : MC_EBADCFG;
-}
-int mc_shard_level_size(mc_engine *e, uint64_t *n) { return e && n ? e->impl->shard_level_size(n) : MC_EBADCFG; }
+    return e && levels_out && nlevels ? shard_side(e)->shard_begin_replicated(min_frontier, max_distinct, max_levels, levels_out, nlevels) : MC_EBADCFG;
+}
+int mc_shard_level_size(mc_engine *e, uint64_t *n) { return e && n ? shard_side(e)->shard_level_size(n) : MC_EBADCFG; }
 int mc_shard_info(mc_engine *e, void **main_stream_out, uint64_t *chunk_states_out, int32_t *traced_out) {
-    return e ? e->impl->shard_info(main_stream_out, chunk_states_out, traced_out) : MC_EBADCFG;
-}
-size_t mc_engine_state_bytes_internal(mc_engine *e) { return e ? e->impl->state_bytes() : 0; }
+    return e ? shard_side(e)->shard_info(main_stream_out, chunk_states_out, traced_out) : MC_EBADCFG;
+}
+size_t mc_engine_state_bytes_internal(mc_engine *e) { return e ? shard_side(e)->state_bytes() : 0; }
 int mc_shard_expand(mc_engine *e, uint64_t first, uint64_t count, uint64_t *send_fp, uint64_t send_cap, uint64_t *send_counts) {
     if (!e || !send_counts) return MC_EBADCFG;
-    const int rc = e->impl->shard_expand_launch(0, first, count, send_cap);
-    return rc ? rc : e->impl->shard_expand_finish(0, send_fp, send_cap, send_counts);
-}
-int mc_shard_set_stream(mc_engine *e, void *hip_stream, int enable) { return e ? e->impl->shard_set_stream(hip_stream, enable) : MC_EBADCFG; }
+    const int rc = shard_side(e)->shard_expand_launch(0, first, count, send_cap);
+    return rc ? rc : shard_side(e)->shard_expand_finish(0, send_fp, send_cap, send_counts);
+}
+int mc_shard_set_stream(mc_engine *e, void *hip_stream, int enable) { return e ? shard_side(e)->shard_set_stream(hip_stream, enable) : MC_EBADCFG; }
 int mc_shard_expand_launch(mc_engine *e, uint32_t slot, uint64_t first, uint64_t count, uint64_t send_cap) {
-    return e ? e->impl->shard_expand_launch(slot, first, count, send_cap) : MC_EBADCFG;
+    return e ? shard_side(e)->shard_expand_launch(slot, first, count, send_cap) : MC_EBADCFG;
 }
 int mc_shard_expand_finish(mc_engine *e, uint32_t slot, uint64_t *send_fp, uint64_t send_cap, uint64_t *send_counts) {
-    return e && send_counts ? e->impl->shard_expand_finish(slot, send_fp, send_cap, send_counts) : MC_EBADCFG;
+    return e && send_counts ? shard_side(e)->shard_expand_finish(slot, send_fp, send_cap, send_counts) : MC_EBADCFG;
 }
 int mc_shard_probe(mc_engine *e, const uint64_t *recv_fp, uint64_t n, uint8_t *answers) {
-    return e ? e->impl->shard_probe(recv_fp, n, answers) : MC_EBADCFG;
+    return e ? shard_side(e)->shard_probe(recv_fp, n, answers) : MC_EBADCFG;
 }
 int mc_shard_materialise(mc_engine *e, const uint8_t *answers_back, uint8_t *send_states, uint64_t send_cap, uint64_t *send_counts) {
-    return e && send_counts ? e->impl->shard_materialise(0, answers_back, send_states, send_cap, send_counts) : MC_EBADCFG;
+    return e && send_counts ? shard_side(e)->shard_materialise(0, answers_back, send_states, send_cap, send_counts) : MC_EBADCFG;
 }
 int mc_shard_materialise_slot(mc_engine *e, uint32_t slot, const uint8_t *answers_back, uint8_t *send_states, uint64_t send_cap,
                               uint64_t *send_counts) {
-    return e && send_counts ? e->impl->shard_materialise(slot, answers_back, send_states, send_cap, send_counts) : MC_EBADCFG;
-}
-int mc_shard_ingest(mc_engine *e, const uint8_t *recv_states, uint64_t n) { return e ? e->impl->shard_ingest(recv_states, n) : MC_EBADCFG; }
-int mc_shard_expand_pack(mc_engine *e, uint32_t slot, uint64_t *send_fp, uint64_t cap) { return e && send_fp ? e->impl->shard_expand_pack(slot, send_fp, cap) : MC_EBADCFG; }
+    return e && send_counts ? shard_side(e)->shard_materialise(slot, answers_back, send_states, send_cap, send_counts) : MC_EBADCFG;
+}
+int mc_shard_ingest(mc_engine *e, const uint8_t *recv_states, uint64_t n) { return e ? shard_side(e)->shard_ingest(recv_states, n) : MC_EBADCFG; }
+int mc_shard_expand_pack(mc_engine *e, uint32_t slot, uint64_t *send_fp, uint64_t cap) { return e && send_fp ? shard_side(e)->shard_expand_pack(slot, send_fp, cap) : MC_EBADCFG; }
 int mc_shard_probe_pack(mc_engine *e, const uint64_t *recv_fp, uint64_t cap, uint8_t *answers) {
-    return e && recv_fp && answers ? e->impl->shard_probe_pack(recv_fp, cap, answers) : MC_EBADCFG;
+    return e && recv_fp && answers ? shard_side(e)->shard_probe_pack(recv_fp, cap, answers) : MC_EBADCFG;
 }
 int mc_shard_keep_pack(mc_engine *e, uint32_t slot, const uint8_t *answers_back, uint64_t cap) {
-    return e && answers_back ? e->impl->shard_keep_pack(slot, answers_back, cap) : MC_EBADCFG;
-}
-int mc_shard_wait_keep(mc_engine *e, uint32_t slot) { return e ? e->impl->shard_wait_keep(slot) : MC_EBADCFG; }
-int mc_shard_keep(mc_engine *e, const uint8_t *answers_back, uint64_t *n_new) { return e && n_new ? e->impl->shard_keep(0, answers_back, n_new) : MC_EBADCFG; }
+    return e && answers_back ? shard_side(e)->shard_keep_pack(slot, answers_back, cap) : MC_EBADCFG;
+}
+int mc_shard_wait_keep(mc_engine *e, uint32_t slot) { return e ? shard_side(e)->shard_wait_keep(slot) : MC_EBADCFG; }
+int mc_shard_keep(mc_engine *e, const uint8_t *answers_back, uint64_t *n_new) { return e && n_new ? shard_side(e)->shard_keep(0, answers_back, n_new) : MC_EBADCFG; }
 int mc_shard_keep_slot(mc_engine *e, uint32_t slot, const uint8_t *answers_back, uint64_t *n_new) {
-    return e ? e->impl->shard_keep(slot, answers_back, n_new) : MC_EBADCFG;
-}
-int mc_shard_end_level(mc_engine *e, uint64_t *new_local) { return e && new_local ? e->impl->shard_end_level(new_local) : MC_EBADCFG; }
+    return e ? shard_side(e)->shard_keep(slot, answers_back, n_new) : MC_EBADCFG;
+}
+int mc_shard_end_level(mc_engine *e, uint64_t *new_local) { return e && new_local ? shard_side(e)->shard_end_level(new_local) : MC_EBADCFG; }
 int mc_shard_counters(mc_engine *e, uint64_t *generated, uint64_t *distinct_local, int32_t *verdict) {
-    return e && generated && distinct_local && verdict ? e->impl->shard_counters(generated, distinct_local, verdict) : MC_EBADCFG;
-}
-int mc_shard_check_frontier(mc_engine *e) { return e ? e->impl->shard_check_frontier() : MC_EBADCFG; }
-int mc_shard_materialise_parents(mc_engine *e, uint32_t slot, uint64_t *send_parents) { return e ? e->impl->shard_materialise_parents(slot, send_parents) : MC_EBADCFG; }
+    return e && generated && distinct_local && verdict ? shard_side(e)->shard_counters(generated, distinct_local, verdict) : MC_EBADCFG;
+}
+int mc_shard_check_frontier(mc_engine *e) { return e ? shard_side(e)->shard_check_frontier() : MC_EBADCFG; }
+int mc_shard_materialise_parents(mc_engine *e, uint32_t slot, uint64_t *send_parents) { return e ? shard_side(e)->shard_materialise_parents(slot, send_parents) : MC_EBADCFG; }
 int mc_shard_ingest_parents(mc_engine *e, const uint64_t *recv_parents, uint64_t n, uint32_t src_rank) {
-    return e ? e->impl->shard_ingest_parents(recv_parents, n, src_rank) : MC_EBADCFG;
+    return e ? shard_side(e)->shard_ingest_parents(recv_parents, n, src_rank) : MC_EBADCFG;
 }
 int mc_shard_violation(mc_engine *e, int32_t *found, uint64_t *idx, uint32_t *slot, int32_t *verdict, int32_t *invariant) {
-    return e && found && idx && slot && verdict && invariant ? e->impl->shard_violation(found, idx, slot, verdict, invariant) : MC_EBADCFG;
-}
-int mc_shard_note_levels(mc_engine *e, const uint64_t *levels, uint32_t n, int32_t verdict) { return e && (levels || !n) ? e->impl->shard_note_levels(levels, n, verdict) : MC_EBADCFG; }
-int mc_shard_resume(mc_engine *e, uint64_t *levels_out, uint32_t *nlevels) { return e && levels_out && nlevels ? e->impl->shard_resume(levels_out, nlevels) : MC_EBADCFG; }
-int mc_shard_checkpoint(mc_engine *e, const char *path) { return e && path ? e->impl->shard_checkpoint(path) : MC_EBADCFG; }
-int mc_shard_restore(mc_engine *e, const char *path) { return e && path ? e->impl->shard_restore(path) : MC_EBADCFG; }
+    return e && found && idx && slot && verdict && invariant ? shard_side(e)->shard_violation(found, idx, slot, verdict, invariant) : MC_EBADCFG;
+}
+int mc_shard_note_levels(mc_engine *e, const uint64_t *levels, uint32_t n, int32_t verdict) { return e && (levels || !n) ? shard_side(e)->shard_note_levels(levels, n, verdict) : MC_EBADCFG; }
+int mc_shard_resume(mc_engine *e, uint64_t *levels_out, uint32_t *nlevels) { return e && levels_out && nlevels ? shard_side(e)->shard_resume(levels_out, nlevels) : MC_EBADCFG; }
+int mc_shard_checkpoint(mc_engine *e, const char *path) { return e && path ? shard_side(e)->shard_checkpoint(path) : MC_EBADCFG; }
+int mc_shard_restore(mc_engine *e, const char *path) { return e && path ? shard_side(e)->shard_restore(path) : MC_EBADCFG; }
 int mc_shard_fetch(mc_engine *e, uint64_t idx, uint8_t *state_out, uint32_t *parent_rank, uint64_t *parent_idx, uint32_t *parent_slot) {
-    return e && state_out && parent_rank && parent_idx && parent_slot ? e->impl->shard_fetch(idx, state_out, parent_rank, parent_idx, parent_slot) : MC_EBADCFG;
+    return e && state_out && parent_rank && parent_idx && parent_slot ? shard_side(e)->shard_fetch(idx, state_out, parent_rank, parent_idx, parent_slot) : MC_EBADCFG;
 }
 
 }
diff --git a/tla_rust_amd/csrc/spec_raft_packed.h b/tla_rust_amd/csrc/spec_raft_packed.h
--- /dev/null
+++ b/tla_rust_amd/csrc/spec_raft_packed.h
@@ -0,0 +1,244 @@
+#pragma once
+#include "spec_raft.h"
+
+namespace mc {
+
+template <int NS>
+struct SpecRaftPacked : SpecRaft<NS> {
+    using B = SpecRaft<NS>;
+    using Params = RaftParams;
+    using Local = typename B::Local;
+    using Delta = typename B::Delta;
+    using Guards = typename B::Guards;
+    using Summary = typename B::Summary;
+    static constexpr bool RAFT_PACKED = true;
+    static constexpr int EL_BITS = 26;
+    static constexpr int P_FP = 0, P_GLOB = 1;
+    MC_HD static constexpr int P_SRV(int i) { return 2 + i; }
+    static constexpr int P_VL = 2 + NS;
+    static constexpr int P_MSG0 = 3 + NS;
+    MC_HD static int P_EL0(const Params &p) { return P_MSG0 + B::msg_words(p); }
+    MC_HD static int P_ALL0(const Params &p) { return P_MSG0 + B::msg_words(p) + p.ce; }
+    MC_HD static int words(const Params &p) { return P_MSG0 + B::msg_words(p) + p.ce + B::all_words(p); }
+    static constexpr int MAX_WORDS = B::MAX_WORDS;
+    static constexpr int PMAX_WORDS = P_MSG0 + 32 + 8 + 16;
+    MC_HD static int vbits(const Params &p) { return NS * p.lb; }
+    MC_HD static bool packable(const Params &p) { return NS * NS * p.lb <= 64 && EL_BITS + NS * p.lb <= 64; }
+    MC_HD static int export_words(const Params &p) { return B::words(p); }
+
+    template <class Ref>
+    struct View {
+        Ref r;
+        int vb, nmw, ce;
+        uint64_t vmask;
+        MC_HD uint64_t get(int w) const {
+            int phys = w, sh = 0;
+            uint64_t mask = ~0ull;
+            if (w >= 2 && w < B::W_MSG0) {
+                const int i = (w - 2) >> 1;
+                const bool vl = ((w - 2) & 1) != 0;
+                phys = vl ? P_VL : 2 + i;
+                sh = vl ? vb * i : 0;
+                mask = vl ? vmask : ~0ull;
+            } else if (w >= B::W_MSG0) {
+                const int e = w - B::W_MSG0 - nmw;
+                const bool el = e >= 0 && e < 2 * ce, hi = (e & 1) != 0;
+                phys = e < 0 ? w - (NS - 1) : el ? P_MSG0 + nmw + (e >> 1) : w - (NS - 1) - ce;
+                sh = el && hi ? EL_BITS : 0;
+                mask = el && !hi ? (1ull << EL_BITS) - 1ull : ~0ull;
+            }
+            return (r.get(phys) >> sh) & mask;
+        }
+    };
+    template <class Ref>
+    MC_HD static View<Ref> view(const Params &p, Ref s) { return View<Ref>{s, vbits(p), B::msg_words(p), p.ce, (1ull << vbits(p)) - 1ull}; }
+
+    static void export_row(const Params &p, const uint64_t *stored, uint64_t *pub) {
+        const View<CWordRef> v = view(p, CWordRef{stored, 1});
+        for (int w = 0; w < B::words(p); w++) pub[w] = v.get(w);
+    }
+    static void import_row(const Params &p, const uint64_t *pub, uint64_t *stored) {
+        const int vb = vbits(p), nmw = B::msg_words(p);
+        stored[P_FP] = pub[B::W_FP];
+        stored[P_GLOB] = pub[B::W_GLOB];
+        uint64_t vl = 0;
+        for (int i = 0; i < NS; i++) {
+            stored[P_SRV(i)] = pub[B::W_SRV(i)];
+            vl |= (pub[B::W_VL(i)] & ((1ull << vb) - 1ull)) << (vb * i);
+        }
+        stored[P_VL] = vl;
+        for (int m = 0; m < nmw; m++) stored[P_MSG0 + m] = pub[B::W_MSG0 + m];
+        for (int e = 0; e < p.ce; e++) {
+            const uint64_t *ew = pub + B::W_EL0(p) + e * B::EL_WORDS;
+            stored[P_EL0(p) + e] = (ew[0] & ((1ull << EL_BITS) - 1ull)) | ((ew[1] & ((1ull << vb) - 1ull)) << EL_BITS);
+        }
+        for (int a = 0; a < B::all_words(p); a++) stored[P_ALL0(p) + a] = pub[B::W_ALL0(p) + a];
+    }
+
+    template <class Ref>
+    MC_HD static void stage_range(const Params &, Ref s, int &lo, int &n) { lo = P_MSG0; n = (B::g_nm(s.get(P_GLOB)) + 1) >> 1; }
+    template <class Ref> MC_HD static uint64_t rd_msg(Ref s, int k) { return (s.get(P_MSG0 + (k >> 1)) >> (32 * (k & 1))) & 0xffffffffull; }
+    template <class Ref>
+    MC_HD static uint64_t fp_of(const Params &, Ref s) { return fp_nonzero(s.get(P_FP)); }
+    template <class Ref>
+    MC_HD static uint64_t fp_recompute(const Params &prm, Ref s) { return B::fp_recompute(prm, view(prm, s)); }
+    template <bool WANT_FP = true, class Ref>
+    MC_HD static void load(const Params &prm, Ref s, Local &l) { B::template load<WANT_FP>(prm, view(prm, s), l); }
+    template <class Ref>
+    MC_HD static void load_expand(const Params &prm, Ref s, Local &l, Guards &g) { B::load_expand(prm, view(prm, s), l, g); }
+    template <bool MEM = false, int FAM = -1, class Ref>
+    MC_HD static unsigned compute(const Params &prm, const Local &l, Ref s, int slot, Delta &d, int &action) {
+        return B::template compute<MEM, FAM>(prm, l, view(prm, s), slot, d, action);
+    }
+    template <class Ref>
+    MC_HD static bool message_generated_only(const Params &prm, const Local &l, Ref s, int slot) {
+        const int q = slot - B::FIX, k = q / 3;
+        return q % 3 == 1 && l.inflight >= prm.max_msgs && k < l.nm && B::m_count(rd_msg(s, k)) == 1;
+    }
+    template <int FAM, class Ref>
+    MC_HD static unsigned eval_pair(const Params &prm, const Summary &q, Ref s, int slot, uint64_t &fp) {
+        return B::template eval_pair<FAM>(prm, q, view(prm, s), slot, fp);
+    }
+    template <class Ref>
+    MC_HD static unsigned eval(const Params &prm, Local &l, Ref s, int slot, uint64_t &fp) { return B::eval(prm, l, view(prm, s), slot, fp); }
+
+    MC_HD static void init(const Params &prm, uint64_t, WordRef out) {
+        for (int w = 0; w < words(prm); w++) out.set(w, 0);
+        const uint64_t sv = B::sv_reset_leader_vars(B::sv_set_term(0, 1), 1);
+        for (int i = 0; i < NS; i++) out.set(P_SRV(i), B::pack_srv(sv, 0));
+        out.set(P_GLOB, B::pack_glob(1, 0));
+        out.set(P_FP, B::hheader(prm, view(prm, out)));
+    }
+
+    template <class Ref>
+    MC_HD static void store_row(const Params &prm, const Local &l, Ref s, const Delta &d, bool ok, uint64_t nfp, WordRef out) {
+        const int W = words(prm);
+        const uint64_t nglob = ok ? B::pack_glob(d.glob, d.clog) : 0ull;
+        const int srv = ok ? d.srv : -1;
+        const uint64_t nsrv = srv >= 0 ? B::pack_srv(d.sv, d.log) : 0ull;
+        const int vb = vbits(prm);
+        const int vm = srv >= 0 ? d.vmode : 0, vsh = vb * srv + (vm == 2 ? prm.lb * d.vj : 0);
+        const uint32_t vlog = (uint32_t)d.vlog;
+        const int wa = d.midxA >> 1, wb = d.midxB >> 1;
+        bool hasA = false, hasB = false;
+        uint64_t xa = 0, xb = 0;
+        if (ok && (d.nmop & 1)) {
+            xa = 2 * wa < l.nm ? s.get(P_MSG0 + wa) : 0ull;
+            xa = B::set_half(xa, d.midxA, d.mnewA);
+            if ((d.nmop & 2) && wb == wa) xa = B::set_half(xa, d.midxB, d.mnewB);
+            hasA = true;
+        }
+        if (ok && (d.nmop & 2) && !((d.nmop & 1) && wb == wa)) { xb = B::set_half(s.get(P_MSG0 + wb), d.midxB, d.mnewB); hasB = true; }
+        const int nmw = B::msg_words(prm), wel = P_MSG0 + nmw, wall = wel + prm.ce;
+        const int e0 = ok && d.eadd ? B::g_ne(l.glob) : -1;
+        constexpr int ALLW = (NS + 3) / 4 + 1;
+        int qlo = 0, qhi = -1;
+        uint64_t xall[ALLW];
+#pragma unroll
+        for (int j = 0; j < ALLW; j++) xall[j] = 0;
+        if (ok && l.nadd) {
+            const int na = B::g_na(l.glob);
+            qlo = na >> 2;
+            qhi = (na + l.nadd - 1) >> 2;
+            if (qhi >= B::all_words(prm)) qhi = B::all_words(prm) - 1;
+#pragma unroll
+            for (int j = 0; j < ALLW; j++) {
+                const int qq = qlo + j;
+                if (qq <= qhi) {
+                    uint64_t x = qq * 4 < na ? s.get(wall + qq) : 0ull;
+                    int pos = na;
+#pragma unroll
+                    for (int i = 0; i < NS; i++)
+                        if (l.addmask >> i & 1) {
+                            if (pos < prm.ca && (pos >> 2) == qq) x |= (s.get(P_SRV(i)) >> B::LOGSH) << (16 * (pos & 3));
+                            pos++;
+                        }
+                    xall[j] = x;
+                }
+            }
+        }
+        constexpr int COPY = 14;
+        uint64_t t[COPY];
+#pragma unroll
+        for (int w0 = 0; w0 < PMAX_WORDS; w0 += COPY) {
+            if (w0 < W) {
+#pragma unroll
+                for (int u = 0; u < COPY; u++) t[u] = s.get(w0 + u < W ? w0 + u : W - 1);
+#pragma unroll
+                for (int u = 0; u < COPY; u++) {
+                    const int w = w0 + u;
+                    if (w >= W) continue;
+                    uint64_t v = t[u];
+                    if (w == P_FP) { if (ok) v = nfp; }
+                    else if (w == P_GLOB) { if (ok) v = nglob; }
+                    else if (w < P_VL) { if (srv == w - 2) v = nsrv; }
+                    else if (w == P_VL) {
+                        if (vm == 1) v &= ~(((1ull << vb) - 1ull) << vsh);
+                        if (vm == 2) v |= (uint64_t)vlog << vsh;
+                    }
+                    else {
+                        const int mw = w - P_MSG0;
+                        if (mw < nmw) {
+                            if (hasA && wa == mw) v = xa;
+                            if (hasB && wb == mw) v = xb;
+                        } else if (w < wall) {
+                            if (w - wel == e0) v = d.ew.get(0) | (d.ew.get(1) << EL_BITS);
+                        } else {
+                            const int qq = w - wall;
+#pragma unroll
+                            for (int j = 0; j < ALLW; j++) if (qq == qlo + j && qq <= qhi) v = xall[j];
+                        }
+                    }
+                    out.set(w, v);
+                }
+            }
+        }
+    }
+    template <bool KNOWN, class Ref>
+    MC_HD static unsigned apply_eval_store(const Params &prm, Ref s, int slot, uint64_t fp_known, WordRef out) {
+        prefetch_row(s, words(prm));
+        const View<Ref> v = view(prm, s);
+        Local l;
+        B::template load<!KNOWN>(prm, v, l);
+        Delta d;
+        int action;
+        const unsigned st = B::template compute<true>(prm, l, v, slot, d, action);
+        const bool ok = (st & ST_ENABLED) && !(st & (ST_OVERFLOW | ST_SPECERR));
+        const uint64_t nfp = !ok ? 0ull : KNOWN ? fp_known : B::delta_fp(prm, l, v, d);
+        store_row(prm, l, s, d, ok, nfp, out);
+        return st;
+    }
+    template <class Ref>
+    MC_HD static unsigned apply(const Params &prm, Ref s, int slot, WordRef out) { return apply_eval_store<false>(prm, s, slot, 0, out); }
+    template <class Ref>
+    MC_HD static unsigned apply_known_fp(const Params &prm, Ref s, int slot, uint64_t fp_nz, WordRef out) {
+        if (fp_nz == fp_nonzero(0)) return apply_eval_store<false>(prm, s, slot, 0, out);
+        return apply_eval_store<true>(prm, s, slot, fp_nz, out);
+    }
+    template <class Ref>
+    MC_HD static unsigned apply_summary_patch(const Params &prm, const Summary &q, Ref s, int slot, uint64_t fp_nz, WordRef out) {
+        const View<Ref> v = view(prm, s);
+        Local l;
+        B::template local_of_summary<-1>(q, v, l);
+        Delta d;
+        int action;
+        const unsigned st = B::template compute<true>(prm, l, v, slot, d, action);
+        const bool ok = (st & ST_ENABLED) && !(st & (ST_OVERFLOW | ST_SPECERR));
+        const uint64_t nfp = !ok ? 0ull : fp_nz != fp_nonzero(0) ? fp_nz : B::delta_fp(prm, l, v, d);
+        store_row(prm, l, s, d, ok, nfp, out);
+        return st;
+    }
+
+    static int action_of(const Params &prm, const uint64_t *parent, int slot) {
+        uint64_t pub[B::MAX_WORDS];
+        export_row(prm, parent, pub);
+        return B::action_of(prm, pub, slot);
+    }
+    static int format(const Params &prm, const uint64_t *w, char *buf, size_t cap) {
+        uint64_t pub[B::MAX_WORDS];
+        export_row(prm, w, pub);
+        return B::format(prm, pub, buf, cap);
+    }
+};
+
+}
diff --git a/tla_rust_amd/csrc/spec_registry.h b/tla_rust_amd/csrc/spec_registry.h
--- a/tla_rust_amd/csrc/spec_registry.h
+++ b/tla_rust_amd/csrc/spec_registry.h
@@ -3,6 +3,7 @@
 #include "spec_paxos.h"
 #include "spec_pluscal.h"
 #include "spec_raft.h"
+#include "spec_raft_packed.h"
 #include "spec_ssi.h"
 #include "spec_vm.h"
 #include "spec_vm_cfg.h"
diff --git a/tla_rust_amd/csrc/violations.h b/tla_rust_amd/csrc/violations.h
--- a/tla_rust_amd/csrc/violations.h
+++ b/tla_rust_amd/csrc/violations.h
@@ -18,6 +18,7 @@
 template <> struct ViolModel<SpecAtomicAdd> { MC_HD static int ninv(const SpecAtomicAdd::Params &) { return 0; } };
 template <> struct ViolModel<SpecPcalIntro> { MC_HD static int ninv(const SpecPcalIntro::Params &) { return 1; } };
 template <int N> struct ViolModel<SpecRaft<N>> { MC_HD static int ninv(const RaftParams &) { return 2; } };
+template <int N> struct ViolModel<SpecRaftPacked<N>> : ViolModel<SpecRaft<N>> {};
 template <> struct ViolModel<SpecSsi> { MC_HD static int ninv(const SsiParams &) { return 8; } };
 template <> struct ViolModel<SpecPaxos> { MC_HD static int ninv(const PaxosParams &p) { return p.kind == 1 ? 1 : 4; } };
 template <int MAXV> struct ViolModel<SpecVmT<MAXV>> { MC_HD static int ninv(const VmParams &p) { return p.ninv; } };
```

Measured after the change: 4.228 billion (median of 6 runs). 1.02x the previous value.
